# lmb-freiburg/flownet2

Hardware: AMD Instinct MI355X
Metric: image-pairs/sec FlowNetC forward at 448x320 (higher is better)
Workload: dtype f32

## Files before the change

flownet2_amd/_lib.py:

```python
from __future__ import annotations

import ctypes as C
import os
import re

_HERE = os.path.dirname(os.path.abspath(__file__))
SO_PATH = os.path.join(_HERE, "libflownet2_hip.so")
INCLUDE_DIR = os.path.join(_HERE, "..", "include")

_SCALARS = {"int": C.c_int, "float": C.c_float, "size_t": C.c_size_t, "long long": C.c_longlong, "unsigned long long": C.c_ulonglong,
            "char": C.c_char}
_POINTERS = {"float": C.c_void_p, "double": C.c_void_p, "void": C.c_void_p, "unsigned char": C.c_void_p, "char": C.c_char_p, "int": C.POINTER(C.c_int),
             "unsigned": C.POINTER(C.c_uint), "size_t": C.POINTER(C.c_size_t)}
_STRUCT_NAMES = {"fn2_l1loss_params": "L1LossParams", "fn2_l1loss_scale": "L1LossScale"}
_DECLARATOR = re.compile(r"^([\w\s*]*?)(\w+)\s*(?:\[(\d+)\])?$")
_FUNCTION = re.compile(r"^([\w\s*]+?)\b(fn2_\w+)\s*\(([^()]*)\)$")


class Fn2Error(RuntimeError):

    def __init__(self, status: int, message: str):
        super().__init__(f"[fn2 status {status}] {message}")
        self.status = status


def _ctype(spec, structs, where):
    words = [w for w in spec.replace("*", " ").split() if w != "const"]
    base, stars = " ".join(words), spec.count("*")
    if stars == 0 and base in _SCALARS:
        return _SCALARS[base]
    if stars == 1 and base in structs:
        return C.POINTER(structs[base])
    if stars == 1 and base in _POINTERS:
        return _POINTERS[base]
    if stars == 2 and base in ("float", "void"):
        return C.POINTER(C.c_void_p)
    raise ValueError(f"C header: unknown type `{spec.strip()}` in `{where}`")


def _declarator(text, structs, where):
    m = _DECLARATOR.match(text.strip())
    if not m or not m.group(1).strip():
        raise ValueError(f"C header: cannot read `{text.strip()}` in `{where}`")
    t = _ctype(m.group(1), structs, where)
    return m.group(2), (t * int(m.group(3)) if m.group(3) else t), m.group(1)


def parse_header(text, structs=None):
    structs = dict(structs or {})
    functions, constants = {}, {}
    text = re.sub(r"/\*.*?\*/", " ", text, flags=re.S)
    for name, value in re.findall(r"^[ \t]*#[ \t]*define[ \t]+(FN2_\w+)[ \t]+(-?(?:0[xX][0-9a-fA-F]+|\d+))[ \t]*$", text, flags=re.M):
        constants[name] = int(value, 0)
    text = re.sub(r"^[ \t]*#.*$", " ", text, flags=re.M)

    def enum(m):
        value = -1
        for item in filter(None, (s.strip() for s in m.group(1).split(","))):
            name, _, v = (s.strip() for s in item.partition("="))
            value = int(v, 0) if v else value + 1
            constants[name] = value
        return " "
    text = re.sub(r"(?:typedef\s+)?enum\s*\w*\s*\{([^{}]*)\}\s*\w*\s*;", enum, text)

    def struct(m):
        cname, fields = m.group(1), []
        for decl in filter(None, (s.strip() for s in m.group(2).split(";"))):
            first, *more = decl.split(",")
            name, t, spec = _declarator(first, structs, "struct " + cname)
            fields.append((name, t))
            fields += [_declarator(spec + " " + other, structs, "struct " + cname)[:2] for other in more]
        pyname = _STRUCT_NAMES.get(cname) or "".join(w.capitalize() for w in cname.split("_")[1:])
        structs[cname] = type(pyname, (C.Structure,), {"_fields_": fields, "__doc__": cname, "__module__": __name__})
        return " "
    text = re.sub(r"typedef\s+struct\s+(fn2_\w+)\s*\{([^{}]*)\}\s*\w+\s*;", struct, text)

    text = re.sub(r'extern\s*"C"\s*\{|\}', " ", text)
    for stmt in filter(None, (" ".join(s.split()) for s in text.split(";"))):
        m = _FUNCTION.match(stmt)
        if not m:
            raise ValueError(f"C header: cannot read the declaration `{stmt}`")
        params = m.group(3).strip()
        args = [] if params == "void" else [_declarator(p, structs, stmt)[1] for p in params.split(",")]
        functions[m.group(2)] = (_ctype(m.group(1), structs, stmt), args)
    return functions, structs, constants


def _parse_headers():
    per_header, structs, constants, metrics = [], {}, {}, {}
    for h in ("flownet2_hip.h", "flownet2_hip_solver.h", "flownet2_hip_corr_route.h", "flownet2_hip_conv_general.h",
              "flownet2_hip_conv_geometry.h", "flownet2_hip_conv_volume.h", "flownet2_hip_lpq_loss.h", "flownet2_hip_flow_metrics.h"):
        with open(os.path.join(INCLUDE_DIR, h)) as f:
            functions, structs, c = parse_header(f.read(), structs)
        per_header.append(functions)
        (metrics if h == "flownet2_hip_flow_metrics.h" else constants).update(c)
    return per_header, structs, constants, metrics


_PER_HEADER, _STRUCTS, CONSTANTS, FLOW_METRICS_CONSTANTS = _parse_headers()
(EXPORTS, SOLVER_EXPORTS, CORR_ROUTE_EXPORTS, CONV_GENERAL_EXPORTS, CONV_GEOMETRY_EXPORTS, CONV_VOLUME_EXPORTS, LPQ_LOSS_EXPORTS,
 FLOW_METRICS_EXPORTS) = (list(f) for f in _PER_HEADER)
PROTOTYPES = {name: proto for f in _PER_HEADER for name, proto in f.items()}
globals().update({cls.__name__: cls for cls in _STRUCTS.values()})
_HOOKS = parse_header("""
    int fn2_debug_set_correlation_impl(int impl);
    int fn2_debug_correlation_units_plan(int N, int H, int W, int policy, unsigned* out_words, int max_words);
    int fn2_debug_set_resample_generic(int on);
    int fn2_debug_set_correlation_trace(void* device_buffer);""")[0]

_lib = None


def lib():
    global _lib
    if _lib is not None:
        return _lib
    if not os.path.exists(SO_PATH):
        raise RuntimeError(
            f"{SO_PATH} not found: the HIP extension is not built. Run `python -m flownet2_amd.build` "
            "(or __graft_entry__.build()). flownet2_amd has no CPU / PyTorch fallback.")
    L = C.CDLL(SO_PATH)
    for table, required in ((PROTOTYPES, True), (_HOOKS, False)):
        for name, (restype, argtypes) in table.items():
            if not hasattr(L, name):
                if required:
                    raise RuntimeError(f"{SO_PATH} does not export {name}")
                continue
            fn = getattr(L, name)
            fn.restype, fn.argtypes = restype, argtypes
    _lib = L
    return L


def check(status: int):
    if status != 0:
        raise Fn2Error(status, lib().fn2_last_error_string().decode())


def version() -> str:
    return lib().fn2_version().decode()
```

flownet2_amd/csrc/bias_act.hip:

```cpp
#include "fn2_common.hpp"

namespace fn2 {

using f32x4 = __attribute__((ext_vector_type(4))) float;

template <bool VEC4>
__global__ void __launch_bounds__(256) bias_leaky_relu(float* __restrict__ data, const float* __restrict__ bias,
                                                       int C, unsigned hw, float slope) {
  const unsigned plane = blockIdx.y;
  const float b = bias ? bias[plane % (unsigned)C] : 0.f;
  float* p = data + (size_t)plane * hw;
  if constexpr (VEC4) {
    const unsigned n4 = hw / 4;
    for (unsigned i = blockIdx.x * blockDim.x + threadIdx.x; i < n4; i += gridDim.x * blockDim.x) {
      f32x4 v = reinterpret_cast<f32x4*>(p)[i];
#pragma unroll
      for (int j = 0; j < 4; ++j) { const float t = v[j] + b; v[j] = t > 0.f ? t : t * slope; }
      reinterpret_cast<f32x4*>(p)[i] = v;
    }
  } else {
    for (unsigned i = blockIdx.x * blockDim.x + threadIdx.x; i < hw; i += gridDim.x * blockDim.x) {
      const float t = p[i] + b;
      p[i] = t > 0.f ? t : t * slope;
    }
  }
}

constexpr int kBwdChunks = 8;

template <bool MASK, bool VEC4>
__global__ void __launch_bounds__(256) bias_leaky_relu_bwd(const float* __restrict__ top_data, const float* __restrict__ top_diff,
                                                           float* __restrict__ bottom_diff, float* __restrict__ partial,
                                                           unsigned hw, float slope, int C, int dctot, int dc0, int yctot, int yc0) {
  __shared__ float red[4];
  const unsigned plane = blockIdx.y;
  const size_t base = (size_t)plane * hw;
  const size_t dbase = ((size_t)(plane / (unsigned)C) * dctot + dc0 + plane % (unsigned)C) * hw;
  const size_t ybase = ((size_t)(plane / (unsigned)C) * yctot + yc0 + plane % (unsigned)C) * hw;
  float acc = 0.f;
  if constexpr (VEC4) {
    const unsigned n4 = hw / 4;
    for (unsigned i = blockIdx.x * 256u + threadIdx.x; i < n4; i += gridDim.x * 256u) {
      f32x4 g = reinterpret_cast<const f32x4*>(top_diff + dbase)[i];
      if constexpr (MASK) {
        const f32x4 y = reinterpret_cast<const f32x4*>(top_data + ybase)[i];
#pragma unroll
        for (int j = 0; j < 4; ++j) g[j] *= y[j] > 0.f ? 1.f : slope;
        reinterpret_cast<f32x4*>(bottom_diff + base)[i] = g;
      }
      acc += (g[0] + g[1]) + (g[2] + g[3]);
    }
  } else {
    for (unsigned i = blockIdx.x * 256u + threadIdx.x; i < hw; i += gridDim.x * 256u) {
      float g = top_diff[dbase + i];
      if constexpr (MASK) {
        g *= top_data[ybase + i] > 0.f ? 1.f : slope;
        bottom_diff[base + i] = g;
      }
      acc += g;
    }
  }
#pragma unroll
  for (int m = 32; m > 0; m >>= 1) acc += __shfl_xor(acc, m, 64);
  if ((threadIdx.x & 63) == 0) red[threadIdx.x >> 6] = acc;
  __syncthreads();
  if (threadIdx.x == 0) partial[(size_t)plane * gridDim.x + blockIdx.x] = (red[0] + red[1]) + (red[2] + red[3]);
}

template <bool MASK, bool VEC4>
__global__ void __launch_bounds__(256) bias_leaky_relu_bwd_channel(const float* __restrict__ top_data, const float* __restrict__ top_diff,
                                                                   float* __restrict__ bottom_diff, float* __restrict__ bias_diff,
                                                                   int N, unsigned hw, float slope, int C, int dctot, int dc0, int yctot, int yc0,
                                                                   int accumulate) {
  __shared__ float red[4];
  const unsigned c = blockIdx.x;
  float acc = 0.f;
  if constexpr (VEC4) {
    const unsigned q = hw / 4, total = (unsigned)N * q;
    for (unsigned e = threadIdx.x; e < total; e += 256u) {
      const unsigned n = e / q, i = e - n * q;
      f32x4 g = reinterpret_cast<const f32x4*>(top_diff + ((size_t)n * dctot + dc0 + c) * hw)[i];
      if constexpr (MASK) {
        const f32x4 y = reinterpret_cast<const f32x4*>(top_data + ((size_t)n * yctot + yc0 + c) * hw)[i];
#pragma unroll
        for (int j = 0; j < 4; ++j) g[j] *= y[j] > 0.f ? 1.f : slope;
        reinterpret_cast<f32x4*>(bottom_diff + ((size_t)n * C + c) * hw)[i] = g;
      }
      acc += (g[0] + g[1]) + (g[2] + g[3]);
    }
  } else {
    const unsigned total = (unsigned)N * hw;
    for (unsigned e = threadIdx.x; e < total; e += 256u) {
      const unsigned n = e / hw, i = e - n * hw;
      float g = top_diff[((size_t)n * dctot + dc0 + c) * hw + i];
      if constexpr (MASK) {
        g *= top_data[((size_t)n * yctot + yc0 + c) * hw + i] > 0.f ? 1.f : slope;
        bottom_diff[((size_t)n * C + c) * hw + i] = g;
      }
      acc += g;
    }
  }
#pragma unroll
  for (int m = 32; m > 0; m >>= 1) acc += __shfl_xor(acc, m, 64);
  if ((threadIdx.x & 63) == 0) red[threadIdx.x >> 6] = acc;
  __syncthreads();
  if (threadIdx.x == 0 && bias_diff) {
    const float tot = (red[0] + red[1]) + (red[2] + red[3]);
    bias_diff[c] = accumulate ? bias_diff[c] + tot : tot;
  }
}

__global__ void __launch_bounds__(256) bias_diff_finalize(const float* __restrict__ partial, float* __restrict__ bias_diff,
                                                          int N, int C, int chunks, int accumulate) {
  const int c = blockIdx.x * 4 + (threadIdx.x >> 6), lane = threadIdx.x & 63;
  if (c >= C) return;
  const int total = N * chunks;
  float acc = 0.f;
  for (int i = lane; i < total; i += 64) {
    const int n = i / chunks, k = i - n * chunks;
    acc += partial[((size_t)n * C + c) * chunks + k];
  }
#pragma unroll
  for (int m = 32; m > 0; m >>= 1) acc += __shfl_xor(acc, m, 64);
  if (lane == 0) bias_diff[c] = accumulate ? bias_diff[c] + acc : acc;
}

static inline bool small_map(int N, int C, long long hw) { return C >= 128 && (long long)N * hw <= 20000; }

}

using namespace fn2;

FN2_API size_t fn2_bias_leaky_relu_backward_workspace_bytes(int N, int C, int H, int W) {
  (void)H; (void)W;
  if (N <= 0 || C <= 0) return 0;
  return sizeof(float) * (size_t)N * C * kBwdChunks;
}

FN2_API int fn2_bias_leaky_relu_backward_slices(const float* top_data, const float* top_diff, int diff_channels, int diff_c0,
                                                float* bottom_diff, float* bias_diff, int N, int C, int H, int W, float negative_slope,
                                                void* workspace, size_t workspace_bytes, void* stream) {
  return fn2_bias_leaky_relu_backward_slices2(top_data, C, 0, top_diff, diff_channels, diff_c0, bottom_diff, bias_diff, N, C, H, W, negative_slope,
                                              workspace, workspace_bytes, stream);
}

FN2_API int fn2_bias_leaky_relu_backward_slices2(const float* top_data, int data_channels, int data_c0, const float* top_diff, int diff_channels,
                                                 int diff_c0, float* bottom_diff, float* bias_diff, int N, int C, int H, int W, float negative_slope,
                                                 void* workspace, size_t workspace_bytes, void* stream) {
  if (N < 0 || C <= 0 || H <= 0 || W <= 0) return fail(FN2_ERR_INVALID_ARG, "bias_leaky_relu_backward: bad shape [%d,%d,%d,%d]", N, C, H, W);
  if (diff_c0 < 0 || diff_c0 + C > diff_channels) return fail(FN2_ERR_INVALID_ARG, "bias_leaky_relu_backward: top_diff slice outside its blob");
  if (data_c0 < 0 || data_c0 + C > data_channels) return fail(FN2_ERR_INVALID_ARG, "bias_leaky_relu_backward: top_data slice outside its blob");
  if (N == 0) return FN2_OK;
  if (!top_data || !top_diff || !bottom_diff) return fail(FN2_ERR_INVALID_ARG, "bias_leaky_relu_backward: null blob");
  const long long planes = (long long)N * C, hw = (long long)H * W;
  if (planes > 65535 || hw >= (1ll << 32)) return fail(FN2_ERR_UNSUPPORTED, "bias_leaky_relu_backward: blob too large");
  const size_t need = fn2_bias_leaky_relu_backward_workspace_bytes(N, C, H, W);
  if (!workspace || workspace_bytes < need) return fail(FN2_ERR_WORKSPACE, "bias_leaky_relu_backward: workspace too small (%zu < %zu)", workspace_bytes, need);
  hipStream_t st = reinterpret_cast<hipStream_t>(stream);
  float* partial = reinterpret_cast<float*>(workspace);
  const bool vec = hw % 4 == 0 && ((reinterpret_cast<uintptr_t>(top_data) | reinterpret_cast<uintptr_t>(top_diff) | reinterpret_cast<uintptr_t>(bottom_diff)) & 15) == 0;
  if (small_map(N, C, hw)) {
    if (vec) hipLaunchKernelGGL((bias_leaky_relu_bwd_channel<true, true>), dim3((unsigned)C), dim3(256), 0, st, top_data, top_diff, bottom_diff, bias_diff, N,
                                (unsigned)hw, negative_slope, C, diff_channels, diff_c0, data_channels, data_c0, 0);
    else hipLaunchKernelGGL((bias_leaky_relu_bwd_channel<true, false>), dim3((unsigned)C), dim3(256), 0, st, top_data, top_diff, bottom_diff, bias_diff, N,
                            (unsigned)hw, negative_slope, C, diff_channels, diff_c0, data_channels, data_c0, 0);
    return check_launch("bias_leaky_relu_backward");
  }
  if (vec) hipLaunchKernelGGL((bias_leaky_relu_bwd<true, true>), dim3(kBwdChunks, (unsigned)planes), dim3(256), 0, st, top_data, top_diff, bottom_diff, partial,
                              (unsigned)hw, negative_slope, C, diff_channels, diff_c0, data_channels, data_c0);
  else hipLaunchKernelGGL((bias_leaky_relu_bwd<true, false>), dim3(kBwdChunks, (unsigned)planes), dim3(256), 0, st, top_data, top_diff, bottom_diff, partial,
                          (unsigned)hw, negative_slope, C, diff_channels, diff_c0, data_channels, data_c0);
  if (bias_diff) hipLaunchKernelGGL(bias_diff_finalize, dim3((C + 3) / 4), dim3(256), 0, st, partial, bias_diff, N, C, kBwdChunks, 0);
  return check_launch("bias_leaky_relu_backward");
}

FN2_API int fn2_conv_backward_bias(const float* top_diff, int diff_channels, int diff_c0, float* bias_diff, int N, int C, int H, int W,
                                   int accumulate, void* workspace, size_t workspace_bytes, void* stream) {
  if (N < 0 || C <= 0 || H <= 0 || W <= 0) return fail(FN2_ERR_INVALID_ARG, "conv_backward_bias: bad shape [%d,%d,%d,%d]", N, C, H, W);
  if (diff_c0 < 0 || diff_c0 + C > diff_channels) return fail(FN2_ERR_INVALID_ARG, "conv_backward_bias: top_diff slice outside its blob");
  if (N == 0) return FN2_OK;
  if (!top_diff || !bias_diff) return fail(FN2_ERR_INVALID_ARG, "conv_backward_bias: null blob");
  const long long planes = (long long)N * C, hw = (long long)H * W;
  if (planes > 65535 || hw >= (1ll << 32)) return fail(FN2_ERR_UNSUPPORTED, "conv_backward_bias: blob too large");
  const size_t need = fn2_bias_leaky_relu_backward_workspace_bytes(N, C, H, W);
  if (!workspace || workspace_bytes < need) return fail(FN2_ERR_WORKSPACE, "conv_backward_bias: workspace too small (%zu < %zu)", workspace_bytes, need);
  hipStream_t st = reinterpret_cast<hipStream_t>(stream);
  float* partial = reinterpret_cast<float*>(workspace);
  const bool vec = hw % 4 == 0 && (reinterpret_cast<uintptr_t>(top_diff) & 15) == 0;
  if (small_map(N, C, hw)) {
    if (vec) hipLaunchKernelGGL((bias_leaky_relu_bwd_channel<false, true>), dim3((unsigned)C), dim3(256), 0, st, nullptr, top_diff, nullptr, bias_diff, N,
                                (unsigned)hw, 1.0f, C, diff_channels, diff_c0, C, 0, accumulate);
    else hipLaunchKernelGGL((bias_leaky_relu_bwd_channel<false, false>), dim3((unsigned)C), dim3(256), 0, st, nullptr, top_diff, nullptr, bias_diff, N,
                            (unsigned)hw, 1.0f, C, diff_channels, diff_c0, C, 0, accumulate);
    return check_launch("conv_backward_bias");
  }
  if (vec) hipLaunchKernelGGL((bias_leaky_relu_bwd<false, true>), dim3(kBwdChunks, (unsigned)planes), dim3(256), 0, st, nullptr, top_diff, nullptr, partial,
                              (unsigned)hw, 1.0f, C, diff_channels, diff_c0, C, 0);
  else hipLaunchKernelGGL((bias_leaky_relu_bwd<false, false>), dim3(kBwdChunks, (unsigned)planes), dim3(256), 0, st, nullptr, top_diff, nullptr, partial,
                          (unsigned)hw, 1.0f, C, diff_channels, diff_c0, C, 0);
  hipLaunchKernelGGL(bias_diff_finalize, dim3((C + 3) / 4), dim3(256), 0, st, partial, bias_diff, N, C, kBwdChunks, accumulate);
  return check_launch("conv_backward_bias");
}

FN2_API int fn2_bias_leaky_relu_backward(const float* top_data, const float* top_diff, float* bottom_diff, float* bias_diff,
                                         int N, int C, int H, int W, float negative_slope, void* workspace, size_t workspace_bytes,
                                         void* stream) {
  return fn2_bias_leaky_relu_backward_slices(top_data, top_diff, C, 0, bottom_diff, bias_diff, N, C, H, W, negative_slope, workspace,
                                             workspace_bytes, stream);
}

FN2_API int fn2_bias_leaky_relu_forward(float* data, const float* bias, int N, int C, int H, int W, float negative_slope,
                                        void* stream) {
  if (N < 0 || C <= 0 || H <= 0 || W <= 0) return fail(FN2_ERR_INVALID_ARG, "bias_leaky_relu: bad shape [%d,%d,%d,%d]", N, C, H, W);
  if (N == 0) return FN2_OK;
  if (!data) return fail(FN2_ERR_INVALID_ARG, "bias_leaky_relu: null blob");
  const long long planes = (long long)N * C, hw = (long long)H * W;
  if (planes > 65535 * 32ll || hw >= (1ll << 32)) return fail(FN2_ERR_UNSUPPORTED, "bias_leaky_relu: blob too large");
  hipStream_t st = reinterpret_cast<hipStream_t>(stream);
  const bool vec = hw % 4 == 0 && (reinterpret_cast<uintptr_t>(data) & 15) == 0;
  const unsigned per = (unsigned)(vec ? hw / 4 : hw);
  unsigned bx = (per + 255) / 256;
  if (bx > 64) bx = 64;
  for (long long p0 = 0; p0 < planes; p0 += 65535) {
    const unsigned py = (unsigned)((planes - p0) < 65535 ? (planes - p0) : 65535);
    float* base = data + (size_t)p0 * hw;
    const float* bb = bias;
    if (p0 % C != 0) return fail(FN2_ERR_UNSUPPORTED, "bias_leaky_relu: N*C > 65535 with C not dividing 65535");
    if (vec) hipLaunchKernelGGL(bias_leaky_relu<true>, dim3(bx, py), dim3(256), 0, st, base, bb, C, (unsigned)hw, negative_slope);
    else     hipLaunchKernelGGL(bias_leaky_relu<false>, dim3(bx, py), dim3(256), 0, st, base, bb, C, (unsigned)hw, negative_slope);
  }
  return check_launch("bias_leaky_relu_forward");
}

namespace fn2 {
template <bool VEC4>
__global__ void __launch_bounds__(256) scale_shift(const float* __restrict__ in, float* __restrict__ out, const float* __restrict__ shift,
                                                   int C, unsigned hw, int out_ctot, int out_c0, float scale) {
  const unsigned plane = blockIdx.y;
  const unsigned n = plane / (unsigned)C, c = plane % (unsigned)C;
  const float sh = shift ? shift[c] : 0.f;
  const float* p = in + (size_t)plane * hw;
  float* q = out + ((size_t)n * out_ctot + out_c0 + c) * hw;
  if constexpr (VEC4) {
    const unsigned n4 = hw / 4;
    for (unsigned i = blockIdx.x * blockDim.x + threadIdx.x; i < n4; i += gridDim.x * blockDim.x) {
      f32x4 v = reinterpret_cast<const f32x4*>(p)[i];
#pragma unroll
      for (int j = 0; j < 4; ++j) {
        float prod = v[j] * scale;
        asm volatile("" : "+v"(prod));
        v[j] = prod + sh;
      }
      reinterpret_cast<f32x4*>(q)[i] = v;
    }
  } else {
    for (unsigned i = blockIdx.x * blockDim.x + threadIdx.x; i < hw; i += gridDim.x * blockDim.x) {
      float prod = p[i] * scale;
      asm volatile("" : "+v"(prod));
      q[i] = prod + sh;
    }
  }
}
}

FN2_API int fn2_scale_shift_forward(const float* bottom, float* top, const float* shift, int N, int C, int H, int W,
                                    int top_channels, int top_c0, float scale, void* stream) {
  if (N < 0 || C < 1 || H < 1 || W < 1) return fn2::fail(FN2_ERR_INVALID_ARG, "scale_shift: bad shape [%d,%d,%d,%d]", N, C, H, W);
  if (top_c0 < 0 || top_c0 + C > top_channels) return fn2::fail(FN2_ERR_INVALID_ARG, "scale_shift: channel slice outside the blob");
  if (N == 0) return FN2_OK;
  if (!bottom || !top) return fn2::fail(FN2_ERR_INVALID_ARG, "scale_shift: NULL blob pointer");
  if ((long long)N * C > 65535) return fn2::fail(FN2_ERR_UNSUPPORTED, "scale_shift: too many planes");
  const unsigned hw = (unsigned)H * (unsigned)W;
  const bool vec = hw % 4 == 0 && ((reinterpret_cast<uintptr_t>(bottom) | reinterpret_cast<uintptr_t>(top)) & 15) == 0;
  if (vec) hipLaunchKernelGGL(fn2::scale_shift<true>, dim3(fn2::blocks_for(hw / 4, 256, 256), (unsigned)(N * C)), dim3(256), 0, fn2::as_stream(stream), bottom, top,
                              shift, C, hw, top_channels, top_c0, scale);
  else hipLaunchKernelGGL(fn2::scale_shift<false>, dim3(fn2::blocks_for(hw, 256, 64), (unsigned)(N * C)), dim3(256), 0, fn2::as_stream(stream), bottom, top, shift,
                          C, hw, top_channels, top_c0, scale);
  return fn2::check_launch("scale_shift_forward");
}
```

flownet2_amd/csrc/conv_mfma.hip:

```cpp
#include "mfma_tile.hpp"

namespace fn2 {
namespace cv {

using namespace mfma;

struct Args {
  const float* in; const float* wp; const float* bias; float* out;
  int N, Cin, Hin, Win, in_ctot, in_c0;
  int Cout, Hout, Wout, out_ctot, out_c0;
  int pad;
  int nchunks;
  int ksteps;
  int tx, ty;
  int ng;
  unsigned total;
  unsigned nbig;
  float slope; int relu;
};

template <int KS_, int S_, int MW_, int NP_, int WM_, int WNX_, int WNY_, int CQ_, int P16_ = 0, int PIN_ = 0>
struct Cfg : Window<((P16_ ? 1 : 4) * WNY_ - 1) * S_ + KS_,
                    ((P16_ ? 16 : 4) * NP_ * WNX_ - 1) * S_ + KS_ + 4,
                    CQ_, WM_ * WNX_ * WNY_> {
// ... 170 lines not shown
}

template <int KS> struct PackTile {
  static constexpr int T = KS * KS;
  static constexpr int QT = KS == 1 ? 8 : KS == 3 ? 3 : KS == 4 ? 2 : 1;
  static constexpr int CIL = 4 * QT, ROW = CIL * T + 1;
  static constexpr int LDS_FLOATS = 64 * ROW;
};

template <int KS, int ORDER>
__global__ void __launch_bounds__(256) pack_weights_view(const float* __restrict__ w, float* __restrict__ wp, int ksteps, int kalloc,
                                                         int src_co, int src_ci, long long s_co, long long s_ci, int flip) {
  using P = PackTile<KS>;
  constexpr int T = P::T, QT = P::QT, CIL = P::CIL, ROW = P::ROW;
  __shared__ float tile[P::LDS_FLOATS];
  const int grp = blockIdx.x, cq0 = blockIdx.y * QT;
  const int co0 = 64 * grp, ci0 = 4 * cq0;
  const int nquads = ksteps / T;
  constexpr int TOTAL = 64 * CIL * T;
  if constexpr (ORDER == 0) {
    const float* src = w + (size_t)co0 * s_co + (size_t)ci0 * T;
#pragma unroll
    for (int i = threadIdx.x; i < TOTAL; i += 256) {
      const int col = i / (CIL * T), e = i - col * (CIL * T), c = e / T;
      tile[col * ROW + e] = (co0 + col < src_co && ci0 + c < src_ci) ? src[(size_t)col * s_co + e] : 0.f;
    }
  } else if constexpr (ORDER == 1) {
    const float* src = w + (size_t)ci0 * s_ci + (size_t)co0 * T;
#pragma unroll
    for (int i = threadIdx.x; i < TOTAL; i += 256) {
      const int c = i / (64 * T), e = i - c * (64 * T), col = e / T, t = e - col * T;
      tile[col * ROW + c * T + t] = (co0 + col < src_co && ci0 + c < src_ci) ? src[(size_t)c * s_ci + e] : 0.f;
    }
  } else {
#pragma unroll
    for (int i = threadIdx.x; i < TOTAL; i += 256) {
      const int col = i / (CIL * T), e = i - col * (CIL * T), c = e / T, t = e - c * T;
      tile[col * ROW + e] = (co0 + col < src_co && ci0 + c < src_ci) ? w[(size_t)(co0 + col) * s_co + (size_t)(ci0 + c) * s_ci + t] : 0.f;
    }
  }
  __syncthreads();
  const int nq = min(QT, nquads - cq0);
  float* dst = wp + ((size_t)grp * kalloc + (size_t)cq0 * T) * 256;
  const int j = threadIdx.x & 3, lane = threadIdx.x >> 2;
  const float* trow = tile + (16 * j + (lane & 15)) * ROW + (lane >> 4) * T;
#pragma unroll
  for (int ks = 0; ks < QT * T; ++ks) {
    const int cq = ks / T, tap = ks - cq * T;
    if (cq < nq) dst[ks * 256 + threadIdx.x] = trow[4 * cq * T + (flip ? T - 1 - tap : tap)];
  }
  if (cq0 + QT >= nquads)
    for (int i = threadIdx.x; i < (kalloc - ksteps) * 256; i += 256) wp[((size_t)grp * kalloc + ksteps) * 256 + i] = 0.f;
}

template <int KS>
static void launch_pack_view(const float* w, float* wp, int Cout, int ksteps, int kalloc, int src_co, int src_ci, long long s_co, long long s_ci, int flip,
                             hipStream_t st) {
  using P = PackTile<KS>;
  const dim3 grid((unsigned)((Cout + 63) / 64), (unsigned)cdiv(ksteps / P::T, P::QT));
  if (s_ci == (long long)P::T) hipLaunchKernelGGL((pack_weights_view<KS, 0>), grid, dim3(256), 0, st, w, wp, ksteps, kalloc, src_co, src_ci, s_co, s_ci, flip);
  else if (s_co == (long long)P::T) hipLaunchKernelGGL((pack_weights_view<KS, 1>), grid, dim3(256), 0, st, w, wp, ksteps, kalloc, src_co, src_ci, s_co, s_ci, flip);
  else hipLaunchKernelGGL((pack_weights_view<KS, 2>), grid, dim3(256), 0, st, w, wp, ksteps, kalloc, src_co, src_ci, s_co, s_ci, flip);
}

constexpr int kSpare = 8;
constexpr int kChunkQuads = 2;

inline int chunk_quads(int KS) { return KS == 1 ? 8 : kChunkQuads; }
inline int ksteps_for(int Cin, int KS) { return cdiv(cdiv(Cin, 4), chunk_quads(KS)) * chunk_quads(KS) * KS * KS; }

template <class K>
static void set_geometry(Args& a) {
  if constexpr (K::P16) {
    a.Win *= a.Hin; a.Hin = 1; a.Wout *= a.Hout; a.Hout = 1;
  }
  a.tx = cdiv(a.Wout, K::TW); a.ty = cdiv(a.Hout, K::TH);
  a.ng = a.Cout / (16 * K::MW * K::WM);
  a.nchunks = cdiv(cdiv(a.Cin, 4), K::CQ);
}

inline long long tiles_of(const Args& a) { return (long long)a.N * a.tx * a.ty * a.ng; }

template <class K>
static int launch(const Args& base, hipStream_t st) {
  Args a = base;
  set_geometry<K>(a);
  a.nbig = (unsigned)tiles_of(a);
  return launch_tiles<&conv_mfma<K>>(a, tiles_of(a), K::THREADS, (int)(sizeof(float) * 2 * K::BUF), "conv_mfma", "conv_mfma_forward", st);
}

inline unsigned whole_rounds(long long tiles) { return (unsigned)(tiles / 256 * 256); }

template <class K>
static int launch_tail(const Args& base, hipStream_t st) {
  if constexpr (K::MW < 2) {
    return fail(FN2_ERR_UNSUPPORTED, "conv_mfma: variant has no split tail");
  } else {
    Args a = base;
    set_geometry<K>(a);
    if (tiles_of(a) > 0x1fffff00ll) return fail(FN2_ERR_UNSUPPORTED, "conv_mfma: grid too large");
    a.total = (unsigned)tiles_of(a); a.nbig = whole_rounds(a.total);
    const unsigned nsm = 2 * (a.total - a.nbig);
    const unsigned grid = a.nbig + 8 * ((nsm + 7) / 8);
    constexpr size_t lds = sizeof(float) * 2 * K::BUF;
    set_dynamic_lds_once<&conv_mfma_tail<K>>((int)lds);
    hipLaunchKernelGGL((conv_mfma_tail<K>), dim3(grid), dim3(K::THREADS), lds, st, a);
    return check_launch("conv_mfma_forward");
  }
}

struct Variant {
  int ks, s, mw, np, wm, wnx, wny, p16;
  int (*fn)(const Args&, hipStream_t);
  int (*fn_tail)(const Args&, hipStream_t);
};

#define FN2_CV_LIST(X) \
   \
  X(1, 1, 2, 7, 2, 2, 1, 8, 1) X(1, 1, 2, 7, 2, 1, 2, 8, 1) X(1, 1, 4, 7, 1, 2, 2, 8, 0) X(1, 1, 4, 7, 1, 1, 4, 8, 0) X(1, 1, 2, 6, 2, 2, 1, 8, 1) \
  X(1, 1, 2, 4, 2, 2, 1, 8, 1) X(1, 1, 2, 7, 1, 2, 2, 8, 0) X(1, 1, 2, 7, 1, 4, 1, 8, 0) X(1, 1, 2, 4, 1, 2, 2, 8, 0) X(1, 1, 4, 4, 1, 2, 2, 8, 0) \
   \
  X(3, 1, 2, 7, 2, 2, 1, 2, 1) X(3, 1, 2, 7, 2, 1, 2, 2, 1) X(3, 1, 4, 7, 1, 2, 2, 2, 0) X(3, 1, 4, 7, 1, 1, 4, 2, 0) \
  X(3, 1, 2, 6, 2, 2, 1, 2, 1) X(3, 1, 4, 6, 1, 2, 2, 2, 0) X(3, 1, 4, 4, 1, 2, 2, 2, 0) X(3, 1, 2, 4, 2, 2, 1, 2, 1) \
   \
  X(3, 2, 2, 7, 2, 1, 2, 2, 1) X(3, 2, 4, 7, 1, 1, 4, 2, 0) X(3, 2, 2, 6, 2, 2, 1, 2, 1) X(3, 2, 4, 6, 1, 2, 2, 2, 0) X(3, 2, 2, 4, 2, 2, 1, 2, 1) \
   \
  X(4, 2, 2, 7, 2, 2, 1, 2, 1) X(4, 2, 2, 7, 2, 1, 2, 2, 1) X(4, 2, 4, 7, 1, 2, 2, 2, 0) X(4, 2, 2, 6, 2, 2, 1, 2, 1) X(4, 2, 4, 4, 1, 2, 2, 2, 0) X(4, 2, 2, 4, 2, 2, 1, 2, 1) \
   \
  X(5, 2, 2, 7, 2, 2, 1, 1, 1) X(5, 2, 2, 7, 2, 1, 2, 1, 1) X(5, 2, 4, 7, 1, 2, 2, 1, 0) X(5, 2, 4, 7, 1, 1, 4, 1, 0) \
  X(5, 2, 2, 6, 2, 2, 1, 1, 1) X(5, 2, 4, 6, 1, 2, 2, 1, 0) X(5, 2, 4, 4, 1, 2, 2, 1, 0) \
   \
  X(7, 2, 2, 6, 2, 2, 1, 1, 1) X(7, 2, 2, 7, 2, 2, 1, 1, 1) X(7, 2, 4, 4, 1, 2, 2, 1, 0) X(7, 2, 4, 6, 1, 2, 2, 1, 0) X(7, 2, 2, 4, 2, 2, 1, 1, 1)

template <class K, int TAIL> struct TailFn { static constexpr int (*fn)(const Args&, hipStream_t) = nullptr; };
template <class K> struct TailFn<K, 1> { static constexpr int (*fn)(const Args&, hipStream_t) = &launch_tail<K>; };

#define FN2_CV_ROW(KS, S, MW, NP, WM, WNX, WNY, CQ, TAIL) \
  {KS, S, MW, NP, WM, WNX, WNY, 0, &launch<Cfg<KS, S, MW, NP, WM, WNX, WNY, CQ>>, TailFn<Cfg<KS, S, MW, NP, WM, WNX, WNY, CQ>, TAIL>::fn},
#define FN2_CV_ROW16(MW, NP, WM, WNX, WNY, TAIL) \
  {1, 1, MW, NP, WM, WNX, WNY, 1, &launch<Cfg<1, 1, MW, NP, WM, WNX, WNY, 8, 1>>, TailFn<Cfg<1, 1, MW, NP, WM, WNX, WNY, 8, 1>, TAIL>::fn},
#define FN2_CV_PIN(KS, S, MW, NP, WM, WNX, WNY, CQ, P16, TAIL) \
  {KS, S, MW, NP, WM, WNX, WNY, P16, &launch<Cfg<KS, S, MW, NP, WM, WNX, WNY, CQ, P16, 1>>, TailFn<Cfg<KS, S, MW, NP, WM, WNX, WNY, CQ, P16, 1>, TAIL>::fn},
static const Variant kVariants[] = {FN2_CV_LIST(FN2_CV_ROW)
  FN2_CV_ROW16(2, 7, 2, 2, 1, 1) FN2_CV_ROW16(2, 7, 4, 1, 1, 1) FN2_CV_ROW16(4, 7, 1, 4, 1, 0) FN2_CV_ROW16(4, 7, 2, 2, 1, 0) FN2_CV_ROW16(2, 5, 2, 2, 1, 1)
  FN2_CV_ROW16(2, 4, 2, 2, 1, 1) FN2_CV_ROW16(2, 7, 1, 4, 1, 0) FN2_CV_ROW16(2, 5, 1, 4, 1, 0) FN2_CV_ROW16(4, 5, 1, 4, 1, 0) FN2_CV_ROW16(2, 4, 1, 4, 1, 0)
  FN2_CV_ROW16(4, 5, 2, 2, 1, 0) FN2_CV_ROW16(4, 4, 2, 2, 1, 0)
  FN2_CV_ROW16(2, 9, 4, 1, 1, 1) FN2_CV_ROW16(2, 9, 2, 2, 1, 1) FN2_CV_ROW16(2, 3, 2, 2, 1, 1) FN2_CV_ROW16(4, 3, 1, 4, 1, 0)
  FN2_CV_ROW16(4, 9, 4, 1, 1, 0) FN2_CV_ROW16(4, 9, 2, 2, 1, 0) FN2_CV_ROW16(4, 7, 4, 1, 1, 0)
  FN2_CV_PIN(5, 2, 2, 7, 2, 2, 1, 1, 0, 1) FN2_CV_PIN(5, 2, 2, 7, 2, 1, 2, 1, 0, 1)
  FN2_CV_PIN(1, 1, 4, 9, 4, 1, 1, 8, 1, 0) FN2_CV_PIN(1, 1, 2, 9, 4, 1, 1, 8, 1, 1) FN2_CV_PIN(1, 1, 2, 5, 2, 2, 1, 8, 1, 1) FN2_CV_PIN(1, 1, 4, 7, 4, 1, 1, 8, 1, 0)
  FN2_CV_PIN(1, 1, 2, 7, 2, 2, 1, 8, 1, 1) FN2_CV_PIN(1, 1, 2, 3, 2, 2, 1, 8, 1, 1)
  FN2_CV_PIN(3, 1, 2, 7, 2, 2, 1, 2, 0, 1) FN2_CV_PIN(3, 1, 2, 6, 2, 2, 1, 2, 0, 1) FN2_CV_PIN(3, 2, 2, 7, 2, 1, 2, 2, 0, 1) FN2_CV_PIN(3, 2, 2, 6, 2, 2, 1, 2, 0, 1)
  FN2_CV_PIN(4, 2, 2, 7, 2, 2, 1, 2, 0, 1) FN2_CV_PIN(4, 2, 2, 6, 2, 2, 1, 2, 0, 1) FN2_CV_PIN(5, 2, 2, 6, 2, 2, 1, 1, 0, 1)
  FN2_CV_PIN(7, 2, 2, 6, 2, 2, 1, 1, 0, 1) FN2_CV_PIN(7, 2, 4, 6, 1, 2, 2, 1, 0, 0)};
constexpr int kNumVariants = sizeof(kVariants) / sizeof(kVariants[0]);

int g_forced_variant = -1;

static double variant_cost(const Variant& v, const Args& a, bool tail) {
  const int tw = (v.p16 ? 16 : 4) * v.np * v.wnx, th = (v.p16 ? 1 : 4) * v.wny;
  const long long wgs = v.p16 ? (long long)a.N * cdiv(a.Wout * a.Hout, tw) * (a.Cout / (16 * v.mw * v.wm))
                              : (long long)a.N * cdiv(a.Wout, tw) * cdiv(a.Hout, th) * (a.Cout / (16 * v.mw * v.wm));
  double rounds = (double)((wgs + 255) / 256);
  if (tail) {
    const long long r = wgs % 256;
    if (wgs < 256 || r == 0 || r > 128) return 1e30;
    rounds = (double)(wgs / 256) + 0.5 * 1.12;
  }
  const double eff = 1.0 / (1.0 + 0.08 * (4.0 / v.mw - 1.0) + 0.02 * (7.0 / v.np - 1.0));
  return rounds * v.mw * v.np / eff;
}

static bool variant_applies(const Variant& v, const Args& a, int KS, int S) {
  if (!v.p16 && a.Win % 4 != 0) return false;
  return v.ks == KS && v.s == S && a.Cout % (16 * v.mw * v.wm) == 0;
}

}
}

using namespace fn2;

FN2_API size_t fn2_conv_mfma_packed_floats(int Cout, int Cin, int kernel) {
  if (Cout <= 0 || Cout % 32 != 0 || Cin <= 0 || kernel <= 0) return 0;
  return (size_t)((Cout + 63) / 64) * (cv::ksteps_for(Cin, kernel) + cv::kSpare) * 256;
}

FN2_API int fn2_conv_mfma_pack_weights_view(const float* weight, float* packed, int Cout, int Cin, int kernel, int src_cout, int src_cin,
                                            long long stride_cout, long long stride_cin, int flip, void* stream);

FN2_API int fn2_conv_mfma_pack_weights(const float* weight, float* packed, int Cout, int Cin, int kernel, void* stream) {
  if (!weight || !packed) return fail(FN2_ERR_INVALID_ARG, "conv_mfma_pack_weights: null blob");
  if (Cout <= 0 || Cout % 32 != 0 || Cin <= 0 || (kernel != 1 && kernel != 3 && kernel != 4 && kernel != 5 && kernel != 7))
    return fail(FN2_ERR_UNSUPPORTED, "conv_mfma_pack_weights: needs Cout %% 32 == 0 and kernel_size 1, 3, 4, 5 or 7 (got Cout %d, kernel %d)", Cout, kernel);
  return fn2_conv_mfma_pack_weights_view(weight, packed, Cout, Cin, kernel, Cout, Cin, (long long)Cin * kernel * kernel, (long long)kernel * kernel, 0, stream);
}

FN2_API int fn2_conv_mfma_pack_weights_view(const float* weight, float* packed, int Cout, int Cin, int kernel, int src_cout, int src_cin,
                                            long long stride_cout, long long stride_cin, int flip, void* stream) {
  if (!weight || !packed) return fail(FN2_ERR_INVALID_ARG, "conv_mfma_pack_weights_view: null blob");
  if (Cout <= 0 || Cout % 32 != 0 || Cin <= 0 || (kernel != 1 && kernel != 3 && kernel != 4 && kernel != 5 && kernel != 7))
    return fail(FN2_ERR_UNSUPPORTED, "conv_mfma_pack_weights_view: needs Cout %% 32 == 0 and kernel_size 1, 3, 4, 5 or 7 (got Cout %d, kernel %d)", Cout, kernel);
  if (src_cout < 1 || src_cout > Cout || src_cin < 1 || src_cin > Cin || stride_cout < 1 || stride_cin < 1)
    return fail(FN2_ERR_INVALID_ARG, "conv_mfma_pack_weights_view: bad source view (%d of %d, %d of %d channels, strides %lld / %lld)", src_cout, Cout,
                src_cin, Cin, stride_cout, stride_cin);
  const int ksteps = cv::ksteps_for(Cin, kernel), kalloc = ksteps + cv::kSpare;
  hipStream_t st = as_stream(stream);
  switch (kernel) {
    case 1: cv::launch_pack_view<1>(weight, packed, Cout, ksteps, kalloc, src_cout, src_cin, stride_cout, stride_cin, flip ? 1 : 0, st); break;
    case 3: cv::launch_pack_view<3>(weight, packed, Cout, ksteps, kalloc, src_cout, src_cin, stride_cout, stride_cin, flip ? 1 : 0, st); break;
    case 4: cv::launch_pack_view<4>(weight, packed, Cout, ksteps, kalloc, src_cout, src_cin, stride_cout, stride_cin, flip ? 1 : 0, st); break;
    case 5: cv::launch_pack_view<5>(weight, packed, Cout, ksteps, kalloc, src_cout, src_cin, stride_cout, stride_cin, flip ? 1 : 0, st); break;
    default: cv::launch_pack_view<7>(weight, packed, Cout, ksteps, kalloc, src_cout, src_cin, stride_cout, stride_cin, flip ? 1 : 0, st); break;
  }
  return check_launch("conv_mfma_pack_weights_view");
}

FN2_API int fn2_conv_mfma_supported(int Cin, int Hin, int Win, int Cout, int kernel, int stride, int pad) {
  if (Cin <= 0 || Hin <= 0 || Win <= 0 || Cout <= 0 || Cout % 32 != 0) return 0;
  if (kernel == 1 ? ((long long)Hin * Win) % 4 != 0 : Win % 4 != 0) return 0;
  if (!((kernel == 1 && stride == 1) || (kernel == 3 && (stride == 1 || stride == 2)) || (kernel == 4 && stride == 2) || (kernel == 5 && stride == 2) || (kernel == 7 && stride == 2))) return 0;
  if (pad < 0 || pad > 4 || pad > kernel - 1) return 0;
  if ((long long)Cin * Hin * Win >= (1ll << 28)) return 0;
  const int Hout = (Hin + 2 * pad - kernel) / stride + 1, Wout = (Win + 2 * pad - kernel) / stride + 1;
  if (Hout < 1 || Wout < 1) return 0;
  cv::Args a{};
  a.Win = Win; a.Cout = Cout;
  for (int i = 0; i < cv::kNumVariants; ++i)
    if (cv::variant_applies(cv::kVariants[i], a, kernel, stride)) return 1;
  return 0;
}

FN2_API int fn2_debug_set_conv_variant(int v) { cv::g_forced_variant = v; return FN2_OK; }
FN2_API int fn2_conv_mfma_num_variants(void) { return cv::kNumVariants; }

FN2_API int fn2_conv_mfma_forward(const float* bottom, const float* packed_weight, const float* bias, float* top,
                                  int N, int Cin, int Hin, int Win, int bottom_channels, int bottom_c0,
                                  int Cout, int top_channels, int top_c0, int kernel, int stride, int pad,
                                  int relu, float negative_slope, void* stream) {
  if (N < 0) return fail(FN2_ERR_INVALID_ARG, "conv_mfma: bad batch");
  if (N == 0) return FN2_OK;
  if (const int rc = mfma::check_conv_args("conv_mfma", bottom, packed_weight, top, Cin, bottom_channels, bottom_c0, Cout, top_channels, top_c0, [&] {
        return fn2_conv_mfma_supported(Cin, Hin, Win, Cout, kernel, stride, pad) ? FN2_OK
            : fail(FN2_ERR_UNSUPPORTED, "conv_mfma: unsupported geometry (Cin %d, %dx%d, Cout %d, k %d s %d p %d)", Cin, Hin, Win, Cout, kernel, stride, pad);
      }))
    return rc;
  cv::Args a{};
  a.in = bottom; a.wp = packed_weight; a.bias = bias; a.out = top;
  a.N = N; a.Cin = Cin; a.Hin = Hin; a.Win = Win; a.in_ctot = bottom_channels; a.in_c0 = bottom_c0;
  a.Cout = Cout; a.Hout = (Hin + 2 * pad - kernel) / stride + 1; a.Wout = (Win + 2 * pad - kernel) / stride + 1;
  a.out_ctot = top_channels; a.out_c0 = top_c0; a.pad = pad;
  a.ksteps = cv::ksteps_for(Cin, kernel) + cv::kSpare;
  a.slope = negative_slope; a.relu = relu;
  hipStream_t st = as_stream(stream);
  static TuneCache cache("conv_mfma", cv::kNumVariants);
  const TuneKey key{N, Cin, Hin, Win, Cout, kernel, stride, pad, bottom_channels == Cin, top_channels == Cout};
  mfma::Pick p;
  if (const int rc = mfma::pick_variant(p, "conv_mfma", cv::g_forced_variant, cv::kNumVariants, true, cache, key, st,
                                        [&](int i) { return cv::variant_applies(cv::kVariants[i], a, kernel, stride); },
                                        [&](int i, bool tail) { return cv::variant_cost(cv::kVariants[i], a, tail); },
                                        [&](int i, bool tail) { return tail ? cv::kVariants[i].fn_tail(a, st) : cv::kVariants[i].fn(a, st); },
                                        [&](int i) { return cv::kVariants[i].fn_tail != nullptr; }))
    return rc;
  return p.tail ? cv::kVariants[p.variant].fn_tail(a, st) : cv::kVariants[p.variant].fn(a, st);
}
```

flownet2_amd/csrc/flow_head.hip:

```cpp
#include "fn2_common.hpp"

namespace fn2 {

constexpr int kHeadPix = 64;

template <int G>
__global__ void __launch_bounds__(kHeadPix* G) conv3x3_c2_taps(const float* __restrict__ in, const float* __restrict__ w,
                                                                float* __restrict__ P, int N, int C, int H, int W, int nsplit) {
  __shared__ float red[G][18][kHeadPix];
  const int lane_pix = threadIdx.x % kHeadPix;
  const int grp = __builtin_amdgcn_readfirstlane(threadIdx.x / kHeadPix);
  const size_t plane = (size_t)H * W;
  const long long total = (long long)N * H * W;
  const long long p = (long long)blockIdx.x * kHeadPix + lane_pix;
  const bool live = p < total;
  const int n = live ? (int)(p / (long long)plane) : 0;
  const unsigned pix = live ? (unsigned)(p - (long long)n * plane) : 0u;
  const float* src = in + (size_t)n * C * plane + pix;
  float a[18];
#pragma unroll
  for (int k = 0; k < 18; ++k) a[k] = 0.f;
  const int ngroups = G * nsplit;
  const int c_per = (C + ngroups - 1) / ngroups;
  const int c_lo = min(C, ((int)blockIdx.y * G + grp) * c_per), c_hi = min(C, c_lo + c_per);
  for (int c = c_lo; c < c_hi; c += 8) {
    float v[8];
#pragma unroll
    for (int cc = 0; cc < 8; ++cc) v[cc] = (c + cc < c_hi) ? src[(size_t)(c + cc) * plane] : 0.f;
    __builtin_amdgcn_sched_barrier(0);
#pragma unroll
    for (int cc = 0; cc < 8; ++cc) {
      if (c + cc < c_hi) {
        const float* w0 = w + (size_t)(c + cc) * 9;
        const float* w1 = w + ((size_t)C + c + cc) * 9;
#pragma unroll
        for (int t = 0; t < 9; ++t) {
          a[t] = fmaf(w0[t], v[cc], a[t]);
          a[9 + t] = fmaf(w1[t], v[cc], a[9 + t]);
        }
      }
    }
  }
#pragma unroll
  for (int k = 0; k < 18; ++k) red[grp][k][lane_pix] = a[k];
  __syncthreads();
  if (live) {
    float* dst = P + ((size_t)blockIdx.y * N + n) * 18 * plane + pix;
    for (int k = grp; k < 18; k += G) {
      float sacc = 0.f;
#pragma unroll
      for (int g = 0; g < G; ++g) sacc += red[g][k][lane_pix];
      dst[(size_t)k * plane] = sacc;
    }
  }
}

template <int NSPLIT>
__global__ void __launch_bounds__(256) conv3x3_c2_gather(const float* __restrict__ P, const float* __restrict__ bias,
                                                          float* __restrict__ out, int N, int H, int W) {
  const unsigned plane = (unsigned)H * W;
  const unsigned pix = blockIdx.x * 256u + threadIdx.x;
  if (pix >= plane) return;
  const int y = pix / W, x = pix - y * W;
  const unsigned no = blockIdx.y;
  const unsigned n = no >> 1, o = no & 1;
  float v[NSPLIT][9];
#pragma unroll
  for (int sp = 0; sp < NSPLIT; ++sp) {
    const float* Pn = P + (((size_t)sp * N + n) * 18 + o * 9) * plane;
#pragma unroll
    for (int dy = 0; dy < 3; ++dy)
#pragma unroll
      for (int dx = 0; dx < 3; ++dx) {
        const int yy = y + dy - 1, xx = x + dx - 1;
        const bool ok = yy >= 0 && yy < H && xx >= 0 && xx < W;
        v[sp][dy * 3 + dx] = ok ? Pn[(size_t)(dy * 3 + dx) * plane + (unsigned)yy * W + xx] : 0.f;
      }
  }
  float sacc = bias ? bias[o] : 0.f;
#pragma unroll
  for (int sp = 0; sp < NSPLIT; ++sp)
#pragma unroll
    for (int t = 0; t < 9; ++t) sacc += v[sp][t];
  out[(size_t)no * plane + pix] = sacc;
}

__global__ void __launch_bounds__(256) deconv4x4s2_c2(const float* __restrict__ in, const float* __restrict__ w,
                                                       const float* __restrict__ bias, float* __restrict__ out,
                                                       int N, int H, int W, int out_ctot, int out_c0) {
  const int Ho = 2 * H, Wo = 2 * W;
  const long long total = (long long)N * Ho * Wo;
  for (long long idx = blockIdx.x * (long long)blockDim.x + threadIdx.x; idx < total; idx += (long long)gridDim.x * blockDim.x) {
    const int X = (int)(idx % Wo), Y = (int)((idx / Wo) % Ho), n = (int)(idx / ((long long)Wo * Ho));
    float a0 = bias ? bias[0] : 0.f, a1 = bias ? bias[1] : 0.f;
#pragma unroll
    for (int ty = 0; ty < 2; ++ty) {
      const int ky = ((Y + 1) & 1) + 2 * ty;
      const int iy = (Y + 1 - ky) / 2;
      if (Y + 1 - ky < 0 || iy >= H) continue;
#pragma unroll
      for (int tx = 0; tx < 2; ++tx) {
        const int kx = ((X + 1) & 1) + 2 * tx;
        const int ix = (X + 1 - kx) / 2;
        if (X + 1 - kx < 0 || ix >= W) continue;
#pragma unroll
        for (int c = 0; c < 2; ++c) {
          const float v = in[(((size_t)n * 2 + c) * H + iy) * W + ix];
          a0 = fmaf(w[((c * 2 + 0) * 4 + ky) * 4 + kx], v, a0);
          a1 = fmaf(w[((c * 2 + 1) * 4 + ky) * 4 + kx], v, a1);
        }
      }
    }
    out[(((size_t)n * out_ctot + out_c0 + 0) * Ho + Y) * Wo + X] = a0;
    out[(((size_t)n * out_ctot + out_c0 + 1) * Ho + Y) * Wo + X] = a1;
  }
}

}

using namespace fn2;

constexpr int kHeadG = 16;

static int head_splits(int N, int C, int H, int W) {
  const long long blocks = ((long long)order_batch(N) * H * W + kHeadPix - 1) / kHeadPix;
  int nsplit = 1;
  while (nsplit < 8 && blocks * kHeadG * nsplit < 4096 && C >= 8 * kHeadG * nsplit * 2) nsplit *= 2;
  return nsplit;
}

FN2_API size_t fn2_predict_flow_conv_workspace_bytes(int N, int C, int H, int W) {
  if (N < 1 || C < 1 || H < 1 || W < 1) return 0;
  return sizeof(float) * (size_t)head_splits(N, C, H, W) * N * 18 * H * W;
}

FN2_API int fn2_predict_flow_conv_forward(const float* in, const float* weight, const float* bias, float* out,
                                          int N, int C, int H, int W, void* workspace, size_t workspace_bytes, void* stream) {
  if (N < 0 || C < 1 || H < 1 || W < 1) return fail(FN2_ERR_INVALID_ARG, "predict_flow_conv: bad shape [%d,%d,%d,%d]", N, C, H, W);
  if (N == 0) return FN2_OK;
  if (!in || !weight || !out) return fail(FN2_ERR_INVALID_ARG, "predict_flow_conv: NULL blob pointer");
  if ((long long)H * W >= (1ll << 31) || 2ll * N > 65535) return fail(FN2_ERR_UNSUPPORTED, "predict_flow_conv: blob too large");
  const size_t need = fn2_predict_flow_conv_workspace_bytes(N, C, H, W);
  if (!workspace || workspace_bytes < need) return fail(FN2_ERR_WORKSPACE, "predict_flow_conv: workspace too small (%zu < %zu)", workspace_bytes, need);
  const long long total = (long long)N * H * W;
  const unsigned blocks = (unsigned)((total + kHeadPix - 1) / kHeadPix);
  const int nsplit = head_splits(N, C, H, W);
  hipStream_t st = as_stream(stream);
  float* P = reinterpret_cast<float*>(workspace);
  hipLaunchKernelGGL(conv3x3_c2_taps<kHeadG>, dim3(blocks, nsplit), dim3(kHeadPix * kHeadG), 0, st, in, weight, P, N, C, H, W, nsplit);
  const dim3 g2(((unsigned)H * W + 255) / 256, 2 * N);
  switch (nsplit) {
    case 1: hipLaunchKernelGGL(conv3x3_c2_gather<1>, g2, dim3(256), 0, st, P, bias, out, N, H, W); break;
    case 2: hipLaunchKernelGGL(conv3x3_c2_gather<2>, g2, dim3(256), 0, st, P, bias, out, N, H, W); break;
    case 4: hipLaunchKernelGGL(conv3x3_c2_gather<4>, g2, dim3(256), 0, st, P, bias, out, N, H, W); break;
    default: hipLaunchKernelGGL(conv3x3_c2_gather<8>, g2, dim3(256), 0, st, P, bias, out, N, H, W); break;
  }
  return check_launch("predict_flow_conv_forward");
}

FN2_API int fn2_upsample_flow_deconv_forward(const float* in, const float* weight, const float* bias, float* out,
                                             int N, int H, int W, void* stream) {
  if (N < 0 || H < 1 || W < 1) return fail(FN2_ERR_INVALID_ARG, "upsample_flow_deconv: bad shape");
  if (N == 0) return FN2_OK;
  if (!in || !weight || !out) return fail(FN2_ERR_INVALID_ARG, "upsample_flow_deconv: NULL blob pointer");
  const long long total = (long long)N * 4 * H * W;
  hipLaunchKernelGGL(deconv4x4s2_c2, dim3(blocks_for(total, 256, 4096)), dim3(256), 0, as_stream(stream), in, weight, bias, out, N, H, W, 2, 0);
  return check_launch("upsample_flow_deconv_forward");
}

FN2_API int fn2_upsample_flow_deconv_forward_into(const float* in, const float* weight, const float* bias, float* top,
                                                  int N, int H, int W, int top_channels, int top_c0, void* stream) {
  if (N < 0 || H < 1 || W < 1) return fail(FN2_ERR_INVALID_ARG, "upsample_flow_deconv: bad shape");
  if (top_c0 < 0 || top_c0 + 2 > top_channels) return fail(FN2_ERR_INVALID_ARG, "upsample_flow_deconv: channel slice outside the blob");
  if (N == 0) return FN2_OK;
  if (!in || !weight || !top) return fail(FN2_ERR_INVALID_ARG, "upsample_flow_deconv: NULL blob pointer");
  const long long total = (long long)N * 4 * H * W;
  hipLaunchKernelGGL(deconv4x4s2_c2, dim3(blocks_for(total, 256, 4096)), dim3(256), 0, as_stream(stream), in, weight, bias, top, N, H, W, top_channels, top_c0);
  return check_launch("upsample_flow_deconv_forward_into");
}
```

flownet2_amd/csrc/resample.hip:

```cpp
#include "fn2_common.hpp"

#include <cmath>

#pragma clang fp contract(off)

namespace fn2 {

__device__ __forceinline__ float bicubic_coeff(float x_) {
  const float x = fabsf(x_);
  if (x <= 1.0f) return x * x * (1.5f * x - 2.5f) + 1.0f;
  else if (x < 2.0f) return x * (x * (-0.5f * x + 2.5f) - 4.0f) + 2.0f;
  else return 0.0f;
}
__device__ __forceinline__ float triangle_coeff(float x) {
  if (-1 <= x && x < 0) return x + 1;
  if (0 <= x && x <= 1) return 1 - x;
  return 0;
}

struct ResampleArgs {
  int NC, Hin, Win, Hout, Wout;
  float fx, fy, ax, ay;
  int rx, ry;
  int ppt;
  int C, octot, oc0, o2ctot, o2c0;
  float in_scale, out2_scale;
};

__device__ __forceinline__ size_t top_plane(int plane, int C, int ctot, int c0) {
  const int n = plane / C;
  return (size_t)n * ctot + c0 + (plane - n * C);
}
__device__ __forceinline__ float scaled(float v, float s) { return v * s; }


template <bool EXTRA>
__global__ void __launch_bounds__(256) resample_nearest(const float* __restrict__ in, float* __restrict__ out, float* __restrict__ out2, ResampleArgs a) {
  const unsigned hw_out = (unsigned)a.Hout * a.Wout, hw_in = (unsigned)a.Hin * a.Win;
  const unsigned p = blockIdx.x * 256u + threadIdx.x;
  if (p >= hw_out) return;
  const int y_out = p / a.Wout, x_out = p - y_out * a.Wout;
  const float x_in = x_out * a.fx + a.fy / 2.0f - 0.5f;
  const float y_in = y_out * a.fy + a.fx / 2.0f - 0.5f;
  int xr = (int)roundf(x_in), yr = (int)roundf(y_in);
  xr = min(max(xr, 0), a.Win - 1);
  yr = min(max(yr, 0), a.Hin - 1);
  const unsigned src = (unsigned)yr * a.Win + xr;
  for (int c = blockIdx.y * a.ppt; c < min(a.NC, (int)(blockIdx.y + 1) * a.ppt); ++c) {
    const float raw = in[(size_t)c * hw_in + src];
    const float v = EXTRA ? scaled(raw, a.in_scale) : raw;
    out[(EXTRA ? top_plane(c, a.C, a.octot, a.oc0) : (size_t)c) * hw_out + p] = v;
    if (EXTRA && out2) out2[top_plane(c, a.C, a.o2ctot, a.o2c0) * hw_out + p] = scaled(v, a.out2_scale);
  }
}

template <bool CUBIC, bool FAST, bool EXTRA>
__global__ void __launch_bounds__(256) resample_interp(const float* __restrict__ in, float* __restrict__ out, float* __restrict__ out2, ResampleArgs a) {
  const unsigned hw_out = (unsigned)a.Hout * a.Wout, hw_in = (unsigned)a.Hin * a.Win;
  const unsigned p = blockIdx.x * 256u + threadIdx.x;
  if (p >= hw_out) return;
  const int y_out = p / a.Wout, x_out = p - y_out * a.Wout;
  const float x_in = x_out * a.fx + a.fy / 2.0f - 0.5f;
  const float y_in = y_out * a.fy + a.fx / 2.0f - 0.5f;
  const int xr = (int)roundf(x_in), yr = (int)roundf(y_in);
  const int c_lo = blockIdx.y * a.ppt, c_hi = min(a.NC, c_lo + a.ppt);
  if constexpr (FAST) {
    float px[5], ky[5];
    unsigned xo[5], yo[5], mx = 0u, my = 0u;
#pragma unroll
    for (int i = 0; i < 5; ++i) {
      const int x = xr - 2 + i, y = yr - 2 + i;
      const bool okx = x >= 0 && x < a.Win && (i >= 2 - a.rx && i <= 2 + a.rx);
      const bool oky = y >= 0 && y < a.Hin && (i >= 2 - a.ry && i <= 2 + a.ry);
      const float kx = CUBIC ? bicubic_coeff(a.ax * (x_in - x)) : triangle_coeff(a.ax * (x_in - x));
      const float kyv = CUBIC ? bicubic_coeff(a.ay * (y_in - y)) : triangle_coeff(a.ay * (y_in - y));
      px[i] = okx ? a.ax * kx * a.ay : 0.f;
      ky[i] = oky ? kyv : 0.f;
      xo[i] = okx ? (unsigned)x : 0u;
      yo[i] = oky ? (unsigned)y * a.Win : 0u;
      mx |= (okx ? 1u : 0u) << i;
      my |= (oky ? 1u : 0u) << i;
    }
    float wsum = 0.f;
#pragma unroll
    for (int j = 0; j < 5; ++j)
#pragma unroll
      for (int i = 0; i < 5; ++i) wsum += px[i] * ky[j];
    for (int c = c_lo; c < c_hi; ++c) {
      const float* src = in + (size_t)c * hw_in;
      float sum = 0.f;
#pragma unroll
      for (int j = 0; j < 5; ++j)
#pragma unroll
        for (int i = 0; i < 5; ++i) {
          const float w = px[i] * ky[j];
          const float tap = ((mx >> i) & (my >> j) & 1u) ? src[yo[j] + xo[i]] : 0.f;
          sum = fmaf(w, EXTRA ? scaled(tap, a.in_scale) : tap, sum);
        }
      const float v = (!wsum) ? 0.f : (sum / wsum);
      out[(EXTRA ? top_plane(c, a.C, a.octot, a.oc0) : (size_t)c) * hw_out + p] = v;
      if (EXTRA && out2) out2[top_plane(c, a.C, a.o2ctot, a.o2c0) * hw_out + p] = scaled(v, a.out2_scale);
    }
  } else {
    const int y0 = max(yr - a.ry, 0), y1 = min(yr + a.ry, a.Hin - 1);
    const int x0 = max(xr - a.rx, 0), x1 = min(xr + a.rx, a.Win - 1);
    for (int c = c_lo; c < c_hi; ++c) {
      const float* src = in + (size_t)c * hw_in;
      float sum = 0.f, wsum = 0.f;
      for (int y = y0; y <= y1; ++y) {
        const float kyv = CUBIC ? bicubic_coeff(a.ay * (y_in - y)) : triangle_coeff(a.ay * (y_in - y));
        for (int x = x0; x <= x1; ++x) {
          const float dx = x_in - x;
          const float w = a.ax * (CUBIC ? bicubic_coeff(a.ax * dx) : triangle_coeff(a.ax * dx)) * a.ay * kyv;
          const float tap = src[(size_t)y * a.Win + x];
          sum = fmaf(w, EXTRA ? scaled(tap, a.in_scale) : tap, sum);
          wsum += w;
        }
      }
      const float v = (!wsum) ? 0.f : (sum / wsum);
      out[(EXTRA ? top_plane(c, a.C, a.octot, a.oc0) : (size_t)c) * hw_out + p] = v;
      if (EXTRA && out2) out2[top_plane(c, a.C, a.o2ctot, a.o2c0) * hw_out + p] = scaled(v, a.out2_scale);
    }
  }
}

constexpr int kLeanTW = 64, kLeanTH = 32, kLeanRows = 8, kLeanPlanes = 2;
constexpr int kLeanFR = kLeanTH + 6, kLeanLW = 80;
constexpr int kLeanScanVec = 3, kLeanScanScalar = 11;

template <bool EXTRA>
__device__ __attribute__((noinline)) void resample_exact_rows(const float* __restrict__ src, float* __restrict__ dst, float* __restrict__ dst2,
                                                               const ResampleArgs& a, int x_out, bool live_x, int y_first, int y_last) {
  const float x_in = x_out * a.fx + a.fy / 2.0f - 0.5f;
  const int xr = (int)roundf(x_in);
  float px[5]; unsigned xo[5], mx = 0u;
#pragma unroll
  for (int i = 0; i < 5; ++i) {
    const int x = xr - 2 + i;
    const bool okx = x >= 0 && x < a.Win;
    px[i] = okx ? a.ax * triangle_coeff(a.ax * (x_in - x)) * a.ay : 0.f;
    xo[i] = okx ? (unsigned)x : 0u;
    mx |= (okx ? 1u : 0u) << i;
  }
  for (int y_out = y_first; y_out <= y_last; y_out += 4) {
    const float y_in = y_out * a.fy + a.fx / 2.0f - 0.5f;
    const int yr = (int)roundf(y_in);
    float ky[5]; unsigned yo[5], my = 0u;
#pragma unroll
    for (int j = 0; j < 5; ++j) {
      const int y = yr - 2 + j;
      const bool oky = y >= 0 && y < a.Hin;
      ky[j] = oky ? triangle_coeff(a.ay * (y_in - y)) : 0.f;
      yo[j] = oky ? (unsigned)y * a.Win : 0u;
// ... 78 lines not shown
  if (vec) {
#pragma unroll
    for (int it = 0; it < kLeanScanVec; ++it) {
      const unsigned idx = threadIdx.x + 256u * it;
      const unsigned r = ncol == 1u ? idx : __umulhi(idx, magic), q = idx - r * ncol;
#pragma unroll
      for (int pl = 0; pl < kLeanPlanes; ++pl) {
        f4 t = v[it][pl];
        if constexpr (EXTRA) t *= a.in_scale;
        poison[pl] = __builtin_elementwise_fma(f2{0.f, 0.f}, f2{t[0], t[1]}, poison[pl]);
        poison[pl] = __builtin_elementwise_fma(f2{0.f, 0.f}, f2{t[2], t[3]}, poison[pl]);
        if (idx < nitem) *reinterpret_cast<f4*>(&s_img[pl][r * kLeanLW + 4 * q]) = t;
      }
    }
  } else {
#pragma unroll 4
    for (int it = 0; it < kLeanScanScalar; ++it) {
      const unsigned idx = threadIdx.x + 256u * it;
      const unsigned r = ncol == 1u ? idx : __umulhi(idx, magic), q = idx - r * ncol;
      const size_t goff = (size_t)(fy0 + (int)r) * a.Win + fx0 + q;
#pragma unroll
      for (int pl = 0; pl < kLeanPlanes; ++pl) {
        float t = idx < nitem ? in[(size_t)min(c_lo + pl, a.NC - 1) * hw_in + goff] : 0.f;
        if constexpr (EXTRA) t = scaled(t, a.in_scale);
        poison[pl][0] = fmaf(0.f, t, poison[pl][0]);
        if (idx < nitem) s_img[pl][r * kLeanLW + q] = t;
      }
    }
  }
  unsigned badmask = 0u;
#pragma unroll
  for (int pl = 0; pl < kLeanPlanes; ++pl) {
    const float p = poison[pl][0] + poison[pl][1];
    badmask |= (p != p ? 1u : 0u) << pl;
  }
  if (badmask) atomicOr(&s_bad, badmask);
  __syncthreads();
  const unsigned verdict = s_bad;
  const int xl0 = min(max(cx, 0), a.Win - 1) - fx0, xl1 = min(max(cx + 1, 0), a.Win - 1) - fx0;
  char* dstb[kLeanPlanes]; char* dst2b[kLeanPlanes];
#pragma unroll
  for (int pl = 0; pl < kLeanPlanes; ++pl) {
    const int c = min(c_lo + pl, a.NC - 1);
    dstb[pl] = reinterpret_cast<char*>(out + (EXTRA ? top_plane(c, a.C, a.octot, a.oc0) : (size_t)c) * hw_out);
    dst2b[pl] = (EXTRA && out2) ? reinterpret_cast<char*>(out2 + top_plane(c, a.C, a.o2ctot, a.o2c0) * hw_out) : nullptr;
  }
  if (verdict) {
#pragma unroll
    for (int pl = 0; pl < kLeanPlanes; ++pl)
      if (c_lo + pl < a.NC && ((verdict >> pl) & 1u))
        resample_exact_rows<EXTRA>(in + (size_t)(c_lo + pl) * hw_in, reinterpret_cast<float*>(dstb[pl]), reinterpret_cast<float*>(dst2b[pl]), a, x_out, live_x,
                                   y0 + ty, yh_out);
  }
#pragma unroll
  for (int k = 0; k < kLeanRows; ++k) {
    const int row = kLeanTW + ty + 4 * k;
    const int y_out = y0 + ty + 4 * k;
    const int cy = s_c[row];
    const f2 kyv = *reinterpret_cast<const f2*>(&s_k[row][0]);
    const int yl0 = (min(max(cy, 0), a.Hin - 1) - fy0) * kLeanLW, yl1 = (min(max(cy + 1, 0), a.Hin - 1) - fy0) * kLeanLW;
    const float w0 = pxl[0] * kyv[0], w1 = pxl[1] * kyv[0], w2 = pxl[0] * kyv[1], w3 = pxl[1] * kyv[1];
    const float wsum = (((0.f + w0) + w1) + w2) + w3;
    const unsigned boff = 4u * ((unsigned)y_out * (unsigned)a.Wout + (unsigned)x_out);
    const bool live = live_x && y_out <= yh_out;
#pragma unroll
    for (int pl = 0; pl < kLeanPlanes; ++pl) {
      const float t0 = s_img[pl][yl0 + xl0], t1 = s_img[pl][yl0 + xl1], t2 = s_img[pl][yl1 + xl0], t3 = s_img[pl][yl1 + xl1];
      const float sum = fmaf(w3, t3, fmaf(w2, t2, fmaf(w1, t1, fmaf(w0, t0, 0.f))));
      const float v = (!wsum) ? 0.f : (sum / wsum);
      if (live && c_lo + pl < a.NC && !((verdict >> pl) & 1u)) {
        *reinterpret_cast<float*>(dstb[pl] + boff) = v;
        if (EXTRA && dst2b[pl]) *reinterpret_cast<float*>(dst2b[pl] + boff) = scaled(v, a.out2_scale);
      }
    }
  }
}

template <int F, bool EXTRA>
__global__ void __launch_bounds__(256) resample_up_linear(const float* __restrict__ in, float* __restrict__ out, float* __restrict__ out2, ResampleArgs a) {
  const unsigned hw_out = (unsigned)a.Hout * a.Wout, hw_in = (unsigned)a.Hin * a.Win;
  const unsigned p = blockIdx.x * 256u + threadIdx.x;
  if (p >= hw_in) return;
  const int i = p / a.Win, j = p - i * a.Win;
  unsigned xo[5], yo[5], mx = 0u, my = 0u;
#pragma unroll
  for (int t = 0; t < 5; ++t) {
    const int x = j - 2 + t, y = i - 2 + t;
    const bool okx = x >= 0 && x < a.Win, oky = y >= 0 && y < a.Hin;
    xo[t] = okx ? (unsigned)x : 0u;
    yo[t] = oky ? (unsigned)y * a.Win : 0u;
    mx |= (okx ? 1u : 0u) << t;
    my |= (oky ? 1u : 0u) << t;
  }
  float px[F][3], ky[F][3], wsum[F][F];
#pragma unroll
  for (int ph = 0; ph < F; ++ph) {
    const float x_in = (F * j + ph) * a.fx + a.fy / 2.0f - 0.5f;
    const float y_in = (F * i + ph) * a.fy + a.fx / 2.0f - 0.5f;
#pragma unroll
    for (int t = 0; t < 3; ++t) {
      const int x = j - 1 + t, y = i - 1 + t;
      px[ph][t] = ((mx >> (t + 1)) & 1u) ? a.ax * triangle_coeff(a.ax * (x_in - x)) * a.ay : 0.f;
      ky[ph][t] = ((my >> (t + 1)) & 1u) ? triangle_coeff(a.ay * (y_in - y)) : 0.f;
    }
  }
#pragma unroll
  for (int py = 0; py < F; ++py)
#pragma unroll
    for (int qx = 0; qx < F; ++qx) {
      float w = 0.f;
#pragma unroll
      for (int r = 0; r < 3; ++r)
#pragma unroll
        for (int t = 0; t < 3; ++t) w += px[qx][t] * ky[py][r];
      wsum[py][qx] = w;
    }
  using vec_t = __attribute__((ext_vector_type(F))) float;
  const int c_lo = blockIdx.y * a.ppt, c_hi = min(a.NC, c_lo + a.ppt);
  for (int c = c_lo; c < c_hi; ++c) {
    const float* src = in + (size_t)c * hw_in;
    float v[3][3], poison = 0.f;
#pragma unroll
    for (int r = 0; r < 5; ++r)
#pragma unroll
      for (int t = 0; t < 5; ++t) {
        float s = ((mx >> t) & (my >> r) & 1u) ? src[yo[r] + xo[t]] : 0.f;
        if constexpr (EXTRA) s = scaled(s, a.in_scale);
        if (r >= 1 && r <= 3 && t >= 1 && t <= 3) v[r - 1][t - 1] = s;
        else poison = fmaf(0.f, s, poison);
      }
    const size_t pix0 = (size_t)(F * i) * a.Wout + F * j;
    float* dst = out + (EXTRA ? top_plane(c, a.C, a.octot, a.oc0) : (size_t)c) * hw_out + pix0;
    float* dst2 = (EXTRA && out2) ? out2 + top_plane(c, a.C, a.o2ctot, a.o2c0) * hw_out + pix0 : nullptr;
#pragma unroll
    for (int py = 0; py < F; ++py) {
      vec_t o;
#pragma unroll
      for (int qx = 0; qx < F; ++qx) {
        float sum = poison;
#pragma unroll
        for (int r = 0; r < 3; ++r)
#pragma unroll
          for (int t = 0; t < 3; ++t) sum = fmaf(px[qx][t] * ky[py][r], v[r][t], sum);
        const float ws = wsum[py][qx];
        o[qx] = (!ws) ? 0.f : (ws == 1.0f ? sum : sum / ws);
      }
      *reinterpret_cast<vec_t*>(dst + (size_t)py * a.Wout) = o;
      if (EXTRA && dst2) {
        vec_t o2;
#pragma unroll
        for (int qx = 0; qx < F; ++qx) o2[qx] = scaled(o[qx], a.out2_scale);
        *reinterpret_cast<vec_t*>(dst2 + (size_t)py * a.Wout) = o2;
      }
    }
  }
}

}

using namespace fn2;

static int g_resample_generic = 0;
FN2_API int fn2_debug_set_resample_generic(int on) { g_resample_generic = on; return FN2_OK; }

FN2_API int fn2_resample_forward_slices(const float* in, float in_scale, float* out, int top_channels, int top_c0,
                                        float* out2, int top2_channels, int top2_c0, float out2_scale,
                                        int N, int C, int Hin, int Win, int Hout, int Wout, int type, int antialias_param, void* stream) {
  if (N < 0 || C < 1 || Hin < 1 || Win < 1) return fail(FN2_ERR_INVALID_ARG, "resample: bad bottom shape");
  if (Hout < 1 || Wout < 1) return fail(FN2_ERR_INVALID_ARG, "ResampleLayer must have top_height > 0 and top_width > 0");
  if (type != FN2_RESAMPLE_NEAREST && type != FN2_RESAMPLE_LINEAR && type != FN2_RESAMPLE_CUBIC)
    return fail(FN2_ERR_UNSUPPORTED, "ResampleLayer: only CUBIC, LINEAR and NEAREST interpolation is supported for now");
  if (N == 0) return FN2_OK;
  if (!in || !out) return fail(FN2_ERR_INVALID_ARG, "resample: NULL blob pointer");
  if (top_c0 < 0 || top_c0 + C > top_channels || (out2 && (top2_c0 < 0 || top2_c0 + C > top2_channels)))
    return fail(FN2_ERR_INVALID_ARG, "resample: channel slice outside its blob");
  ResampleArgs a;
  a.C = C; a.octot = top_channels; a.oc0 = top_c0; a.o2ctot = out2 ? top2_channels : C; a.o2c0 = out2 ? top2_c0 : 0;
  a.in_scale = in_scale; a.out2_scale = out2_scale;
  a.NC = N * C; a.Hin = Hin; a.Win = Win; a.Hout = Hout; a.Wout = Wout;
  a.fx = (float)Win / (float)Wout;
  a.fy = (float)Hin / (float)Hout;
  const bool is_down = (a.fx > 1) || (a.fy > 1);
  const bool antialias = is_down && antialias_param;
  const int kernel_width = (type == FN2_RESAMPLE_CUBIC) ? 4 : 2;
  a.ax = 1.0f / (antialias ? a.fx : 1.0f);
  a.ay = 1.0f / (antialias ? a.fy : 1.0f);
  a.rx = (a.fx < 1.0f) ? 2 : (int)std::ceil((float)kernel_width / a.ax);
  a.ry = (a.fy < 1.0f) ? 2 : (int)std::ceil((float)kernel_width / a.ay);
  if ((long long)Hout * Wout >= (1ll << 29) || (long long)Hin * Win >= (1ll << 29)) return fail(FN2_ERR_UNSUPPORTED, "resample: plane too large");
  const unsigned bx = (unsigned)(((long long)Hout * Wout + 255) / 256);
  a.ppt = 1;
  while (a.ppt < 8 && (long long)bx * ((a.NC + 2 * a.ppt - 1) / (2 * a.ppt)) >= 2048) a.ppt *= 2;
  const unsigned by = (unsigned)((a.NC + a.ppt - 1) / a.ppt);
  if (by > 65535u) return fail(FN2_ERR_UNSUPPORTED, "resample: too many planes");
  const dim3 grid(bx, by);
  hipStream_t st = as_stream(stream);
  const bool fast = a.rx <= 2 && a.ry <= 2;
  const int up = (Wout == 4 * Win && Hout == 4 * Hin) ? 4 : (Wout == 2 * Win && Hout == 2 * Hin) ? 2 : 0;
  if (type == FN2_RESAMPLE_LINEAR && up && ((reinterpret_cast<uintptr_t>(out) | reinterpret_cast<uintptr_t>(out2)) & 15) == 0 && !g_resample_generic) {
    const unsigned bxi = (unsigned)(((long long)Hin * Win + 255) / 256);
    a.ppt = 1;
    while (a.ppt < 4 && (long long)bxi * ((a.NC + 2 * a.ppt - 1) / (2 * a.ppt)) >= 8192) a.ppt *= 2;
    const dim3 gi(bxi, (unsigned)((a.NC + a.ppt - 1) / a.ppt));
    if (gi.y > 65535u) return fail(FN2_ERR_UNSUPPORTED, "resample: too many planes");
    const bool extra = in_scale != 1.0f || out2 || top_channels != C;
    if (up == 4 && extra) hipLaunchKernelGGL((resample_up_linear<4, true>), gi, dim3(256), 0, st, in, out, out2, a);
    else if (up == 4) hipLaunchKernelGGL((resample_up_linear<4, false>), gi, dim3(256), 0, st, in, out, out2, a);
    else if (extra) hipLaunchKernelGGL((resample_up_linear<2, true>), gi, dim3(256), 0, st, in, out, out2, a);
    else hipLaunchKernelGGL((resample_up_linear<2, false>), gi, dim3(256), 0, st, in, out, out2, a);
    return check_launch("resample_forward");
  }
  const bool ex = in_scale != 1.0f || out2 || top_channels != C;
  if (type == FN2_RESAMPLE_LINEAR && fast && a.ax == 1.0f && a.ay == 1.0f && a.rx == 2 && a.ry == 2 && a.fx <= 1.0f && a.fy <= 1.0f && !g_resample_generic) {
    const unsigned gx = (unsigned)((Wout + kLeanTW - 1) / kLeanTW), gy = (unsigned)((Hout + kLeanTH - 1) / kLeanTH);
    const unsigned gz = (unsigned)((a.NC + kLeanPlanes - 1) / kLeanPlanes);
    if (gy > 65535u || gz > 65535u) return fail(FN2_ERR_UNSUPPORTED, "resample: too many tiles / planes");
    if (ex) hipLaunchKernelGGL((resample_linear_lean<true>), dim3(gx, gy, gz), dim3(256), 0, st, in, out, out2, a);
    else hipLaunchKernelGGL((resample_linear_lean<false>), dim3(gx, gy, gz), dim3(256), 0, st, in, out, out2, a);
    return check_launch("resample_forward");
  }
#define FN2_RS(K_) do { if (ex) hipLaunchKernelGGL((K_<true>), grid, dim3(256), 0, st, in, out, out2, a); \
                        else hipLaunchKernelGGL((K_<false>), grid, dim3(256), 0, st, in, out, out2, a); } while (0)
#define FN2_RSI(C_, F_) do { if (ex) hipLaunchKernelGGL((resample_interp<C_, F_, true>), grid, dim3(256), 0, st, in, out, out2, a); \
                             else hipLaunchKernelGGL((resample_interp<C_, F_, false>), grid, dim3(256), 0, st, in, out, out2, a); } while (0)
  if (type == FN2_RESAMPLE_NEAREST) FN2_RS(resample_nearest);
  else if (type == FN2_RESAMPLE_CUBIC) { if (fast) FN2_RSI(true, true); else FN2_RSI(true, false); }
  else { if (fast) FN2_RSI(false, true); else FN2_RSI(false, false); }
#undef FN2_RS
#undef FN2_RSI
  return check_launch("resample_forward");
}

FN2_API int fn2_resample_forward(const float* in, float* out, int N, int C, int Hin, int Win, int Hout, int Wout,
                                 int type, int antialias_param, void* stream) {
  return fn2_resample_forward_slices(in, 1.0f, out, C, 0, nullptr, 0, 0, 1.0f, N, C, Hin, Win, Hout, Wout, type, antialias_param, stream);
}
```

flownet2_amd/functional.py:

```python
from __future__ import annotations

import collections
import os

import torch

from . import ops


_BATCH_INVARIANT = [False]


def set_batch_invariant(on: bool = True):
    _BATCH_INVARIANT[0] = bool(on)
    ops.set_batch_invariant(bool(on))


def batch_invariant() -> bool:
    return _BATCH_INVARIANT[0]


LIBRARY_FALLBACKS = [0]


# ... 302 lines not shown
        d0, d1 = ops.l1loss_backward_multi(ctx.params, b0, b1, ctx.weights, g.contiguous(), ctx.ws, need1=need1)
        grads = [d if ctx.needs_input_grad[3 + k] else None for k, d in enumerate(d0)]
        grads += [d if ctx.needs_input_grad[3 + n + k] else None for k, d in enumerate(d1)]
        return (None, None, None) + tuple(grads)


def l1_loss_multi(preds, targets, weights, l2_per_location=False, l2_prescale_by_channels=False, normalize_by_num_entries=False,
                  epsilon=1e-2, plateau=0.0):
    p = ops.l1_params(l2_per_location, l2_prescale_by_channels, normalize_by_num_entries, epsilon, plateau)
    blobs = [t.contiguous() for t in preds] + [t.contiguous() for t in targets]
    return _L1LossMulti.apply(p, tuple(float(w) for w in weights), len(preds), *blobs)


class _LpqLoss(torch.autograd.Function):
    @staticmethod
    def forward(ctx, b0, b1, params):
        loss, ws = ops.lpq_loss_forward(params, b0, b1)
        ctx.params, ctx.ws = params, ws
        ctx.save_for_backward(b0, b1)
        return loss

    @staticmethod
    def backward(ctx, g):
        b0, b1 = ctx.saved_tensors
        d0, d1 = ops.lpq_loss_backward(ctx.params, b0, b1, float(g), ctx.ws)
        return (d0 if ctx.needs_input_grad[0] else None), (d1 if (b1 is not None and ctx.needs_input_grad[1]) else None), None


def lpq_loss(b0, b1=None, p=1.0, q=1.0, p_epsilon=0.0, q_epsilon=1e-2, l2_prescale_by_channels=False, normalize_by_num_entries=False):
    params = ops.lpq_params(p, q, p_epsilon, q_epsilon, l2_prescale_by_channels, normalize_by_num_entries)
    return _LpqLoss.apply(b0.contiguous(), b1.contiguous() if b1 is not None else None, params)


class _LpqLossMulti(torch.autograd.Function):

    @staticmethod
    def forward(ctx, params, weights, n, *blobs):
        b0, b1 = list(blobs[:n]), list(blobs[n:])
        total, losses, ws = ops.lpq_loss_forward_multi(params, b0, b1, weights)
        ctx.params, ctx.weights, ctx.n, ctx.ws = params, weights, n, ws
        ctx.save_for_backward(*blobs)
        ctx.mark_non_differentiable(losses)
        return total, losses

    @staticmethod
    def backward(ctx, g, _g_losses):
        n = ctx.n
        blobs = ctx.saved_tensors
        b0, b1 = list(blobs[:n]), list(blobs[n:])
        need1 = any(ctx.needs_input_grad[3 + n:])
        d0, d1 = ops.lpq_loss_backward_multi(ctx.params, b0, b1, ctx.weights, g.contiguous(), ctx.ws, need1=need1)
        grads = [d if ctx.needs_input_grad[3 + k] else None for k, d in enumerate(d0)]
        grads += [d if ctx.needs_input_grad[3 + n + k] else None for k, d in enumerate(d1)]
        return (None, None, None) + tuple(grads)


def lpq_loss_multi(preds, targets, weights, p=1.0, q=1.0, p_epsilon=0.0, q_epsilon=1e-2, l2_prescale_by_channels=False,
                   normalize_by_num_entries=False):
    params = ops.lpq_params(p, q, p_epsilon, q_epsilon, l2_prescale_by_channels, normalize_by_num_entries)
    blobs = [t.contiguous() for t in preds] + [t.contiguous() for t in targets]
    return _LpqLossMulti.apply(params, tuple(float(w) for w in weights), len(preds), *blobs)


def flow_metrics(pred, gt, valid=None, occ=None, *, outlier=(3.0, 0.05), bands=(10.0, 40.0), epe_map=False):
    from .evaluate import FlowMetrics
    if torch.is_grad_enabled() and any(t is not None and t.requires_grad for t in (pred, gt, valid, occ)):
        raise RuntimeError("flow_metrics is not differentiable: detach the inputs or call it under torch.no_grad() (the training loss is "
                           "l1_loss / lpq_loss)")
    results, emap = ops.flow_metrics(pred, gt, valid, occ, outlier=outlier, bands=bands, epe_map=epe_map)
    return FlowMetrics(results[:-1].cpu().numpy(), epe_map=emap)


def add_loss_flags(ap):
    ap.add_argument("--loss", choices=("l1", "lpq"), default="l1", help="l1: L1Loss{l2_per_location} (the default); lpq: LpqLoss with --lpq-p / --lpq-q")
    ap.add_argument("--lpq-p", type=float, nargs="+", default=[2.0], metavar="P", help="p of every episode (one value: constant)")
    ap.add_argument("--lpq-q", type=float, nargs="+", default=[0.2], metavar="Q", help="q of every episode")
    ap.add_argument("--lpq-starts", type=int, nargs="+", default=[], metavar="ITER", help="iteration at which each episode starts (the first is 0)")
    ap.add_argument("--lpq-p-epsilon", type=float, default=0.0)
    ap.add_argument("--lpq-q-epsilon", type=float, default=1e-2)


def loss_schedule(args):
    from .lpq_schedule import LpqSchedule
    return LpqSchedule(args.lpq_starts, args.lpq_p, args.lpq_q) if args.loss == "lpq" else None


class _PredictFlow(torch.autograd.Function):

    @staticmethod
    def forward(ctx, x, weight, bias):
        ctx.save_for_backward(x, weight)
        ctx.has_bias = bias is not None
        return ops.predict_flow_conv_forward(x.contiguous(), weight.contiguous(), bias)

    @staticmethod
    def backward(ctx, g):
        x, w = ctx.saved_tensors
        blob, c0 = _channel_slice(x)
        g = g.contiguous()
        need_x, need_w, need_b = ctx.needs_input_grad[0], ctx.needs_input_grad[1], ctx.has_bias and ctx.needs_input_grad[2]
        side = _wgrad_side_stream(g, x, w) if (need_w or need_b) and need_x else None
        if side is None:
            return ops.predict_flow_conv_backward((blob, c0, x.shape[1]), w, g, need_x, need_w, need_b)
        dx, _, _ = ops.predict_flow_conv_backward((blob, c0, x.shape[1]), w, g, True, False, False)
        main = torch.cuda.current_stream(g.device)
        side.wait_stream(main)
        with torch.cuda.stream(side):
            _, dw, db = ops.predict_flow_conv_backward((blob, c0, x.shape[1]), w, g, False, need_w, need_b)
        for t in (g, blob):
            t.record_stream(side)
        for t in (dw, db):
            if t is not None:
                t.record_stream(main)
        if dw is not None:
            _SIDE_PENDING.append((w, dw.data_ptr()))
        return dx, dw, db


class _UpsampleFlow(torch.autograd.Function):

    @staticmethod
    def forward(ctx, x, weight, bias, into=None):
        ctx.save_for_backward(x, weight)
        ctx.has_bias = bias is not None
        if into is None:
            return ops.upsample_flow_deconv_forward(x.contiguous(), weight.contiguous(), bias)
        ops.upsample_flow_deconv_forward(x.contiguous(), weight.contiguous(), bias, out=into[0], out_c0=into[1])
        return into[0][:, into[1]:into[1] + 2]

    @staticmethod
    def backward(ctx, g):
        x, w = ctx.saved_tensors
        dx, dw, db = ops.upsample_flow_deconv_backward(x.contiguous(), w, g.contiguous(), ctx.needs_input_grad[0], ctx.needs_input_grad[1],
                                                       ctx.has_bias and ctx.needs_input_grad[2])
        return dx, dw, db, None


def predict_flow_conv(x, weight, bias=None):
    run = lambda xx, ww, bb: ops.predict_flow_conv_forward(xx.contiguous(), ww.contiguous(), bb)
    if _needs_grad(x, weight, bias):
        if ops.predict_flow_conv_backward_supported(x.shape[0], x.shape[1], x.shape[2], x.shape[3]):
            return _PredictFlow.apply(x, weight, bias)
        return _OwnForwardConv.apply(x, weight, bias, run, 1, 1, 0.0, False, False)
    return run(x, weight, bias)


def upsample_flow_deconv(x, weight, bias=None, out=None, out_c0=0):
    if out is not None and not _needs_grad(x, weight, bias):
        return ops.upsample_flow_deconv_forward(x.contiguous(), weight.contiguous(), bias, out=out, out_c0=out_c0)
    run = lambda xx, ww, bb: ops.upsample_flow_deconv_forward(xx.contiguous(), ww.contiguous(), bb)
    if _needs_grad(x, weight, bias):
        return _UpsampleFlow.apply(x, weight, bias, None if out is None else (out, out_c0))
    return run(x, weight, bias)


class _BiasLeakyReLU(torch.autograd.Function):

    @staticmethod
    def forward(ctx, y, bias, negative_slope):
        ctx.mark_dirty(y)
        ops.bias_leaky_relu_(y, bias, negative_slope)
        ctx.slope = negative_slope
        ctx.has_bias = bias is not None
        ctx.save_for_backward(y)
        return y

    @staticmethod
    def backward(ctx, g):
        (y,) = ctx.saved_tensors
        d, db = ops.bias_leaky_relu_backward(y, g.contiguous(), ctx.slope, ctx.has_bias and ctx.needs_input_grad[1])
        return d, db, None


def conv_bias_leaky_relu(y, bias, negative_slope=0.1):
    if not y.is_contiguous():
        if bias is not None:
            y = y + bias.view(1, -1, 1, 1)
        return torch.nn.functional.leaky_relu(y, negative_slope)
    if torch.is_grad_enabled() and (y.requires_grad or (bias is not None and bias.requires_grad)):
        return _BiasLeakyReLU.apply(y, bias, negative_slope)
    return ops.bias_leaky_relu_(y, bias, negative_slope)


def invalidate_weight_caches():
    _bump_weight_generation()
    _PACKED_T.clear()


_WEIGHT_GENERATION = [0]


def weight_generation() -> int:
    return _WEIGHT_GENERATION[0]


def _bump_weight_generation(*_a, **_k):
    _WEIGHT_GENERATION[0] += 1


try:
    from torch.optim.optimizer import register_optimizer_step_post_hook as _reg_step_hook
    _reg_step_hook(_bump_weight_generation)
    _HAVE_STEP_HOOK = True
except Exception:
    _HAVE_STEP_HOOK = False


def _cached(cache, key, w, make):
    import weakref
    if w.requires_grad and (not _HAVE_STEP_HOOK or (w.is_cuda and torch.cuda.is_current_stream_capturing())):
        cache.pop(key, None)
        return make()
    gen = _WEIGHT_GENERATION[0] if w.requires_grad else -1
    hit = cache.get(key)
    if hit is None or hit[0]() is not w or hit[1] != w._version or hit[3] != gen:
        hit = (weakref.ref(w, lambda _r, k=key: cache.pop(k, None)), w._version, make(), gen)
        cache[key] = hit
    return hit[2]


_ROUTE_FORCE = [False]


def set_route_force(on: bool = True):
    _ROUTE_FORCE[0] = bool(on)


ArithSwitch = collections.namedtuple("ArithSwitch", "key env setter getter what of report covers")
ARITH_SWITCHES = (
    ArithSwitch("conv", "FN2_CONV_ARITH", "set_conv_arithmetic", "conv_arithmetic", "conv", "convolution forward", "convolution forward",
                "split-bf16 on the direct 5x5 / 2 layers"),
    ArithSwitch("deconv", "FN2_DECONV_ARITH", "set_deconv_arithmetic", "deconv_arithmetic", "deconv", "deconvolution forward", "deconvolution forward",
                "split-bf16 in the GEMM of the 4x4 / 2 layers"),
    ArithSwitch("wino", "FN2_WINO_ARITH", "set_winograd_arithmetic", "winograd_arithmetic", "winograd", "Winograd 3x3 forward", "winograd forward",
                "split-bf16 on the 3x3 / 1 layers with Cout % 64 == 0"),
    ArithSwitch("corr", "FN2_CORR_ARITH", "set_correlation_arithmetic", "correlation_arithmetic", "correlation", "correlation forward", "correlation forward",
                "split-bf16 in the FlowNetC correlation (same fp64 bound as the exact kernel; measured times: profiles/corr_bf16x3_bench.md)"),
    ArithSwitch("dgrad", "FN2_DGRAD_ARITH", "set_conv_backward_arithmetic", "conv_backward_arithmetic", "conv backward", "convolution data gradient",
                "data-gradient", "split-bf16 on the 5x5 / 2 layers"),
    ArithSwitch("wgrad", "FN2_WGRAD_ARITH", "set_conv_weight_gradient_arithmetic", "conv_weight_gradient_arithmetic", "conv weight gradient",
                "convolution weight gradient", "weight-gradient", "split-bf16 on the 5x5 / 2 layers"),
)
_CONV_ARITHMETICS = ("fp32", "bf16x3")
_ARITH_SWITCH = {s.key: s for s in ARITH_SWITCHES}
_ARITH = {s.key: "fp32" for s in ARITH_SWITCHES}


def _set_arithmetic(key: str, name: str):
    if name not in _CONV_ARITHMETICS:
        raise ValueError("%s arithmetic must be one of %s, got %r" % (_ARITH_SWITCH[key].what, ", ".join(_CONV_ARITHMETICS), name))
    _ARITH[key] = name


def arithmetic(key: str) -> str:
    return _ARITH[key]


def _bf16x3(key: str) -> bool:
    return _ARITH[key] == "bf16x3"


for _s in ARITH_SWITCHES:
    if os.environ.get(_s.env):
        _set_arithmetic(_s.key, os.environ[_s.env])


def set_conv_arithmetic(name: str = "fp32"):
    _set_arithmetic("conv", name)


def conv_arithmetic() -> str:
    return arithmetic("conv")


def set_deconv_arithmetic(name: str = "fp32"):
    _set_arithmetic("deconv", name)


def deconv_arithmetic() -> str:
    return arithmetic("deconv")


def set_winograd_arithmetic(name: str = "fp32"):
    _set_arithmetic("wino", name)


def winograd_arithmetic() -> str:
    return arithmetic("wino")


get_winograd_arithmetic = winograd_arithmetic


def set_conv_backward_arithmetic(name: str):
    _set_arithmetic("dgrad", name)


def conv_backward_arithmetic() -> str:
    return arithmetic("dgrad")


def set_conv_weight_gradient_arithmetic(name: str):
    _set_arithmetic("wgrad", name)


def conv_weight_gradient_arithmetic() -> str:
# ... 367 lines not shown
```

flownet2_amd/graph_backend.py:

```python
from __future__ import annotations

import contextlib
import types

import torch.nn.functional as F

NEG_SLOPE = 0.1

_LISTENERS = []


@contextlib.contextmanager
def listening(fn):
    _LISTENERS.append(fn)
    try:
        yield fn
    finally:
        _LISTENERS.remove(fn)


def _declines(*args, **kwargs):
    return None


class GraphBackend:
    FORWARDED = ("correlation", "resample", "flow_warp", "channel_norm", "downsample", "l1_loss", "scale_shift", "resample_slices",
                 "flow_warp_slices", "channel_norm_slices", "l1_loss_multi", "downsample_ahead", "wait_ahead", "lpq_loss", "lpq_loss_multi")

    def __init__(self, obj):
        get = lambda name: getattr(obj, name, None)
        self.obj = obj
        for name in self.FORWARDED:
            if get(name) is not None:
                setattr(self, name, get(name))
        self.own_conv, self.own_deconv = get("conv_mfma_relu") or _declines, get("deconv_relu") or _declines
        self.own_correlation_relu_into = get("correlation_relu_into") or _declines
        self._predict, self._upsample = get("predict_flow_conv"), get("upsample_flow_deconv")
        self._bias_act = get("conv_bias_leaky_relu")
        self._conv2d = get("lib_conv2d") or (lambda x, w, b, s, p: F.conv2d(x, w, b, stride=s, padding=p))
        self._deconv2d = get("lib_conv_transpose2d") or (lambda x, w, b, s, p: F.conv_transpose2d(x, w, b, stride=s, padding=p))
        self._act = get("leaky_relu") or (lambda y, slope, name: F.leaky_relu(y, slope))
        self.conv_route_name, self.relu_chain_supported = get("conv_route_name"), get("relu_chain_supported")
        self.writes_slices = self.own_conv is not _declines
        self.fuses_correlation = self.own_correlation_relu_into is not _declines
        self.has_slices = get("resample_slices") is not None
        self.has_scale_shift = get("scale_shift") is not None
        self.trains_in_place = get("conv_backward") is not None
        self.has_stem_chain = self.trains_in_place and self.conv_route_name is not None and self.relu_chain_supported is not None
        self.has_multi_loss = get("l1_loss_multi") is not None
        self.has_multi_lpq_loss = get("lpq_loss_multi") is not None
        self.targets_ahead = get("downsample_ahead") is not None

    def __getattr__(self, name):
        if name in self.FORWARDED:
            return getattr(self.obj, name)
        raise AttributeError(name)

    def _ran(self, name, y, **info):
        for fn in list(_LISTENERS):
            fn(name, y, dict(info, backend=self))

    def wrote(self, kind, name, y, out, out_c0, channels, x, w=None, stride=1, pad=0):
        if _LISTENERS:
            self._ran(name, y if y.requires_grad else out[:, out_c0:out_c0 + channels], kind=kind, act=True, x=x, w=w, stride=stride, pad=pad,
                      own=True, into=True)

    def conv_wb(self, x, w, b, stride, pad, act=True, slope=NEG_SLOPE, name=None, relu_chain=None):
        y = self.own_conv(x, w, b, stride, pad, slope, act, relu_chain=relu_chain)
        own = y is not None
        if not own:
            if relu_chain is not None:
                raise RuntimeError("relu_chain: no own kernel takes this layer (its consumer was told the stem kernel would)")
            if act and self._bias_act is not None:
                y = self._bias_act(self._conv2d(x, w, None, stride, pad), b, slope)
            else:
                y = self._conv2d(x, w, b, stride, pad)
                if act:
                    y = self._act(y, slope, name)
        if _LISTENERS:
            self._ran(name, y, kind="conv", act=act, x=x, w=w, stride=stride, pad=pad, own=own, into=False)
        return y

    def conv(self, x, P, name, stride, pad, act=True, relu_chain=None):
        return self.conv_wb(x, P[name + ".w"], P[name + ".b"], stride, pad, act, NEG_SLOPE, name, relu_chain)

    def deconv_wb(self, x, w, b, act=True, slope=NEG_SLOPE, name=None):
        y = self.own_deconv(x, w, b, slope, act)
        own = y is not None
        if not own:
            if act and self._bias_act is not None:
                y = self._bias_act(self._deconv2d(x, w, None, 2, 1), b, slope)
            else:
                y = self._deconv2d(x, w, b, 2, 1)
                if act:
                    y = self._act(y, slope, name)
        if _LISTENERS:
            self._ran(name, y, kind="deconv", act=act, x=x, w=w, stride=2, pad=1, own=own, into=False)
        return y

    def deconv(self, x, P, name, act=True):
        return self.deconv_wb(x, P[name + ".w"], P[name + ".b"], act, NEG_SLOPE, name)

    def predict_flow(self, x, P, name):
        if self._predict is not None:
            return self._predict(x, P[name + ".w"], P[name + ".b"])
        return self.conv(x, P, name, 1, 1, act=False)

    def upsample_flow(self, x, P, name, out=None, out_c0=0):
        if self._upsample is None:
            return None if out is not None else self.deconv(x, P, name, act=False)
        if out is not None:
            return self._upsample(x, P[name + ".w"], P[name + ".b"], out=out, out_c0=out_c0)
        return self._upsample(x, P[name + ".w"], P[name + ".b"])

    def leaky_relu(self, x, name, slope=NEG_SLOPE):
        y = self._act(x, slope, name)
        if _LISTENERS:
            self._ran(name, y, kind="relu", act=True, x=x, own=False, into=False)
        return y


_MODULE_ADAPTERS = {}


def backend_of(obj) -> GraphBackend:
    if isinstance(obj, GraphBackend):
        return obj
    if obj is None or isinstance(obj, types.ModuleType):
        be = _MODULE_ADAPTERS.get(obj)
        if be is None:
            be = _MODULE_ADAPTERS[obj] = GraphBackend(obj)
        return be
    return GraphBackend(obj)
```

flownet2_amd/nets.py:

```python
from __future__ import annotations

import math
import os
from typing import Dict, Optional

import torch

from .graph_backend import NEG_SLOPE, GraphBackend, backend_of, listening

FLOW_SCALE = 20.0
SD_FLOW_SCALE = 0.05
LOSS_WEIGHTS = {6: 0.32, 5: 0.08, 4: 0.02, 3: 0.01, 2: 0.005}

_ENC_TAIL = [("conv4", 256, 512, 3, 2, 1), ("conv4_1", 512, 512, 3, 1, 1), ("conv5", 512, 512, 3, 2, 1),
             ("conv5_1", 512, 512, 3, 1, 1), ("conv6", 512, 1024, 3, 2, 1), ("conv6_1", 1024, 1024, 3, 1, 1)]
_DEC = [("Convolution1", "conv", 1024, 2), ("deconv5", "deconv", 1024, 512), ("upsample_flow6to5", "deconv", 2, 2),
        ("Convolution2", "conv", 1026, 2), ("deconv4", "deconv", 1026, 256), ("upsample_flow5to4", "deconv", 2, 2),
        ("Convolution3", "conv", 770, 2), ("deconv3", "deconv", 770, 128), ("upsample_flow4to3", "deconv", 2, 2),
        ("Convolution4", "conv", 386, 2), ("deconv2", "deconv", 386, 64), ("upsample_flow3to2", "deconv", 2, 2),
        ("Convolution5", "conv", 194, 2)]


def layer_table(kind: str = "C", in_channels: int = 6):
    t = []
    if kind == "C":
        t += [("conv1", "conv", 3, 64, 7, 2, 3), ("conv2", "conv", 64, 128, 5, 2, 2), ("conv3", "conv", 128, 256, 5, 2, 2),
              ("conv_redir", "conv", 256, 32, 1, 1, 0), ("conv3_1", "conv", 473, 256, 3, 1, 1)]
    else:
        t += [("conv1", "conv", in_channels, 64, 7, 2, 3), ("conv2", "conv", 64, 128, 5, 2, 2), ("conv3", "conv", 128, 256, 5, 2, 2),
              ("conv3_1", "conv", 256, 256, 3, 1, 1)]
    t += [(n, "conv", ci, co, k, s, p) for (n, ci, co, k, s, p) in _ENC_TAIL]
    for (n, k, ci, co) in _DEC:
        t.append((n, k, ci, co, 3, 1, 1) if k == "conv" else (n, k, ci, co, 4, 2, 1))
    return t


def init_params(kind: str = "C", seed: int = 0, device="cpu", in_channels: int = 6) -> Dict[str, torch.Tensor]:
    g = torch.Generator().manual_seed(seed)
    params = {}
    for (name, k, ci, co, ks, s, p) in layer_table(kind, in_channels):
        shape = (co, ci, ks, ks) if k == "conv" else (ci, co, ks, ks)
        fan_in = ci * ks * ks if k == "conv" else ci * ks * ks / (s * s)
        std = math.sqrt(2.0 / ((1 + NEG_SLOPE ** 2) * fan_in))
        if name.startswith("Convolution"):
            std *= 0.5
        if name.startswith("upsample_flow"):
            std = 0.25
        params[name + ".w"] = (torch.randn(shape, generator=g) * std).to(device)
        params[name + ".b"] = torch.zeros(co).to(device)
    return params


def num_params(params) -> int:
    return sum(int(v.numel()) for v in params.values())


def conv_forward(x, w, b, stride, pad, act, backend, slope=None, relu_chain=None):
    return backend_of(backend).conv_wb(x, w, b, stride, pad, act, NEG_SLOPE if slope is None else slope, relu_chain=relu_chain)


_LAST_ROUTE = [""]


def _note_route(name, y, info):
    if info["kind"] != "conv":
        return
    be, x, w = info["backend"], info["x"], info["w"]
    if not info["own"]:
        _LAST_ROUTE[0] = "library conv2d"
    elif be.conv_route_name is None:
        _LAST_ROUTE[0] = "own kernel"
    else:
        _LAST_ROUTE[0] = "fn2 %s" % be.conv_route_name(x.shape, w, info["stride"], info["pad"], info["act"], not info["into"])


def _trace_route(name, y, info):
    if info["kind"] == "conv":
        _note_route(name, y, info)
        print("conv route %-16s in %-22s k%d s%d act=%d -> %s%s" % (name, tuple(info["x"].shape), info["w"].shape[2], info["stride"], info["act"],
                                                                  _LAST_ROUTE[0], " (into its Concat blob)" if info["into"] else ""))


if os.environ.get("FN2_TRACE_CONV") == "1":
    listening(_trace_route).__enter__()


_CONSTS: Dict[tuple, torch.Tensor] = {}


def _const(device, values):
    key = (str(device), tuple(float(v) for v in values))
    if key not in _CONSTS:
        _CONSTS[key] = torch.tensor(key[1], device=device, dtype=torch.float32)
    return _CONSTS[key]


def deconv_forward(x, w, b, act=True, backend=None, slope=None):
    return backend_of(backend).deconv_wb(x, w, b, act, NEG_SLOPE if slope is None else slope)


def _conv_into_concat(x, P, name, stride, pad, extra_channels, be, relu_chain=None):
    w = P[name + ".w"]
    training = torch.is_grad_enabled() and (x.requires_grad or _any_requires_grad(P))
    if be.writes_slices and w.shape[2] in (3, 5) and (be.trains_in_place or not training):
        k = w.shape[2]
        ho, wo = (x.shape[2] + 2 * pad - k) // stride + 1, (x.shape[3] + 2 * pad - k) // stride + 1
        blob = torch.empty((x.shape[0], w.shape[0] + extra_channels, ho, wo), device=x.device, dtype=x.dtype)
        y = be.own_conv(x, w, P[name + ".b"], stride, pad, NEG_SLOPE, True, out=blob, out_c0=0, relu_chain=relu_chain)
        if y is not None:
            be.wrote("conv", name, y, blob, 0, w.shape[0], x, w, stride, pad)
            return blob, (y if (training and y.requires_grad) else blob[:, :w.shape[0]])
    if relu_chain is not None:
        raise RuntimeError("relu_chain: conv '%s' left the own-kernel route after its producer was told it would fold the ReLU derivative" % name)
    return None, be.conv(x, P, name, stride, pad)


def _any_requires_grad(P) -> bool:
    vals = P.P.values() if isinstance(P, _Prefixed) else P.values()
    return any(v.requires_grad for v in vals)


def _refine_stage(P, skip, x, dname, flow, uname, be):
    blob, s = skip if isinstance(skip, tuple) else (None, skip)
    if blob is None:
        return torch.cat([s, be.deconv(x, P, dname), be.upsample_flow(flow, P, uname)], 1)
    wd, bd = P[dname + ".w"], P[dname + ".b"]
    cs, cd = s.shape[1], wd.shape[1]
    assert blob.shape[1] == cs + cd + 2
    d = be.own_deconv(x, wd, bd, NEG_SLOPE, True, out=blob, out_c0=cs)
    if d is not None:
        be.wrote("deconv", dname, d, blob, cs, cd, x, wd, 2, 1)
    stage_params = [wd, bd, P[uname + ".w"], P[uname + ".b"]]
    if torch.is_grad_enabled() and (s.requires_grad or x.requires_grad or flow.requires_grad or any(p.requires_grad for p in stage_params)):
        u = be.upsample_flow(flow, P, uname, out=blob, out_c0=cs + cd) if d is not None else None
        if d is None or u is None:
            return torch.cat([s, be.deconv(x, P, dname), be.upsample_flow(flow, P, uname)], 1)
        part = lambda t, c0, c: t if t.requires_grad else blob[:, c0:c0 + c]
        return _ConcatInPlace.apply(blob, s, part(d, cs, cd), part(u, cs + cd, 2))
    if d is None:
        blob[:, cs:cs + cd].copy_(be.deconv(x, P, dname))
    if be.upsample_flow(flow, P, uname, out=blob, out_c0=cs + cd) is None:
        blob[:, cs + cd:].copy_(be.upsample_flow(flow, P, uname))
    return blob


def _decoder(P, conv6_1, conv5_1, conv4_1, conv3_1, conv2, be):
    flow6 = be.predict_flow(conv6_1, P, "Convolution1")
    c5 = _refine_stage(P, conv5_1, conv6_1, "deconv5", flow6, "upsample_flow6to5", be)
    flow5 = be.predict_flow(c5, P, "Convolution2")
    c4 = _refine_stage(P, conv4_1, c5, "deconv4", flow5, "upsample_flow5to4", be)
    flow4 = be.predict_flow(c4, P, "Convolution3")
    c3 = _refine_stage(P, conv3_1, c4, "deconv3", flow4, "upsample_flow4to3", be)
    flow3 = be.predict_flow(c3, P, "Convolution4")
    c2 = _refine_stage(P, conv2, c3, "deconv2", flow3, "upsample_flow3to2", be)
    flow2 = be.predict_flow(c2, P, "Convolution5")
    return {2: flow2, 3: flow3, 4: flow4, 5: flow5, 6: flow6}


def _skip_conv(x, P, name, stride, pad, dname, be, relu_chain=None):
    return _conv_into_concat(x, P, name, stride, pad, P[dname + ".w"].shape[1] + 2, be, relu_chain=relu_chain)


RELU_CHAIN = [True]


def _stem_chain(P, x, be):
    if not (RELU_CHAIN[0] and be.has_stem_chain and torch.is_grad_enabled() and x.is_cuda):
        return None, None
    w1, w2 = P["conv1.w"], P["conv2.w"]
    if not (w1.requires_grad and w2.requires_grad and P["conv1.b"].requires_grad) or x.requires_grad:
        return None, None
    if be.conv_route_name(x.shape, w1, 2, 3) != "stem":
        return None, None
    c1_shape = (x.shape[0], w1.shape[0], (x.shape[2] - 1) // 2 + 1, (x.shape[3] - 1) // 2 + 1)
    if not be.relu_chain_supported(c1_shape, w2, 2, 2):
        return None, None
    cell = {"masked": False, "slope": NEG_SLOPE}
    return (1, cell), (2, cell)


class _ConcatInPlace(torch.autograd.Function):

    @staticmethod
    def forward(ctx, blob, *parts):
        ctx.cuts = [p.shape[1] for p in parts]
        assert sum(ctx.cuts) == blob.shape[1] and all(p.data_ptr() >= blob.data_ptr() for p in parts)
        return blob.view_as(blob)

    @staticmethod
    def backward(ctx, g):
        out, c0 = [None], 0
        for c in ctx.cuts:
            out.append(g[:, c0:c0 + c])
            c0 += c
        return tuple(out)


class _SplitTowers(torch.autograd.Function):

    @staticmethod
    def forward(ctx, x):
        n = x.shape[0] // 2
        return x[:n], x[n:]

    @staticmethod
    def backward(ctx, ga, gb):
        return torch.cat([ga, gb], 0)


class _StackedAndFirstTower(torch.autograd.Function):

    @staticmethod
    def forward(ctx, x):
        return x.view_as(x), x[:x.shape[0] // 2]

    @staticmethod
    def backward(ctx, g_all, g_first):
        if g_all._base is not None or not g_all.is_contiguous():
            g_all = g_all.clone(memory_format=torch.contiguous_format)
        g_all[:g_first.shape[0]].add_(g_first)
        return g_all


_CORR = dict(pad=20, kernel_size=1, max_displacement=20, stride_1=1, stride_2=2)


def flownet_c_core(P, img0, img1, backend, towers=None):
    be = backend_of(backend)
    x = towers if towers is not None else torch.cat([img0, img1], 0)
    n = x.shape[0] // 2
    chain1, chain2 = _stem_chain(P, x, be)
    c1 = be.conv(x, P, "conv1", 2, 3, relu_chain=chain1)
    blob2, c2 = _skip_conv(c1, P, "conv2", 2, 2, "deconv2", be, relu_chain=chain2)
    training = torch.is_grad_enabled() and c2.requires_grad
    c2_first = None
    if training:
        c2, c2_first = _StackedAndFirstTower.apply(c2)
    c3 = be.conv(c2, P, "conv3", 2, 2)
    c3a, c3b = _SplitTowers.apply(c3) if (training and c3.requires_grad) else (c3[:n], c3[n:])
    wr, br = P["conv_redir.w"], P["conv_redir.b"]
    cr = wr.shape[0]
    cat = None
    if be.fuses_correlation:
        cat = torch.empty((n, cr + 441, c3a.shape[2], c3a.shape[3]), device=c3a.device, dtype=c3a.dtype)
        if be.trains_in_place and torch.is_grad_enabled() and (c3a.requires_grad or c3b.requires_grad):
            redir = be.own_conv(c3a, wr, br, 1, 0, NEG_SLOPE, True, out=cat, out_c0=0)
            if redir is not None:
                be.wrote("conv", "conv_redir", redir, cat, 0, cr, c3a, wr, 1, 0)
            corr = be.own_correlation_relu_into(c3a, c3b, cat, cr, NEG_SLOPE, training=True, **_CORR)
            be.wrote("relu", "relu", corr, cat, cr, 441, c3a)
            if redir is not None and redir.requires_grad:
                cat = _ConcatInPlace.apply(cat, redir, corr)
            else:
                cat = torch.cat([be.conv(c3a, P, "conv_redir", 1, 0), corr], 1)
        else:
            corr = be.own_correlation_relu_into(c3a, c3b, cat, cr, NEG_SLOPE, **_CORR)
            if corr is None:
                cat = None
            else:
                be.wrote("relu", "relu", corr, cat, cr, 441, c3a)
                redir = None
                if not (torch.is_grad_enabled() and _any_requires_grad(P)):
                    redir = be.own_conv(c3a, wr, br, 1, 0, NEG_SLOPE, True, out=cat, out_c0=0)
                if redir is None:
                    cat[:, :cr].copy_(be.conv(c3a, P, "conv_redir", 1, 0))
                else:
                    be.wrote("conv", "conv_redir", redir, cat, 0, cr, c3a, wr, 1, 0)
    if cat is None:
        redir = be.conv(c3a, P, "conv_redir", 1, 0)
        corr = be.correlation(c3a, c3b, **_CORR)
        cat = torch.cat([redir, be.leaky_relu(corr, "relu")], 1)
    blob3, c31 = _skip_conv(cat, P, "conv3_1", 1, 1, "deconv3", be)
    c4 = be.conv(c31, P, "conv4", 2, 1)
    blob4, c41 = _skip_conv(c4, P, "conv4_1", 1, 1, "deconv4", be)
    c5 = be.conv(c41, P, "conv5", 2, 1)
    blob5, c51 = _skip_conv(c5, P, "conv5_1", 1, 1, "deconv5", be)
    c6 = be.conv(c51, P, "conv6", 2, 1)
    c61 = be.conv(c6, P, "conv6_1", 1, 1)
    c2s = c2_first if c2_first is not None else c2[:n]
    skip2 = (blob2[:n], c2s) if blob2 is not None else c2s
    return _decoder(P, c61, (blob5, c51), (blob4, c41), (blob3, c31), skip2, be)


def flownet_s_core(P, x, backend=None):
    be = backend_of(backend)
    c1 = be.conv(x, P, "conv1", 2, 3)
    blob2, c2 = _skip_conv(c1, P, "conv2", 2, 2, "deconv2", be)
    c3 = be.conv(c2, P, "conv3", 2, 2)
    blob3, c31 = _skip_conv(c3, P, "conv3_1", 1, 1, "deconv3", be)
    c4 = be.conv(c31, P, "conv4", 2, 1)
    blob4, c41 = _skip_conv(c4, P, "conv4_1", 1, 1, "deconv4", be)
    c5 = be.conv(c41, P, "conv5", 2, 1)
    blob5, c51 = _skip_conv(c5, P, "conv5_1", 1, 1, "deconv5", be)
    c6 = be.conv(c51, P, "conv6", 2, 1)
    c61 = be.conv(c6, P, "conv6_1", 1, 1)
    return _decoder(P, c61, (blob5, c51), (blob4, c41), (blob3, c31), (blob2, c2), be)


def adapted_size(h: int, w: int, divisor: int = 64):
    return int(math.ceil(h / divisor) * divisor), int(math.ceil(w / divisor) * divisor)


def deploy_forward(kind: str, P, img0, img1, backend, mean: Optional[torch.Tensor] = None):
    backend = backend_of(backend)
    N, _, H, W = img0.shape
    ah, aw = adapted_size(H, W)
    neg_default = mean is None
    if mean is None:
        mean = _const(img0.device, (0.411, 0.433, 0.45))
    if (ah, aw) == (H, W) and img0.is_cuda and not torch.is_grad_enabled() and backend.has_scale_shift:
        neg_mean = _const(img0.device, (-0.411, -0.433, -0.45)) if neg_default else (-mean).contiguous()
        if kind == "C":
            x = torch.empty((2 * N, 3, H, W), device=img0.device, dtype=torch.float32)
            backend.scale_shift(img0, 1.0 / 255.0, neg_mean, out=x[:N])
            backend.scale_shift(img1, 1.0 / 255.0, neg_mean, out=x[N:])
            flows = flownet_c_core(P, None, None, backend, towers=x)
        else:
            x = torch.empty((N, 6, H, W), device=img0.device, dtype=torch.float32)
            backend.scale_shift(img0, 1.0 / 255.0, neg_mean, out=x, out_c0=0)
            backend.scale_shift(img1, 1.0 / 255.0, neg_mean, out=x, out_c0=3)
            flows = flownet_s_core(P, x, backend)
    else:
        pre = []
        for im in (img0, img1):
            x = im * (1.0 / 255.0)
            if (ah, aw) != (H, W):
                x = backend.resample(x, ah, aw)
            pre.append(x - mean.view(1, 3, 1, 1))
        if kind == "C":
            flows = flownet_c_core(P, pre[0], pre[1], backend)
        else:
            flows = flownet_s_core(P, torch.cat(pre, 1), backend)
    if img0.is_cuda and not torch.is_grad_enabled() and backend.has_slices:
        flow = backend.resample_slices(flows[2], H, W, in_scale=FLOW_SCALE)
        if (ah, aw) == (H, W):
            return flow
    else:
        flow = flows[2] * FLOW_SCALE
        flow = backend.resample(flow, H, W)
    scale = _const(flow.device, (W / float(aw), H / float(ah)))
    return flow * scale.view(1, 2, 1, 1)


def loss_targets_ahead(gt_flow, backend, divisors=None):
    backend = backend_of(backend)
    if not (backend.targets_ahead and gt_flow.is_cuda):
        return None
    H, W = gt_flow.shape[2], gt_flow.shape[3]
    divisors = divisors or {s: 2 ** s for s in LOSS_WEIGHTS}
    gt = gt_flow * (1.0 / FLOW_SCALE)
    sizes = [(H // divisors[s], W // divisors[s]) for s in LOSS_WEIGHTS]
    tgts, ev = backend.downsample_ahead(gt, sizes)
    return {"targets": dict(zip(LOSS_WEIGHTS, tgts)), "event": ev, "sizes": dict(zip(LOSS_WEIGHTS, sizes))}


FINAL_FLOW_GT_SCALE = {"SD": 1.0 / SD_FLOW_SCALE, "fusion": 1.0}


def _lpq_kwargs(loss):
    if not (isinstance(loss, (tuple, list)) and 3 <= len(loss) <= 5 and loss[0] == "lpq"):
        raise ValueError('loss: None or ("lpq", p, q[, p_epsilon[, q_epsilon]]), got %r' % (loss,))
    p_eps, q_eps = (tuple(loss[3:]) + (0.0, 1e-2)[len(loss) - 3:])
    return dict(p=float(loss[1]), q=float(loss[2]), p_epsilon=float(p_eps), q_epsilon=float(q_eps), normalize_by_num_entries=True)


def final_flow_loss(flow, gt_flow, backend, scale, loss=None):
    backend = backend_of(backend)
    tgt = backend.downsample(gt_flow * scale, flow.shape[2], flow.shape[3])
    if loss is not None:
        return backend.lpq_loss(flow, tgt, **_lpq_kwargs(loss))
    return backend.l1_loss(flow, tgt, l2_per_location=True, normalize_by_num_entries=True)


def multiscale_loss(flows, gt_flow, backend, targets=None, loss=None):
    backend = backend_of(backend)
    lpq = _lpq_kwargs(loss) if loss is not None else None
    if (backend.has_multi_loss if lpq is None else backend.has_multi_lpq_loss) and gt_flow.is_cuda:
        scales = list(LOSS_WEIGHTS.items())
        preds = [flows[s] for s, _ in scales]
        if targets is not None and all(tuple(targets["sizes"][s]) == tuple(flows[s].shape[2:]) for s, _ in scales):
            backend.wait_ahead(targets["event"])
            tgts = [targets["targets"][s] for s, _ in scales]
        else:
            gt = gt_flow * (1.0 / FLOW_SCALE)
            tgts = [backend.downsample(gt, p.shape[2], p.shape[3]) for p in preds]
        if lpq is not None:
            return backend.lpq_loss_multi(preds, tgts, [w for _, w in scales], **lpq)[0]
        return backend.l1_loss_multi(preds, tgts, [w for _, w in scales], l2_per_location=True, normalize_by_num_entries=True)[0]
    gt = gt_flow * (1.0 / FLOW_SCALE)
    total = 0.0
    for s, w in LOSS_WEIGHTS.items():
        pred = flows[s]
        tgt = backend.downsample(gt, pred.shape[2], pred.shape[3])
        if lpq is not None:
            total = total + w * backend.lpq_loss(pred, tgt, **lpq)
        else:
            total = total + w * backend.l1_loss(pred, tgt, l2_per_location=True, normalize_by_num_entries=True)
    return total


def conv_flops(kind: str, h: int, w: int, in_channels: int = 6) -> float:
    fl = 0.0
    size = {}
    hh, ww = h, w
    res = {"conv1": 2, "conv2": 4, "conv3": 8, "conv_redir": 8, "conv3_1": 8, "conv4": 16, "conv4_1": 16, "conv5": 32, "conv5_1": 32,
           "conv6": 64, "conv6_1": 64, "Convolution1": 64, "deconv5": 32, "upsample_flow6to5": 32, "Convolution2": 32,
           "deconv4": 16, "upsample_flow5to4": 16, "Convolution3": 16, "deconv3": 8, "upsample_flow4to3": 8, "Convolution4": 8,
           "deconv2": 4, "upsample_flow3to2": 4, "Convolution5": 4}
    for (name, k, ci, co, ks, s, p) in layer_table(kind, in_channels):
        oh, ow = hh // res[name], ww // res[name]
        macs = oh * ow * co * ci * ks * ks if k == "conv" else (oh // 2) * (ow // 2) * ci * co * ks * ks
        mult = 2 if (kind == "C" and name in ("conv1", "conv2", "conv3")) else 1
        fl += 2.0 * macs * mult
    return fl


_SD_TABLE = [("conv0", "conv", 6, 64, 3, 1, 1), ("conv1", "conv", 64, 64, 3, 2, 1), ("conv1_1", "conv", 64, 128, 3, 1, 1),
             ("conv2", "conv", 128, 128, 3, 2, 1), ("conv2_1", "conv", 128, 128, 3, 1, 1), ("conv3", "conv", 128, 256, 3, 2, 1),
             ("conv3_1", "conv", 256, 256, 3, 1, 1), ("conv4", "conv", 256, 512, 3, 2, 1), ("conv4_1", "conv", 512, 512, 3, 1, 1),
             ("conv5", "conv", 512, 512, 3, 2, 1), ("conv5_1", "conv", 512, 512, 3, 1, 1), ("conv6", "conv", 512, 1024, 3, 2, 1),
             ("conv6_1", "conv", 1024, 1024, 3, 1, 1),
             ("Convolution1", "conv", 1024, 2, 3, 1, 1), ("deconv5", "deconv", 1024, 512, 4, 2, 1), ("upsample_flow6to5", "deconv", 2, 2, 4, 2, 1),
             ("interconv5", "conv", 1026, 512, 3, 1, 1), ("Convolution2", "conv", 512, 2, 3, 1, 1),
             ("deconv4", "deconv", 1026, 256, 4, 2, 1), ("upsample_flow5to4", "deconv", 2, 2, 4, 2, 1),
             ("interconv4", "conv", 770, 256, 3, 1, 1), ("Convolution3", "conv", 256, 2, 3, 1, 1),
             ("deconv3", "deconv", 770, 128, 4, 2, 1), ("upsample_flow4to3", "deconv", 2, 2, 4, 2, 1),
             ("interconv3", "conv", 386, 128, 3, 1, 1), ("Convolution4", "conv", 128, 2, 3, 1, 1),
             ("deconv2", "deconv", 386, 64, 4, 2, 1), ("upsample_flow3to2", "deconv", 2, 2, 4, 2, 1),
             ("interconv2", "conv", 194, 64, 3, 1, 1), ("Convolution5", "conv", 64, 2, 3, 1, 1)]
_FUSE_TABLE = [("conv0", "conv", 11, 64, 3, 1, 1), ("conv1", "conv", 64, 64, 3, 2, 1), ("conv1_1", "conv", 64, 128, 3, 1, 1),
               ("conv2", "conv", 128, 128, 3, 2, 1), ("conv2_1", "conv", 128, 128, 3, 1, 1),
               ("Convolution5", "conv", 128, 2, 3, 1, 1), ("deconv1", "deconv", 128, 32, 4, 2, 1), ("upsample_flow2to1", "deconv", 2, 2, 4, 2, 1),
               ("interconv1", "conv", 162, 32, 3, 1, 1), ("Convolution6", "conv", 32, 2, 3, 1, 1),
               ("deconv0", "deconv", 162, 16, 4, 2, 1), ("upsample_flow1to0", "deconv", 2, 2, 4, 2, 1),
               ("interconv0", "conv", 82, 16, 3, 1, 1), ("Convolution7", "conv", 16, 2, 3, 1, 1)]


_SD_RES = {"conv0": 1, "conv1": 2, "conv1_1": 2, "conv2": 4, "conv2_1": 4, "conv3": 8, "conv3_1": 8, "conv4": 16, "conv4_1": 16, "conv5": 32,
           "conv5_1": 32, "conv6": 64, "conv6_1": 64, "Convolution1": 64, "deconv5": 32, "upsample_flow6to5": 32, "interconv5": 32,
           "Convolution2": 32, "deconv4": 16, "upsample_flow5to4": 16, "interconv4": 16, "Convolution3": 16, "deconv3": 8,
           "upsample_flow4to3": 8, "interconv3": 8, "Convolution4": 8, "deconv2": 4, "upsample_flow3to2": 4, "interconv2": 4, "Convolution5": 4}
_FUSE_RES = {"conv0": 1, "conv1": 2, "conv1_1": 2, "conv2": 4, "conv2_1": 4, "Convolution5": 4, "deconv1": 2, "upsample_flow2to1": 2,
             "interconv1": 2, "Convolution6": 2, "deconv0": 1, "upsample_flow1to0": 1, "interconv0": 1, "Convolution7": 1}


def _table_flops(table, res, h, w):
    fl = 0.0
    for (name, k, ci, co, ks, s, p) in table:
        oh, ow = h // res[name], w // res[name]
        fl += 2.0 * (oh * ow * co * ci * ks * ks if k == "conv" else (oh // 2) * (ow // 2) * ci * co * ks * ks)
    return fl


def flownet2_conv_flops(h: int, w: int) -> float:
    return conv_flops("C", h, w) + 2 * conv_flops("S", h, w, 12) + _table_flops(_SD_TABLE, _SD_RES, h, w) + _table_flops(_FUSE_TABLE, _FUSE_RES, h, w)


def _init_table(table, prefix, g, params, device):
    for (name, k, ci, co, ks, s, p) in table:
        shape = (co, ci, ks, ks) if k == "conv" else (ci, co, ks, ks)
        fan_in = ci * ks * ks if k == "conv" else ci * ks * ks / (s * s)
        std = math.sqrt(2.0 / ((1 + NEG_SLOPE ** 2) * fan_in))
        if name.startswith("Convolution"):
            std *= 0.5
        if name.startswith("upsample_flow"):
            std = 0.25
        params[prefix + name + ".w"] = (torch.randn(shape, generator=g) * std).to(device)
        params[prefix + name + ".b"] = torch.zeros(co).to(device)


def init_params_flownet2(seed: int = 0, device="cpu") -> Dict[str, torch.Tensor]:
    g = torch.Generator().manual_seed(seed)
    P: Dict[str, torch.Tensor] = {}
    _init_table(layer_table("C"), "", g, P, device)
    _init_table(layer_table("S", 12), "net2_", g, P, device)
    _init_table(layer_table("S", 12), "net3_", g, P, device)
    _init_table(_SD_TABLE, "netsd_", g, P, device)
    _init_table(_FUSE_TABLE, "fuse_", g, P, device)
    return P


class _Prefixed(dict):

    def __init__(self, P, prefix):
        super().__init__()
        self.P, self.prefix = P, prefix

    def __getitem__(self, k):
        return self.P[self.prefix + k]


def flownet_sd_core(P, x, backend):
    be = backend_of(backend)
    c0 = be.conv(x, P, "conv0", 1, 1)
    c1 = be.conv(be.conv(c0, P, "conv1", 2, 1), P, "conv1_1", 1, 1)
    blob2, c2 = _conv_into_concat(be.conv(c1, P, "conv2", 2, 1), P, "conv2_1", 1, 1, 64 + 2, be)
    blob3, c3 = _conv_into_concat(be.conv(c2, P, "conv3", 2, 1), P, "conv3_1", 1, 1, 128 + 2, be)
    blob4, c4 = _skip_conv(be.conv(c3, P, "conv4", 2, 1), P, "conv4_1", 1, 1, "deconv4", be)
    blob5, c5 = _skip_conv(be.conv(c4, P, "conv5", 2, 1), P, "conv5_1", 1, 1, "deconv5", be)
    c6 = be.conv(be.conv(c5, P, "conv6", 2, 1), P, "conv6_1", 1, 1)
    flow6 = be.predict_flow(c6, P, "Convolution1")
    cat5 = _refine_stage(P, (blob5, c5), c6, "deconv5", flow6, "upsample_flow6to5", be)
    flow5 = be.predict_flow(be.conv(cat5, P, "interconv5", 1, 1, act=False), P, "Convolution2")
    cat4 = _refine_stage(P, (blob4, c4), cat5, "deconv4", flow5, "upsample_flow5to4", be)
    flow4 = be.predict_flow(be.conv(cat4, P, "interconv4", 1, 1, act=False), P, "Convolution3")
    cat3 = _refine_stage(P, (blob3, c3), cat4, "deconv3", flow4, "upsample_flow4to3", be)
    flow3 = be.predict_flow(be.conv(cat3, P, "interconv3", 1, 1, act=False), P, "Convolution4")
    cat2 = _refine_stage(P, (blob2, c2), cat3, "deconv2", flow3, "upsample_flow3to2", be)
    return be.predict_flow(be.conv(cat2, P, "interconv2", 1, 1, act=False), P, "Convolution5")


def fusion_core(P, x, backend):
    be = backend_of(backend)
    blob0, c0 = _conv_into_concat(x, P, "conv0", 1, 1, 16 + 2, be)
    blob1, c1 = _conv_into_concat(be.conv(c0, P, "conv1", 2, 1), P, "conv1_1", 1, 1, 32 + 2, be)
    c2 = be.conv(be.conv(c1, P, "conv2", 2, 1), P, "conv2_1", 1, 1)
    flow2 = be.predict_flow(c2, P, "Convolution5")
    cat1 = _refine_stage(P, (blob1, c1), c2, "deconv1", flow2, "upsample_flow2to1", be)
    flow1 = be.predict_flow(be.conv(cat1, P, "interconv1", 1, 1, act=False), P, "Convolution6")
    cat0 = _refine_stage(P, (blob0, c0), cat1, "deconv0", flow1, "upsample_flow1to0", be)
    return be.predict_flow(be.conv(cat0, P, "interconv0", 1, 1, act=False), P, "Convolution7")


def flownet2_deploy_forward(P, img0, img1, backend, mean: Optional[torch.Tensor] = None):
    backend = backend_of(backend)
    N, _, H, W = img0.shape
    ah, aw = adapted_size(H, W)
    neg_mean = _const(img0.device, (-0.411, -0.433, -0.45)) if mean is None else (-mean).contiguous()
    if mean is None:
        mean = _const(img0.device, (0.411, 0.433, 0.45))
    if img0.is_cuda and not torch.is_grad_enabled() and backend.has_slices:
        return _flownet2_pick_streams(P, img0, img1, backend, neg_mean)
    if (ah, aw) == (H, W) and img0.is_cuda and not torch.is_grad_enabled() and backend.has_scale_shift:
        a = backend.scale_shift(img0, 1.0 / 255.0, neg_mean)
        b = backend.scale_shift(img1, 1.0 / 255.0, neg_mean)
    else:
        a = backend.resample(img0 * (1.0 / 255.0), ah, aw) - mean.view(1, 3, 1, 1)
        b = backend.resample(img1 * (1.0 / 255.0), ah, aw) - mean.view(1, 3, 1, 1)

    def refine_input(flow_q):
        flow = backend.resample(flow_q * FLOW_SCALE, ah, aw)
        warped = backend.flow_warp(b, flow)
        err = backend.channel_norm(a - warped)
        return flow, warped, err

    flow1_q = flownet_c_core(P, a, b, backend)[2]
    f1, w1, e1 = refine_input(flow1_q)
    flow2_q = flownet_s_core(_Prefixed(P, "net2_"), torch.cat([a, b, w1, f1 * (1.0 / FLOW_SCALE), e1], 1), backend)[2]
    f2, w2, e2 = refine_input(flow2_q)
    flow3_q = flownet_s_core(_Prefixed(P, "net3_"), torch.cat([a, b, w2, f2 * (1.0 / FLOW_SCALE), e2], 1), backend)[2]
    flow_css = backend.resample(flow3_q * FLOW_SCALE, ah, aw, type=1)
    flow_sd = backend.resample(flownet_sd_core(_Prefixed(P, "netsd_"), torch.cat([a, b], 1), backend) * SD_FLOW_SCALE, ah, aw, type=1)
    err_css = backend.channel_norm(a - backend.flow_warp(b, flow_css))
    err_sd = backend.channel_norm(a - backend.flow_warp(b, flow_sd))
    fuse_in = torch.cat([a, flow_sd, flow_css, backend.channel_norm(flow_sd), backend.channel_norm(flow_css), err_sd, err_css], 1)
    flow = fusion_core(_Prefixed(P, "fuse_"), fuse_in, backend)
    flow = backend.resample(flow, H, W)
    scale = _const(flow.device, (W / float(aw), H / float(ah)))
    return flow * scale.view(1, 2, 1, 1)


_SD_STREAM = {"mode": "auto", "streams": {}, "picked": {}}


def set_sd_side_stream(mode="auto"):
    _SD_STREAM["mode"] = {True: "on", False: "off"}.get(mode, mode)
    _SD_STREAM["picked"] = {}


def _flownet2_pick_streams(P, img0, img1, backend, neg_mean):
    import time
    mode = _SD_STREAM["mode"]
    run = lambda side: _flownet2_deploy_forward_slices(P, img0, img1, backend, neg_mean, side)
    if mode != "auto":
        return run(mode == "on")
    key = (img0.device, tuple(img0.shape))
    st = _SD_STREAM["picked"].get(key)
    if isinstance(st, bool):
        return run(st)
    if torch.cuda.is_current_stream_capturing():
        return run(True)
    if st is None:
        st = _SD_STREAM["picked"][key] = {"n": 0, True: [], False: []}
    n = st["n"]
    st["n"] += 1
    if n == 0:
        return run(True)
    side = n % 2 == 1
    torch.cuda.synchronize(img0.device)
    t0 = time.perf_counter()
    out = run(side)
    torch.cuda.synchronize(img0.device)
    st[side].append(time.perf_counter() - t0)
    if n >= 4:
        _SD_STREAM["picked"][key] = min(st[True]) <= 1.01 * min(st[False])
        _SD_STREAM.setdefault("timings_ms", {})[key] = {"second_stream": round(min(st[True]) * 1e3, 4), "one_stream": round(min(st[False]) * 1e3, 4)}
    return out


def sd_side_stream_timings():
    return dict(_SD_STREAM.get("timings_ms", {}))


def sd_side_stream_picks():
    return {k: v for k, v in _SD_STREAM["picked"].items() if isinstance(v, bool)}


def _sd_side_stream(dev, on):
    if not on:
        return None
    st = _SD_STREAM["streams"].get(dev)
    if st is None:
        st = _SD_STREAM["streams"][dev] = torch.cuda.Stream(device=dev)
    return st


def _flownet2_deploy_forward_slices(P, img0, img1, backend, neg_mean, sd_beside=True):
    N, _, H, W = img0.shape
    ah, aw = adapted_size(H, W)
    dev = img0.device
    new = lambda c: torch.empty((N, c, ah, aw), device=dev, dtype=torch.float32)
    towers = torch.empty((2 * N, 3, ah, aw), device=dev, dtype=torch.float32)
    blob = new(12)
    pair = new(6)
    fuse = new(11)
    for k, img in enumerate((img0, img1)):
        if (ah, aw) == (H, W):
            src, s = img, 1.0 / 255.0
        else:
            src, s = backend.resample_slices(img, ah, aw, in_scale=1.0 / 255.0), 1.0
        backend.scale_shift(src, s, neg_mean, out=towers[k * N:(k + 1) * N])
        backend.scale_shift(src, s, neg_mean, out=blob, out_c0=3 * k)
        backend.scale_shift(src, s, neg_mean, out=pair, out_c0=3 * k)
        if k == 0:
            backend.scale_shift(src, s, neg_mean, out=fuse, out_c0=0)
    A, B, WARPED = (blob, 0, 3), (blob, 3, 3), (blob, 6, 3)

    def refine_input(flow_q):
        flow = backend.resample_slices(flow_q, ah, aw, in_scale=FLOW_SCALE, out2=(blob, 9, 2), out2_scale=1.0 / FLOW_SCALE)
        backend.flow_warp_slices(B, flow, out=WARPED)
        backend.channel_norm_slices(A, minus=WARPED, out=(blob, 11, 1))

    side = _sd_side_stream(dev, sd_beside)
    sd_q = None
    if side is not None:
        main = torch.cuda.current_stream(dev)
        side.wait_stream(main)
        with torch.cuda.stream(side):
            sd_q = flownet_sd_core(_Prefixed(P, "netsd_"), pair, backend)
    flow1_q = flownet_c_core(P, None, None, backend, towers=towers)[2]
    refine_input(flow1_q)
    flow2_q = flownet_s_core(_Prefixed(P, "net2_"), blob, backend)[2]
    refine_input(flow2_q)
    flow3_q = flownet_s_core(_Prefixed(P, "net3_"), blob, backend)[2]
    if side is not None:
        main.wait_stream(side)
        sd_q.record_stream(main)
    else:
        sd_q = flownet_sd_core(_Prefixed(P, "netsd_"), pair, backend)
    backend.resample_slices(sd_q, ah, aw, type=1, in_scale=SD_FLOW_SCALE, out=(fuse, 3, 2))
    backend.resample_slices(flow3_q, ah, aw, type=1, in_scale=FLOW_SCALE, out=(fuse, 5, 2))
    backend.channel_norm_slices((fuse, 3, 2), out=(fuse, 7, 1))
    backend.channel_norm_slices((fuse, 5, 2), out=(fuse, 8, 1))
    backend.flow_warp_slices(B, (fuse, 3, 2), out=WARPED)
    backend.channel_norm_slices(A, minus=WARPED, out=(fuse, 9, 1))
    backend.flow_warp_slices(B, (fuse, 5, 2), out=WARPED)
    backend.channel_norm_slices(A, minus=WARPED, out=(fuse, 10, 1))
    flow = fusion_core(_Prefixed(P, "fuse_"), fuse, backend)
    if (ah, aw) == (H, W):
        return flow
    flow = backend.resample(flow, H, W)
    scale = _const(flow.device, (W / float(aw), H / float(ah)))
    return flow * scale.view(1, 2, 1, 1)
# ... 1 lines not shown
```

flownet2_amd/ops.py:

```python
from __future__ import annotations

import ctypes as C

import torch

from . import _lib
from ._lib import CorrParams, L1LossParams, check


def _consts(*names):
    return tuple(_lib.CONSTANTS["FN2_" + n] for n in names)


MULTIPLY, SUBTRACT = _consts("CORR_MULTIPLY", "CORR_SUBTRACT")
FILL_ZERO, FILL_NAN = _consts("FILL_ZERO", "FILL_NAN")
NEAREST, LINEAR, CUBIC, AREA = _consts("RESAMPLE_NEAREST", "RESAMPLE_LINEAR", "RESAMPLE_CUBIC", "RESAMPLE_AREA")


def _stream():
    return C.c_void_p(torch.cuda.current_stream().cuda_stream)


def _chk(t: torch.Tensor, name: str, ndim: int = 4):
    if not isinstance(t, torch.Tensor) or not t.is_cuda:
# ... 329 lines not shown
        if b1 is not None and b1.shape != b0.shape:
            raise ValueError("LpqLoss: bottom blobs must have the same shape")
    shapes = (C.c_int * (4 * n))(*[int(d) for b in b0s for d in b.shape])
    return _ptr_array(b0s), _ptr_array(b1s), shapes, (C.c_float * n)(*[float(w) for w in weights]), b0s, b1s


def _ptr_array(tensors):
    return (C.c_void_p * len(tensors))(*[t.data_ptr() if t is not None else None for t in tensors])


def lpq_loss_forward_multi(params, bottoms0, bottoms1, weights):
    n = len(bottoms0)
    dev = bottoms0[0].device
    _, ws_bytes, sync_bytes = lpq_loss_sizes(n)
    ws = torch.empty(ws_bytes, dtype=torch.uint8, device=dev)
    key = (dev.index, int(torch.cuda.current_stream().cuda_stream))
    sync = _LPQ_SYNC.get(key)
    if sync is None:
        sync = _LPQ_SYNC[key] = torch.zeros(sync_bytes, dtype=torch.uint8, device=dev)
    losses = torch.empty((n,), device=dev, dtype=torch.float32)
    total = torch.empty((), device=dev, dtype=torch.float32)
    p0, p1, shapes, lw, _b0s, _b1s = _lpq_scales(bottoms0, bottoms1, weights)
    check(_lib.lib().fn2_lpq_loss_forward_multi(n, p0, p1, shapes, lw, *params, _ptr(losses), _ptr(total), _ptr(ws), ws.numel(), _ptr(sync),
                                                _stream()))
    return total, losses, ws


def lpq_loss_backward_multi(params, bottoms0, bottoms1, weights, total_diff, workspace, need1=False):
    n = len(bottoms0)
    p0, p1, shapes, lw, b0s, b1s = _lpq_scales(bottoms0, bottoms1, weights)
    d0 = [torch.empty_like(b) for b in b0s]
    d1 = [torch.empty_like(b) if (need1 and b1s[k] is not None) else None for k, b in enumerate(b0s)]
    td = _chk(total_diff.reshape(1), "total_diff", ndim=1) if total_diff is not None else None
    check(_lib.lib().fn2_lpq_loss_backward_multi(n, p0, p1, _ptr_array(d0), _ptr_array(d1), shapes, lw, *params, _ptr(td), _ptr(workspace),
                                                 workspace.numel(), _stream()))
    return d0, d1


_FLOW_METRICS_K = _lib.FLOW_METRICS_CONSTANTS["FN2_FLOW_METRICS_K"]


def flow_metrics_sizes(N: int, H: int, W: int):
    nbytes, k = C.c_size_t(), C.c_int()
    check(_lib.lib().fn2_flow_metrics_sizes(int(N), int(H), int(W), C.byref(nbytes), C.byref(k)))
    return nbytes.value, k.value


def flow_metrics(pred, gt, valid=None, occ=None, outlier=(3.0, 0.05), bands=(10.0, 40.0), epe_map=False):
    p, g = _chk(pred, "pred"), _chk(gt, "gt")
    if p.shape != g.shape or p.shape[1] != 2:
        raise ValueError(f"flow_metrics: pred {tuple(p.shape)} and gt {tuple(g.shape)} must both be [N,2,H,W]")
    N, _, H, W = p.shape
    v, o = _chk_opt(valid, "valid"), _chk_opt(occ, "occ")
    for name, m in (("valid", v), ("occ", o)):
        if m is not None and tuple(m.shape) != (N, 1, H, W):
            raise ValueError(f"flow_metrics: {name} {tuple(m.shape)} must be [{N},1,{H},{W}]")
    ws = torch.empty(flow_metrics_sizes(N, H, W)[0], dtype=torch.uint8, device=p.device)
    results = torch.empty((N + 1, _FLOW_METRICS_K), dtype=torch.float64, device=p.device)
    emap = torch.empty((N, 1, H, W), dtype=torch.float32, device=p.device) if epe_map else None
    check(_lib.lib().fn2_flow_metrics(_ptr(p), _ptr(g), _ptr(v), _ptr(o), N, H, W, C.c_float(float(outlier[0])), C.c_float(float(outlier[1])),
                                      C.c_float(float(bands[0])), C.c_float(float(bands[1])), _ptr(results), _ptr(emap), _ptr(ws), ws.numel(),
                                      _stream()))
    return results, emap


def channel_norm_forward(x):
    x = _chk(x, "bottom[0]")
    N, Cc, H, W = x.shape
    out = torch.empty((N, 1, H, W), device=x.device, dtype=torch.float32)
    check(_lib.lib().fn2_channel_norm_forward(_ptr(x), _ptr(out), N, Cc, H, W, _stream()))
    return out


def channel_norm_forward_slices(x, minus=None, out=None):
    b, bctot, bc0, Cc = _as_slice(x, "bottom[0]")
    N, _, H, W = b.shape
    m, mctot, mc0 = None, 0, 0
    if minus is not None:
        m, mctot, mc0, Cm = _as_slice(minus, "bottom[1]")
        if Cm != Cc or tuple(m.shape[2:]) != (H, W) or m.shape[0] != N:
            raise ValueError("channel_norm: the subtrahend does not match the bottom")
    if out is None:
        out = torch.empty((N, 1, H, W), device=b.device, dtype=torch.float32)
    top, tctot, tc0, Ct = _as_slice(out, "top[0]")
    if Ct != 1 or top.shape[0] != N or tuple(top.shape[2:]) != (H, W):
        raise ValueError("channel_norm: top slice must be one channel of the bottom's size")
    check(_lib.lib().fn2_channel_norm_forward_slices(_ptr(b), bctot, bc0, _ptr(m), mctot, mc0, _ptr(top), tctot, tc0, N, Cc, H, W, _stream()))
    return top


def channel_norm_backward(x, top, top_diff):
    x, top, td = _chk(x, "bottom[0]"), _chk(top, "top"), _chk(top_diff, "top.diff")
    N, Cc, H, W = x.shape
    d = torch.empty_like(x)
    check(_lib.lib().fn2_channel_norm_backward(_ptr(x), _ptr(top), _ptr(td), _ptr(d), N, Cc, H, W, _stream()))
    return d


def downsample_forward(x, top_height, top_width):
    x = _chk(x, "bottom[0]")
    N, Cc, H, W = x.shape
    if top_height < 1 or top_width < 1:
        raise ValueError("DownsampleLayer must have top_height > 0 and top_width > 0")
    out = torch.empty((N, Cc, int(top_height), int(top_width)), device=x.device, dtype=torch.float32)
    check(_lib.lib().fn2_downsample_forward(_ptr(x), _ptr(out), N, Cc, H, W, int(top_height), int(top_width), _stream()))
    return out


def downsample_forward_multi(x, sizes):
    x = _chk(x, "bottom[0]")
    N, Cc, H, W = x.shape
    sizes = [(int(h), int(w)) for h, w in sizes]
    outs = [torch.empty((N, Cc, h, w), device=x.device, dtype=torch.float32) for h, w in sizes]
    n = len(sizes)
    ptrs = (C.c_void_p * n)(*[_ptr(o) for o in outs])
    hs, ws = (C.c_int * n)(*[h for h, _ in sizes]), (C.c_int * n)(*[w for _, w in sizes])
    check(_lib.lib().fn2_downsample_forward_multi(_ptr(x), ptrs, hs, ws, n, N, Cc, H, W, _stream()))
    return outs


def downsample_multi_supported(x_shape, sizes) -> bool:
    H, W = int(x_shape[2]), int(x_shape[3])
    return 1 <= len(sizes) <= 8 and all(int(h) >= 2 and int(w) >= 2 and (int(h), int(w)) != (H, W) for h, w in sizes)


def predict_flow_conv_forward(x, weight, bias=None):
    x, w = _chk(x, "bottom[0]"), _chk(weight, "weight")
    N, Cc, H, W = x.shape
    if tuple(w.shape) != (2, Cc, 3, 3):
        raise ValueError(f"predict_flow weight must be [2,{Cc},3,3], got {tuple(w.shape)}")
    b = _chk(bias, "bias", ndim=1) if bias is not None else None
    out = torch.empty((N, 2, H, W), device=x.device, dtype=torch.float32)
    nbytes = _lib.lib().fn2_predict_flow_conv_workspace_bytes(N, Cc, H, W)
    ws = torch.empty(nbytes, dtype=torch.uint8, device=x.device) if nbytes else None
    check(_lib.lib().fn2_predict_flow_conv_forward(_ptr(x), _ptr(w), _ptr(b), _ptr(out), N, Cc, H, W, _ptr(ws), nbytes, _stream()))
    return out


def upsample_flow_deconv_forward(x, weight, bias=None, out=None, out_c0=0):
    x, w = _chk(x, "bottom[0]"), _chk(weight, "weight")
    N, Cc, H, W = x.shape
    if Cc != 2 or tuple(w.shape) != (2, 2, 4, 4):
        raise ValueError("upsample_flow expects a 2-channel flow and a [2,2,4,4] weight")
    b = _chk(bias, "bias", ndim=1) if bias is not None else None
    if out is not None:
        _chk(out, "top[0]")
        if out.shape[0] != N or tuple(out.shape[2:]) != (2 * H, 2 * W):
            raise ValueError(f"upsample_flow: top blob {tuple(out.shape)} does not match [{N},*,{2 * H},{2 * W}]")
        check(_lib.lib().fn2_upsample_flow_deconv_forward_into(_ptr(x), _ptr(w), _ptr(b), _ptr(out), N, H, W, out.shape[1], int(out_c0), _stream()))
        return out[:, out_c0:out_c0 + 2]
    out = torch.empty((N, 2, 2 * H, 2 * W), device=x.device, dtype=torch.float32)
    check(_lib.lib().fn2_upsample_flow_deconv_forward(_ptr(x), _ptr(w), _ptr(b), _ptr(out), N, H, W, _stream()))
    return out


def bias_leaky_relu_(x, bias=None, negative_slope=0.1):
    if not (isinstance(x, torch.Tensor) and x.is_cuda and x.dtype == torch.float32 and x.dim() == 4 and x.is_contiguous()):
        raise ValueError("bias_leaky_relu_: expected a contiguous float32 CUDA (HIP) NCHW tensor")
    N, Cc, H, W = x.shape
    b = _chk_opt(bias, "bias", 1)
    if b is not None and b.numel() != Cc:
        raise ValueError(f"bias must have {Cc} entries, got {b.numel()}")
    check(_lib.lib().fn2_bias_leaky_relu_forward(_ptr(x), _ptr(b), N, Cc, H, W, C.c_float(float(negative_slope)), _stream()))
    return x


def scale_shift_forward(x, scale, shift=None, out=None, out_c0=0):
    x = _chk(x, "bottom[0]")
    N, Cc, H, W = x.shape
    if out is None:
        out = torch.empty_like(x)
    else:
        _chk(out, "top[0]")
        if out.shape[0] != N or tuple(out.shape[2:]) != (H, W):
            raise ValueError("scale_shift: top blob does not match the bottom")
    s = _chk_opt(shift, "shift", 1)
    check(_lib.lib().fn2_scale_shift_forward(_ptr(x), _ptr(out), _ptr(s), N, Cc, H, W, out.shape[1], out_c0, C.c_float(float(scale)), _stream()))
    return out


def predict_flow_conv_backward_supported(N, C, H, W) -> bool:
    return bool(_lib.lib().fn2_predict_flow_conv_backward_supported(int(N), int(C), int(H), int(W)))


def predict_flow_conv_backward(x, weight, top_diff, need_x=True, need_w=True, need_b=True):
    xb, xctot, xc0, Cc = _as_slice(x, "bottom[0]")
    w, g = _chk(weight, "weight"), _chk(top_diff, "top.diff")
    N, _, H, W = xb.shape
    if tuple(w.shape) != (2, Cc, 3, 3) or tuple(g.shape) != (N, 2, H, W):
        raise ValueError("predict_flow_conv_backward: weight must be [2,C,3,3] and top_diff [N,2,H,W]")
    dx = torch.empty((N, Cc, H, W), device=g.device, dtype=torch.float32) if need_x else None
    dw = torch.empty_like(w) if need_w else None
    db = torch.empty(2, device=g.device, dtype=torch.float32) if need_b else None
    nbytes = _lib.lib().fn2_predict_flow_conv_backward_workspace_bytes(N, Cc, H, W) if (need_w or need_b) else 0
    ws = torch.empty(max(nbytes, 4), dtype=torch.uint8, device=g.device)
    check(_lib.lib().fn2_predict_flow_conv_backward(_ptr(xb), xctot, xc0, _ptr(w), _ptr(g), _ptr(dx), _ptr(dw), _ptr(db), N, Cc, H, W, 0,
                                                    _ptr(ws), nbytes, _stream()))
    return dx, dw, db


def upsample_flow_deconv_backward(x, weight, top_diff, need_x=True, need_w=True, need_b=True):
    x, w, g = _chk(x, "bottom[0]"), _chk(weight, "weight"), _chk(top_diff, "top.diff")
    N, Cc, H, W = x.shape
    if Cc != 2 or tuple(w.shape) != (2, 2, 4, 4) or tuple(g.shape) != (N, 2, 2 * H, 2 * W):
        raise ValueError("upsample_flow_deconv_backward: bottom [N,2,H,W], weight [2,2,4,4], top_diff [N,2,2H,2W]")
    dx = torch.empty_like(x) if need_x else None
    dw = torch.empty_like(w) if need_w else None
    db = torch.empty(2, device=g.device, dtype=torch.float32) if need_b else None
    nbytes = _lib.lib().fn2_upsample_flow_deconv_backward_workspace_bytes(N, H, W) if (need_w or need_b) else 0
    ws = torch.empty(max(nbytes, 4), dtype=torch.uint8, device=g.device)
    check(_lib.lib().fn2_upsample_flow_deconv_backward(_ptr(x), _ptr(w), _ptr(g), _ptr(dx), _ptr(dw), _ptr(db), N, H, W, 0, _ptr(ws), nbytes, _stream()))
    return dx, dw, db


def conv_k7s2_relu_supported(Cin, Hin, Win, Cout) -> bool:
    return bool(_lib.lib().fn2_conv_k7s2_relu_supported(int(Cin), int(Hin), int(Win), int(Cout)))


def conv_k7s2_wgrad_supported(N, Cin, Hin, Win, Cout) -> bool:
    return bool(_lib.lib().fn2_conv_k7s2_wgrad_supported(int(N), int(Cin), int(Hin), int(Win), int(Cout)))


def conv_k7s2_wgrad_ksplit(N, Cin, Hin, Win, Cout) -> int:
    return int(_lib.lib().fn2_conv_k7s2_wgrad_ksplit(int(N), int(Cin), int(Hin), int(Win), int(Cout)))


def conv_k7s2_wgrad(top_diff, bottom):
    d, x = _chk(top_diff, "top.diff"), _chk(bottom, "bottom[0]")
    N, Cin, H, W = x.shape
    Cout = d.shape[1]
    if tuple(d.shape) != (N, Cout, (H - 1) // 2 + 1, (W - 1) // 2 + 1):
        raise ValueError(f"conv_k7s2_wgrad: top_diff {tuple(d.shape)} does not belong to a bottom of {tuple(x.shape)}")
    dw = torch.empty((Cout, Cin, 7, 7), device=x.device, dtype=torch.float32)
    ws, need = _scratch(x.device, _lib.lib().fn2_conv_k7s2_wgrad_workspace_bytes(N, Cin, H, W, Cout))
    check(_lib.lib().fn2_conv_k7s2_wgrad(_ptr(d), _ptr(x), _ptr(dw), N, Cin, H, W, Cout, 0, _ptr(ws), need, _stream()))
    return dw


def conv_k7s2_relu_forward(x, weight, bias=None, negative_slope=0.1):
    x, w = _chk(x, "bottom[0]"), _chk(weight, "weight")
    N, Cin, H, W = x.shape
    Cout = w.shape[0]
    if tuple(w.shape) != (Cout, Cin, 7, 7):
        raise ValueError(f"stem weight must be [Cout,{Cin},7,7], got {tuple(w.shape)}")
    b = _chk_opt(bias, "bias", 1)
    out = torch.empty((N, Cout, (H - 1) // 2 + 1, (W - 1) // 2 + 1), device=x.device, dtype=torch.float32)
    check(_lib.lib().fn2_conv_k7s2_relu_forward(_ptr(x), _ptr(w), _ptr(b), _ptr(out), N, Cin, H, W, Cout,
                                                C.c_float(float(negative_slope)), _stream()))
    return out


CONV_ROUTE_NONE, CONV_ROUTE_DIRECT, CONV_ROUTE_WINOGRAD, CONV_ROUTE_PLANE, CONV_ROUTE_STEM, CONV_ROUTE_HEAD = _consts(
    "CONV_ROUTE_NONE", "CONV_ROUTE_DIRECT", "CONV_ROUTE_WINOGRAD", "CONV_ROUTE_PLANE", "CONV_ROUTE_STEM", "CONV_ROUTE_HEAD")
DECONV_ROUTE_NONE, DECONV_ROUTE_GEMM, DECONV_ROUTE_PLANE, DECONV_ROUTE_HEAD = _consts("DECONV_ROUTE_NONE", "DECONV_ROUTE_GEMM", "DECONV_ROUTE_PLANE",
                                                                                      "DECONV_ROUTE_HEAD")
ROUTE_FORCE, ROUTE_BF16X3, ROUTE_WINO_BF16X3 = _consts("ROUTE_FORCE", "ROUTE_BF16X3", "ROUTE_WINO_BF16X3")
CONV_ARITH_BF16X3, = _consts("CONV_ARITH_BF16X3")
CONV_FWD_ROUTES = {0: None, 1: "direct", 2: "wino", 3: "plane", 4: "stem", 5: "head"}
DECONV_FWD_ROUTES = {0: None, 1: "gemm", 2: "plane", 3: "head"}
CONV_ROUTES = {0: None, 1: "direct", 2: "wino", 3: "plane", 4: None, 5: None}
DECONV_ROUTES = {0: None, 1: "gemm", 2: "plane", 3: None}


def conv_route(N, Cin, Hin, Win, Cout, kernel, stride, pad, force=False):
    return CONV_ROUTES[conv_forward_route(conv_desc(N, Cin, Hin, Win, Cout, kernel, stride, pad), force)]


def deconv_route(N, Cin, Hin, Win, Cout, kernel=4, stride=2, pad=1):
    return DECONV_ROUTES[deconv_forward_route(conv_desc(N, Cin, Hin, Win, Cout, kernel, stride, pad))]


BWD_ROUTES = {0: None, 1: "wino", 2: "tconv", 3: "plane", 4: "direct", 5: "deconv_plane"}


def conv_desc(N, Cin, Hin, Win, Cout, kernel, stride, pad):
    return _lib.ConvDesc(int(N), int(Cin), int(Hin), int(Win), int(Cout), int(kernel), int(stride), int(pad))


def conv_forward_route(desc, force=False, bf16x3=False, wino_bf16x3=False) -> int:
    flags = (ROUTE_FORCE if force else 0) | (ROUTE_BF16X3 if bf16x3 else 0) | (ROUTE_WINO_BF16X3 if wino_bf16x3 else 0)
    return int(_lib.lib().fn2_conv_route(C.byref(desc), flags))


def deconv_forward_route(desc, bf16x3=False) -> int:
    return int(_lib.lib().fn2_deconv_route(C.byref(desc), ROUTE_BF16X3 if bf16x3 else 0))


def conv_pack_weights(weight, desc, route, transposed=False):
    w = _chk(weight, "weight")
    L = _lib.lib()
    floats, pack = (L.fn2_deconv_packed_weight_floats, L.fn2_deconv_pack_weights) if transposed else (L.fn2_conv_packed_weight_floats, L.fn2_conv_pack_weights)
    n = int(floats(C.byref(desc), int(route)))
    k = desc.kernel
    if n == 0 or tuple(w.shape) != ((desc.Cin, desc.Cout, k, k) if transposed else (desc.Cout, desc.Cin, k, k)):
        raise ValueError("conv_pack_weights: route %d has no operand for a weight of shape %s" % (route, tuple(w.shape)))
    packed = torch.empty(n, device=w.device, dtype=torch.float32)
    check(pack(C.byref(desc), int(route), _ptr(w), _ptr(packed), _stream()))
    return packed


def conv_forward(x, packed, bias, desc, route, transposed=False, relu=True, negative_slope=0.1, out=None, out_c0=0, in_c0=0):
    x = _chk(x, "bottom[0]")
    N, Ctot, H, W = x.shape
    k, s, p = desc.kernel, desc.stride, desc.pad
    if (N, H, W) != (desc.N, desc.Hin, desc.Win) or in_c0 < 0 or in_c0 + desc.Cin > Ctot:
        raise ValueError(f"conv_forward: bottom blob {tuple(x.shape)} does not hold the layer's [{desc.N},{desc.Cin},{desc.Hin},{desc.Win}] at channel {in_c0}")
# ... 804 lines not shown
```

Before: 3586.

## Fuse flow-head tap gather with flow upsample and final resample, pair input normalization

```diff
diff --git a/flownet2_amd/_lib.py b/flownet2_amd/_lib.py
--- a/flownet2_amd/_lib.py
+++ b/flownet2_amd/_lib.py
@@ -101,6 +101,9 @@
 (EXPORTS, SOLVER_EXPORTS, CORR_ROUTE_EXPORTS, CONV_GENERAL_EXPORTS, CONV_GEOMETRY_EXPORTS, CONV_VOLUME_EXPORTS, LPQ_LOSS_EXPORTS,
  FLOW_METRICS_EXPORTS) = (list(f) for f in _PER_HEADER)
 PROTOTYPES = {name: proto for f in _PER_HEADER for name, proto in f.items()}
+with open(os.path.join(INCLUDE_DIR, "flownet2_hip_decoder_fusion.h")) as _f:
+    DECODER_FUSION_PROTOTYPES = parse_header(_f.read(), _STRUCTS)[0]
+DECODER_FUSION_EXPORTS = list(DECODER_FUSION_PROTOTYPES)
 globals().update({cls.__name__: cls for cls in _STRUCTS.values()})
 _HOOKS = parse_header("""
     int fn2_debug_set_correlation_impl(int impl);
@@ -120,7 +123,7 @@
             f"{SO_PATH} not found: the HIP extension is not built. Run `python -m flownet2_amd.build` "
             "(or __graft_entry__.build()). flownet2_amd has no CPU / PyTorch fallback.")
     L = C.CDLL(SO_PATH)
-    for table, required in ((PROTOTYPES, True), (_HOOKS, False)):
+    for table, required in ((PROTOTYPES, True), (DECODER_FUSION_PROTOTYPES, True), (_HOOKS, False)):
         for name, (restype, argtypes) in table.items():
             if not hasattr(L, name):
                 if required:
diff --git a/flownet2_amd/csrc/bias_act.hip b/flownet2_amd/csrc/bias_act.hip
--- a/flownet2_amd/csrc/bias_act.hip
+++ b/flownet2_amd/csrc/bias_act.hip
@@ -1,4 +1,5 @@
 #include "fn2_common.hpp"
+#include "../../include/flownet2_hip_decoder_fusion.h"
 
 namespace fn2 {
 
@@ -261,6 +262,58 @@
     }
   }
 }
+
+template <bool VEC4>
+__global__ void __launch_bounds__(256) scale_shift_pair(const float* __restrict__ in0, float* __restrict__ out0, int out0_c0,
+                                                        const float* __restrict__ in1, float* __restrict__ out1, int out1_c0,
+                                                        const float* __restrict__ shift, int C, unsigned hw, int out_ctot, float scale) {
+  const bool second = blockIdx.z != 0;
+  const float* in = second ? in1 : in0;
+  float* out = second ? out1 : out0;
+  const int out_c0 = second ? out1_c0 : out0_c0;
+  const unsigned plane = blockIdx.y;
+  const unsigned n = plane / (unsigned)C, c = plane % (unsigned)C;
+  const float sh = shift ? shift[c] : 0.f;
+  const float* p = in + (size_t)plane * hw;
+  float* q = out + ((size_t)n * out_ctot + out_c0 + c) * hw;
+  if constexpr (VEC4) {
+    const unsigned n4 = hw / 4;
+    for (unsigned i = blockIdx.x * blockDim.x + threadIdx.x; i < n4; i += gridDim.x * blockDim.x) {
+      f32x4 v = reinterpret_cast<const f32x4*>(p)[i];
+#pragma unroll
+      for (int j = 0; j < 4; ++j) {
+        float prod = v[j] * scale;
+        asm volatile("" : "+v"(prod));
+        v[j] = prod + sh;
+      }
+      reinterpret_cast<f32x4*>(q)[i] = v;
+    }
+  } else {
+    for (unsigned i = blockIdx.x * blockDim.x + threadIdx.x; i < hw; i += gridDim.x * blockDim.x) {
+      float prod = p[i] * scale;
+      asm volatile("" : "+v"(prod));
+      q[i] = prod + sh;
+    }
+  }
+}
+}
+
+FN2_API int fn2_scale_shift_forward_pair(const float* bottom0, float* top0, int top0_c0, const float* bottom1, float* top1, int top1_c0,
+                                         const float* shift, int N, int C, int H, int W, int top_channels, float scale, void* stream) {
+  if (N < 0 || C < 1 || H < 1 || W < 1) return fn2::fail(FN2_ERR_INVALID_ARG, "scale_shift_pair: bad shape [%d,%d,%d,%d]", N, C, H, W);
+  if (top0_c0 < 0 || top0_c0 + C > top_channels || top1_c0 < 0 || top1_c0 + C > top_channels)
+    return fn2::fail(FN2_ERR_INVALID_ARG, "scale_shift_pair: channel slice outside the blob");
+  if (N == 0) return FN2_OK;
+  if (!bottom0 || !top0 || !bottom1 || !top1) return fn2::fail(FN2_ERR_INVALID_ARG, "scale_shift_pair: NULL blob pointer");
+  if ((long long)N * C > 65535) return fn2::fail(FN2_ERR_UNSUPPORTED, "scale_shift_pair: too many planes");
+  const unsigned hw = (unsigned)H * (unsigned)W;
+  const uintptr_t all = reinterpret_cast<uintptr_t>(bottom0) | reinterpret_cast<uintptr_t>(top0) | reinterpret_cast<uintptr_t>(bottom1) | reinterpret_cast<uintptr_t>(top1);
+  const bool vec = hw % 4 == 0 && (all & 15) == 0;
+  if (vec) hipLaunchKernelGGL(fn2::scale_shift_pair<true>, dim3(fn2::blocks_for(hw / 4, 256, 256), (unsigned)(N * C), 2), dim3(256), 0, fn2::as_stream(stream),
+                              bottom0, top0, top0_c0, bottom1, top1, top1_c0, shift, C, hw, top_channels, scale);
+  else hipLaunchKernelGGL(fn2::scale_shift_pair<false>, dim3(fn2::blocks_for(hw, 256, 64), (unsigned)(N * C), 2), dim3(256), 0, fn2::as_stream(stream),
+                          bottom0, top0, top0_c0, bottom1, top1, top1_c0, shift, C, hw, top_channels, scale);
+  return fn2::check_launch("scale_shift_forward_pair");
 }
 
 FN2_API int fn2_scale_shift_forward(const float* bottom, float* top, const float* shift, int N, int C, int H, int W,
diff --git a/flownet2_amd/csrc/conv_mfma.hip b/flownet2_amd/csrc/conv_mfma.hip
--- a/flownet2_amd/csrc/conv_mfma.hip
+++ b/flownet2_amd/csrc/conv_mfma.hip
@@ -346,7 +346,8 @@
   FN2_CV_PIN(1, 1, 2, 7, 2, 2, 1, 8, 1, 1) FN2_CV_PIN(1, 1, 2, 3, 2, 2, 1, 8, 1, 1)
   FN2_CV_PIN(3, 1, 2, 7, 2, 2, 1, 2, 0, 1) FN2_CV_PIN(3, 1, 2, 6, 2, 2, 1, 2, 0, 1) FN2_CV_PIN(3, 2, 2, 7, 2, 1, 2, 2, 0, 1) FN2_CV_PIN(3, 2, 2, 6, 2, 2, 1, 2, 0, 1)
   FN2_CV_PIN(4, 2, 2, 7, 2, 2, 1, 2, 0, 1) FN2_CV_PIN(4, 2, 2, 6, 2, 2, 1, 2, 0, 1) FN2_CV_PIN(5, 2, 2, 6, 2, 2, 1, 1, 0, 1)
-  FN2_CV_PIN(7, 2, 2, 6, 2, 2, 1, 1, 0, 1) FN2_CV_PIN(7, 2, 4, 6, 1, 2, 2, 1, 0, 0)};
+  FN2_CV_PIN(7, 2, 2, 6, 2, 2, 1, 1, 0, 1) FN2_CV_PIN(7, 2, 4, 6, 1, 2, 2, 1, 0, 0)
+  FN2_CV_ROW16(2, 1, 1, 4, 1, 0)};
 constexpr int kNumVariants = sizeof(kVariants) / sizeof(kVariants[0]);
 
 int g_forced_variant = -1;
diff --git a/flownet2_amd/csrc/flow_gather.hpp b/flownet2_amd/csrc/flow_gather.hpp
--- /dev/null
+++ b/flownet2_amd/csrc/flow_gather.hpp
@@ -0,0 +1,44 @@
+#pragma once
+#include "fn2_common.hpp"
+
+namespace fn2 {
+
+template <int NSPLIT>
+__device__ __forceinline__ float gather_flow_value(const float* __restrict__ P, const float* __restrict__ bias, int N, int H, int W,
+                                                   unsigned n, unsigned o, int y, int x) {
+  const unsigned plane = (unsigned)H * W;
+  float v[NSPLIT][9];
+#pragma unroll
+  for (int sp = 0; sp < NSPLIT; ++sp) {
+    const float* Pn = P + (((size_t)sp * N + n) * 18 + o * 9) * plane;
+#pragma unroll
+    for (int dy = 0; dy < 3; ++dy)
+#pragma unroll
+      for (int dx = 0; dx < 3; ++dx) {
+        const int yy = y + dy - 1, xx = x + dx - 1;
+        const bool ok = yy >= 0 && yy < H && xx >= 0 && xx < W;
+        v[sp][dy * 3 + dx] = ok ? Pn[(size_t)(dy * 3 + dx) * plane + (unsigned)yy * W + xx] : 0.f;
+      }
+  }
+  float sacc = bias ? bias[o] : 0.f;
+#pragma unroll
+  for (int sp = 0; sp < NSPLIT; ++sp)
+#pragma unroll
+    for (int t = 0; t < 9; ++t) sacc += v[sp][t];
+  return sacc;
+}
+
+template <int NSPLIT, int TH, int TW, int R, int THREADS>
+__device__ __forceinline__ void gather_flow_tile(float* __restrict__ tile, const float* __restrict__ P, const float* __restrict__ bias,
+                                                 int N, int H, int W, unsigned n, int y0, int x0) {
+  constexpr int LH = TH + 2 * R, LW = TW + 2 * R;
+  for (int idx = threadIdx.x; idx < 2 * LH * LW; idx += THREADS) {
+    const int o = idx / (LH * LW), r = idx - o * (LH * LW);
+    const int ly = r / LW, lx = r - ly * LW;
+    const int y = y0 - R + ly, x = x0 - R + lx;
+    const bool in_image = y >= 0 && y < H && x >= 0 && x < W;
+    tile[idx] = in_image ? gather_flow_value<NSPLIT>(P, bias, N, H, W, n, (unsigned)o, y, x) : 0.f;
+  }
+}
+
+}
diff --git a/flownet2_amd/csrc/flow_head.hip b/flownet2_amd/csrc/flow_head.hip
--- a/flownet2_amd/csrc/flow_head.hip
+++ b/flownet2_amd/csrc/flow_head.hip
@@ -1,4 +1,6 @@
 #include "fn2_common.hpp"
+#include "flow_gather.hpp"
+#include "../../include/flownet2_hip_decoder_fusion.h"
 
 namespace fn2 {
 
@@ -106,6 +108,55 @@
 #pragma unroll
         for (int c = 0; c < 2; ++c) {
           const float v = in[(((size_t)n * 2 + c) * H + iy) * W + ix];
+          a0 = fmaf(w[((c * 2 + 0) * 4 + ky) * 4 + kx], v, a0);
+          a1 = fmaf(w[((c * 2 + 1) * 4 + ky) * 4 + kx], v, a1);
+        }
+      }
+    }
+    out[(((size_t)n * out_ctot + out_c0 + 0) * Ho + Y) * Wo + X] = a0;
+    out[(((size_t)n * out_ctot + out_c0 + 1) * Ho + Y) * Wo + X] = a1;
+  }
+}
+
+constexpr int kGuT = 16, kGuL = kGuT + 2;
+
+template <int NSPLIT>
+__global__ void __launch_bounds__(256) flow_gather_upsample(const float* __restrict__ P, const float* __restrict__ bias, float* __restrict__ flow,
+                                                            const float* __restrict__ w, const float* __restrict__ ubias, float* __restrict__ out,
+                                                            int N, int H, int W, int out_ctot, int out_c0) {
+  __shared__ float tile[2 * kGuL * kGuL];
+  const unsigned n = blockIdx.z;
+  const int y0 = blockIdx.y * kGuT, x0 = blockIdx.x * kGuT;
+  gather_flow_tile<NSPLIT, kGuT, kGuT, 1, 256>(tile, P, bias, N, H, W, n, y0, x0);
+  __syncthreads();
+  {
+    const int ty = threadIdx.x / kGuT, tx = threadIdx.x % kGuT;
+    const int y = y0 + ty, x = x0 + tx;
+    if (y < H && x < W) {
+#pragma unroll
+      for (int o = 0; o < 2; ++o) flow[(((size_t)n * 2 + o) * H + y) * W + x] = tile[(o * kGuL + ty + 1) * kGuL + tx + 1];
+    }
+  }
+  const int Ho = 2 * H, Wo = 2 * W;
+#pragma unroll
+  for (int k = 0; k < 4; ++k) {
+    const int lin = k * 256 + threadIdx.x;
+    const int Y = 2 * y0 + lin / (2 * kGuT), X = 2 * x0 + lin % (2 * kGuT);
+    if (Y >= Ho || X >= Wo) continue;
+    float a0 = ubias ? ubias[0] : 0.f, a1 = ubias ? ubias[1] : 0.f;
+#pragma unroll
+    for (int ty = 0; ty < 2; ++ty) {
+      const int ky = ((Y + 1) & 1) + 2 * ty;
+      const int iy = (Y + 1 - ky) / 2;
+      if (Y + 1 - ky < 0 || iy >= H) continue;
+#pragma unroll
+      for (int tx = 0; tx < 2; ++tx) {
+        const int kx = ((X + 1) & 1) + 2 * tx;
+        const int ix = (X + 1 - kx) / 2;
+        if (X + 1 - kx < 0 || ix >= W) continue;
+#pragma unroll
+        for (int c = 0; c < 2; ++c) {
+          const float v = tile[(c * kGuL + iy - y0 + 1) * kGuL + ix - x0 + 1];
           a0 = fmaf(w[((c * 2 + 0) * 4 + ky) * 4 + kx], v, a0);
           a1 = fmaf(w[((c * 2 + 1) * 4 + ky) * 4 + kx], v, a1);
         }
@@ -178,3 +229,41 @@
   hipLaunchKernelGGL(deconv4x4s2_c2, dim3(blocks_for(total, 256, 4096)), dim3(256), 0, as_stream(stream), in, weight, bias, top, N, H, W, top_channels, top_c0);
   return check_launch("upsample_flow_deconv_forward_into");
 }
+
+FN2_API int fn2_predict_flow_splits(int N, int C, int H, int W) {
+  if (N < 1 || C < 1 || H < 1 || W < 1) return 0;
+  return head_splits(N, C, H, W);
+}
+
+FN2_API int fn2_predict_flow_taps_forward(const float* in, const float* weight, float* P, size_t P_bytes, int N, int C, int H, int W, void* stream) {
+  if (N < 0 || C < 1 || H < 1 || W < 1) return fail(FN2_ERR_INVALID_ARG, "predict_flow_taps: bad shape [%d,%d,%d,%d]", N, C, H, W);
+  if (N == 0) return FN2_OK;
+  if (!in || !weight) return fail(FN2_ERR_INVALID_ARG, "predict_flow_taps: NULL blob pointer");
+  if ((long long)H * W >= (1ll << 31) || 2ll * N > 65535) return fail(FN2_ERR_UNSUPPORTED, "predict_flow_taps: blob too large");
+  const size_t need = fn2_predict_flow_conv_workspace_bytes(N, C, H, W);
+  if (!P || P_bytes < need) return fail(FN2_ERR_WORKSPACE, "predict_flow_taps: tap image too small (%zu < %zu)", P_bytes, need);
+  const long long total = (long long)N * H * W;
+  const unsigned blocks = (unsigned)((total + kHeadPix - 1) / kHeadPix);
+  const int nsplit = head_splits(N, C, H, W);
+  hipLaunchKernelGGL(conv3x3_c2_taps<kHeadG>, dim3(blocks, nsplit), dim3(kHeadPix * kHeadG), 0, as_stream(stream), in, weight, P, N, C, H, W, nsplit);
+  return check_launch("predict_flow_taps_forward");
+}
+
+FN2_API int fn2_flow_gather_upsample_forward(const float* P, int splits, const float* bias, float* flow, const float* up_weight, const float* up_bias,
+                                             float* top, int top_channels, int top_c0, int N, int H, int W, void* stream) {
+  if (N < 0 || H < 1 || W < 1) return fail(FN2_ERR_INVALID_ARG, "flow_gather_upsample: bad shape [%d,2,%d,%d]", N, H, W);
+  if (splits != 1 && splits != 2 && splits != 4 && splits != 8) return fail(FN2_ERR_INVALID_ARG, "flow_gather_upsample: %d channel splits", splits);
+  if (top_c0 < 0 || top_c0 + 2 > top_channels) return fail(FN2_ERR_INVALID_ARG, "flow_gather_upsample: channel slice outside the blob");
+  if (N == 0) return FN2_OK;
+  if (!P || !flow || !up_weight || !top) return fail(FN2_ERR_INVALID_ARG, "flow_gather_upsample: NULL blob pointer");
+  const dim3 grid((unsigned)((W + kGuT - 1) / kGuT), (unsigned)((H + kGuT - 1) / kGuT), (unsigned)N);
+  if ((long long)H * W >= (1ll << 29) || grid.y > 65535u || N > 65535) return fail(FN2_ERR_UNSUPPORTED, "flow_gather_upsample: blob too large");
+  hipStream_t st = as_stream(stream);
+  switch (splits) {
+    case 1: hipLaunchKernelGGL(flow_gather_upsample<1>, grid, dim3(256), 0, st, P, bias, flow, up_weight, up_bias, top, N, H, W, top_channels, top_c0); break;
+    case 2: hipLaunchKernelGGL(flow_gather_upsample<2>, grid, dim3(256), 0, st, P, bias, flow, up_weight, up_bias, top, N, H, W, top_channels, top_c0); break;
+    case 4: hipLaunchKernelGGL(flow_gather_upsample<4>, grid, dim3(256), 0, st, P, bias, flow, up_weight, up_bias, top, N, H, W, top_channels, top_c0); break;
+    default: hipLaunchKernelGGL(flow_gather_upsample<8>, grid, dim3(256), 0, st, P, bias, flow, up_weight, up_bias, top, N, H, W, top_channels, top_c0); break;
+  }
+  return check_launch("flow_gather_upsample_forward");
+}
diff --git a/flownet2_amd/csrc/resample.hip b/flownet2_amd/csrc/resample.hip
--- a/flownet2_amd/csrc/resample.hip
+++ b/flownet2_amd/csrc/resample.hip
@@ -1,4 +1,6 @@
 #include "fn2_common.hpp"
+#include "flow_gather.hpp"
+#include "../../include/flownet2_hip_decoder_fusion.h"
 
 #include <cmath>
 
@@ -383,6 +385,82 @@
         for (int qx = 0; qx < F; ++qx) o2[qx] = scaled(o[qx], a.out2_scale);
         *reinterpret_cast<vec_t*>(dst2 + (size_t)py * a.Wout) = o2;
       }
+    }
+  }
+}
+
+constexpr int kGrT = 16, kGrL = kGrT + 4;
+
+template <int NSPLIT>
+__global__ void __launch_bounds__(256) flow_gather_resample_up4(const float* __restrict__ P, const float* __restrict__ bias, float* __restrict__ out,
+                                                                int N, ResampleArgs a) {
+  constexpr int F = 4;
+  __shared__ float tile[2 * kGrL * kGrL];
+  const unsigned n = blockIdx.z;
+  const int y0 = blockIdx.y * kGrT, x0 = blockIdx.x * kGrT;
+  gather_flow_tile<NSPLIT, kGrT, kGrT, 2, 256>(tile, P, bias, N, a.Hin, a.Win, n, y0, x0);
+  __syncthreads();
+  const int li = threadIdx.x / kGrT, lj = threadIdx.x % kGrT;
+  const int i = y0 + li, j = x0 + lj;
+  if (i >= a.Hin || j >= a.Win) return;
+  const unsigned hw_out = (unsigned)a.Hout * a.Wout;
+  unsigned mx = 0u, my = 0u;
+#pragma unroll
+  for (int t = 0; t < 5; ++t) {
+    const int x = j - 2 + t, y = i - 2 + t;
+    mx |= ((x >= 0 && x < a.Win) ? 1u : 0u) << t;
+    my |= ((y >= 0 && y < a.Hin) ? 1u : 0u) << t;
+  }
+  float px[F][3], ky[F][3], wsum[F][F];
+#pragma unroll
+  for (int ph = 0; ph < F; ++ph) {
+    const float x_in = (F * j + ph) * a.fx + a.fy / 2.0f - 0.5f;
+    const float y_in = (F * i + ph) * a.fy + a.fx / 2.0f - 0.5f;
+#pragma unroll
+    for (int t = 0; t < 3; ++t) {
+      const int x = j - 1 + t, y = i - 1 + t;
+      px[ph][t] = ((mx >> (t + 1)) & 1u) ? a.ax * triangle_coeff(a.ax * (x_in - x)) * a.ay : 0.f;
+      ky[ph][t] = ((my >> (t + 1)) & 1u) ? triangle_coeff(a.ay * (y_in - y)) : 0.f;
+    }
+  }
+#pragma unroll
+  for (int py = 0; py < F; ++py)
+#pragma unroll
+    for (int qx = 0; qx < F; ++qx) {
+      float w = 0.f;
+#pragma unroll
+      for (int r = 0; r < 3; ++r)
+#pragma unroll
+        for (int t = 0; t < 3; ++t) w += px[qx][t] * ky[py][r];
+      wsum[py][qx] = w;
+    }
+  using vec_t = __attribute__((ext_vector_type(F))) float;
+#pragma unroll
+  for (int o = 0; o < 2; ++o) {
+    float v[3][3], poison = 0.f;
+#pragma unroll
+    for (int r = 0; r < 5; ++r)
+#pragma unroll
+      for (int t = 0; t < 5; ++t) {
+        const float s = scaled(tile[(o * kGrL + li + r) * kGrL + lj + t], a.in_scale);
+        if (r >= 1 && r <= 3 && t >= 1 && t <= 3) v[r - 1][t - 1] = s;
+        else poison = fmaf(0.f, s, poison);
+      }
+    float* dst = out + ((size_t)n * 2 + o) * hw_out + (size_t)(F * i) * a.Wout + F * j;
+#pragma unroll
+    for (int py = 0; py < F; ++py) {
+      vec_t ov;
+#pragma unroll
+      for (int qx = 0; qx < F; ++qx) {
+        float sum = poison;
+#pragma unroll
+        for (int r = 0; r < 3; ++r)
+#pragma unroll
+          for (int t = 0; t < 3; ++t) sum = fmaf(px[qx][t] * ky[py][r], v[r][t], sum);
+        const float ws = wsum[py][qx];
+        ov[qx] = (!ws) ? 0.f : (ws == 1.0f ? sum : sum / ws);
+      }
+      *reinterpret_cast<vec_t*>(dst + (size_t)py * a.Wout) = ov;
     }
   }
 }
@@ -462,6 +540,33 @@
   return check_launch("resample_forward");
 }
 
+FN2_API int fn2_flow_gather_resample_forward(const float* P, int splits, const float* bias, float in_scale, float* out, int N, int H, int W,
+                                             int Hout, int Wout, void* stream) {
+  if (N < 0 || H < 1 || W < 1) return fail(FN2_ERR_INVALID_ARG, "flow_gather_resample: bad shape [%d,2,%d,%d]", N, H, W);
+  if (splits != 1 && splits != 2 && splits != 4 && splits != 8) return fail(FN2_ERR_INVALID_ARG, "flow_gather_resample: %d channel splits", splits);
+  if (Hout != 4 * H || Wout != 4 * W) return fail(FN2_ERR_UNSUPPORTED, "flow_gather_resample: only the exact x4 up-sampling (%dx%d -> %dx%d asked)", H, W, Hout, Wout);
+  if (N == 0) return FN2_OK;
+  if (!P || !out) return fail(FN2_ERR_INVALID_ARG, "flow_gather_resample: NULL blob pointer");
+  if (reinterpret_cast<uintptr_t>(out) & 15) return fail(FN2_ERR_UNSUPPORTED, "flow_gather_resample: top blob not 16-byte aligned");
+  const dim3 grid((unsigned)((W + kGrT - 1) / kGrT), (unsigned)((H + kGrT - 1) / kGrT), (unsigned)N);
+  if ((long long)Hout * Wout >= (1ll << 29) || grid.y > 65535u || N > 65535) return fail(FN2_ERR_UNSUPPORTED, "flow_gather_resample: blob too large");
+  ResampleArgs a;
+  a.C = 2; a.octot = 2; a.oc0 = 0; a.o2ctot = 2; a.o2c0 = 0;
+  a.in_scale = in_scale; a.out2_scale = 1.0f;
+  a.NC = N * 2; a.Hin = H; a.Win = W; a.Hout = Hout; a.Wout = Wout;
+  a.fx = (float)W / (float)Wout;
+  a.fy = (float)H / (float)Hout;
+  a.ax = 1.0f; a.ay = 1.0f; a.rx = 2; a.ry = 2; a.ppt = 1;
+  hipStream_t st = as_stream(stream);
+  switch (splits) {
+    case 1: hipLaunchKernelGGL(flow_gather_resample_up4<1>, grid, dim3(256), 0, st, P, bias, out, N, a); break;
+    case 2: hipLaunchKernelGGL(flow_gather_resample_up4<2>, grid, dim3(256), 0, st, P, bias, out, N, a); break;
+    case 4: hipLaunchKernelGGL(flow_gather_resample_up4<4>, grid, dim3(256), 0, st, P, bias, out, N, a); break;
+    default: hipLaunchKernelGGL(flow_gather_resample_up4<8>, grid, dim3(256), 0, st, P, bias, out, N, a); break;
+  }
+  return check_launch("flow_gather_resample_forward");
+}
+
 FN2_API int fn2_resample_forward(const float* in, float* out, int N, int C, int Hin, int Win, int Hout, int Wout,
                                  int type, int antialias_param, void* stream) {
   return fn2_resample_forward_slices(in, 1.0f, out, C, 0, nullptr, 0, 0, 1.0f, N, C, Hin, Win, Hout, Wout, type, antialias_param, stream);
diff --git a/flownet2_amd/functional.py b/flownet2_amd/functional.py
--- a/flownet2_amd/functional.py
+++ b/flownet2_amd/functional.py
@@ -478,6 +478,38 @@
     if _needs_grad(x, weight, bias):
         return _UpsampleFlow.apply(x, weight, bias, None if out is None else (out, out_c0))
     return run(x, weight, bias)
+
+
+_DECODER_FUSION = [True]
+
+
+def set_decoder_fusion(on: bool = True):
+    _DECODER_FUSION[0] = bool(on)
+
+
+def decoder_fusion() -> bool:
+    return _DECODER_FUSION[0]
+
+
+def predict_flow_upsample(x, weight, bias, up_weight, up_bias, out, out_c0):
+    if not _DECODER_FUSION[0] or _needs_grad(x, weight, bias, up_weight, up_bias):
+        return None
+    P, _ = ops.predict_flow_taps_forward(x.contiguous(), weight.contiguous())
+    return ops.flow_gather_upsample_forward(P, bias, up_weight.contiguous(), up_bias, out, out_c0)
+
+
+def predict_flow_resample(x, weight, bias, height, width, in_scale=1.0):
+    if not _DECODER_FUSION[0] or _needs_grad(x, weight, bias) or (int(height), int(width)) != (4 * x.shape[2], 4 * x.shape[3]):
+        return None
+    P, _ = ops.predict_flow_taps_forward(x.contiguous(), weight.contiguous())
+    return ops.flow_gather_resample_forward(P, bias, height, width, in_scale)
+
+
+def scale_shift_pair(x0, x1, scale, shift, out0, out1, out0_c0=0, out1_c0=0):
+    if not _DECODER_FUSION[0]:
+        return None
+    with torch.no_grad():
+        return ops.scale_shift_forward_pair(x0.detach().contiguous(), x1.detach().contiguous(), scale, shift, out0, out1, out0_c0, out1_c0)
 
 
 class _BiasLeakyReLU(torch.autograd.Function):
diff --git a/flownet2_amd/graph_backend.py b/flownet2_amd/graph_backend.py
--- a/flownet2_amd/graph_backend.py
+++ b/flownet2_amd/graph_backend.py
@@ -36,6 +36,8 @@
         self.own_conv, self.own_deconv = get("conv_mfma_relu") or _declines, get("deconv_relu") or _declines
         self.own_correlation_relu_into = get("correlation_relu_into") or _declines
         self._predict, self._upsample = get("predict_flow_conv"), get("upsample_flow_deconv")
+        self._predict_upsample, self._predict_resample = get("predict_flow_upsample") or _declines, get("predict_flow_resample") or _declines
+        self.scale_shift_pair = get("scale_shift_pair") or _declines
         self._bias_act = get("conv_bias_leaky_relu")
         self._conv2d = get("lib_conv2d") or (lambda x, w, b, s, p: F.conv2d(x, w, b, stride=s, padding=p))
         self._deconv2d = get("lib_conv_transpose2d") or (lambda x, w, b, s, p: F.conv_transpose2d(x, w, b, stride=s, padding=p))
@@ -113,6 +115,12 @@
             return self._upsample(x, P[name + ".w"], P[name + ".b"], out=out, out_c0=out_c0)
         return self._upsample(x, P[name + ".w"], P[name + ".b"])
 
+    def predict_flow_upsample(self, x, P, name, uname, out, out_c0):
+        return self._predict_upsample(x, P[name + ".w"], P[name + ".b"], P[uname + ".w"], P[uname + ".b"], out, out_c0)
+
+    def predict_flow_resample(self, x, P, name, height, width, in_scale):
+        return self._predict_resample(x, P[name + ".w"], P[name + ".b"], height, width, in_scale)
+
     def leaky_relu(self, x, name, slope=NEG_SLOPE):
         y = self._act(x, slope, name)
         if _LISTENERS:
diff --git a/flownet2_amd/nets.py b/flownet2_amd/nets.py
--- a/flownet2_amd/nets.py
+++ b/flownet2_amd/nets.py
@@ -144,17 +144,37 @@
     return blob
 
 
-def _decoder(P, conv6_1, conv5_1, conv4_1, conv3_1, conv2, be):
-    flow6 = be.predict_flow(conv6_1, P, "Convolution1")
-    c5 = _refine_stage(P, conv5_1, conv6_1, "deconv5", flow6, "upsample_flow6to5", be)
-    flow5 = be.predict_flow(c5, P, "Convolution2")
-    c4 = _refine_stage(P, conv4_1, c5, "deconv4", flow5, "upsample_flow5to4", be)
-    flow4 = be.predict_flow(c4, P, "Convolution3")
-    c3 = _refine_stage(P, conv3_1, c4, "deconv3", flow4, "upsample_flow4to3", be)
-    flow3 = be.predict_flow(c3, P, "Convolution4")
-    c2 = _refine_stage(P, conv2, c3, "deconv2", flow3, "upsample_flow3to2", be)
-    flow2 = be.predict_flow(c2, P, "Convolution5")
-    return {2: flow2, 3: flow3, 4: flow4, 5: flow5, 6: flow6}
+def _head_and_stage(P, head_x, hname, skip, x, dname, uname, be):
+    blob, s = skip if isinstance(skip, tuple) else (None, skip)
+    if blob is not None and not torch.is_grad_enabled():
+        wd, bd = P[dname + ".w"], P[dname + ".b"]
+        cs, cd = s.shape[1], wd.shape[1]
+        assert blob.shape[1] == cs + cd + 2
+        flow = be.predict_flow_upsample(head_x, P, hname, uname, blob, cs + cd) if blob.is_contiguous() else None
+        if flow is not None:
+            d = be.own_deconv(x, wd, bd, NEG_SLOPE, True, out=blob, out_c0=cs)
+            if d is None:
+                blob[:, cs:cs + cd].copy_(be.deconv(x, P, dname))
+            else:
+                be.wrote("deconv", dname, d, blob, cs, cd, x, wd, 2, 1)
+            return flow, blob
+    flow = be.predict_flow(head_x, P, hname)
+    return flow, _refine_stage(P, skip, x, dname, flow, uname, be)
+
+
+def _decoder(P, conv6_1, conv5_1, conv4_1, conv3_1, conv2, be, final=None):
+    flow6, c5 = _head_and_stage(P, conv6_1, "Convolution1", conv5_1, conv6_1, "deconv5", "upsample_flow6to5", be)
+    flow5, c4 = _head_and_stage(P, c5, "Convolution2", conv4_1, c5, "deconv4", "upsample_flow5to4", be)
+    flow4, c3 = _head_and_stage(P, c4, "Convolution3", conv3_1, c4, "deconv3", "upsample_flow4to3", be)
+    flow3, c2 = _head_and_stage(P, c3, "Convolution4", conv2, c3, "deconv2", "upsample_flow3to2", be)
+    flows = {3: flow3, 4: flow4, 5: flow5, 6: flow6}
+    if final is not None and not torch.is_grad_enabled():
+        up = be.predict_flow_resample(c2, P, "Convolution5", final[0], final[1], final[2])
+        if up is not None:
+            flows["final"] = up
+            return flows
+    flows[2] = be.predict_flow(c2, P, "Convolution5")
+    return flows
 
 
 def _skip_conv(x, P, name, stride, pad, dname, be, relu_chain=None):
@@ -225,7 +245,7 @@
 _CORR = dict(pad=20, kernel_size=1, max_displacement=20, stride_1=1, stride_2=2)
 
 
-def flownet_c_core(P, img0, img1, backend, towers=None):
+def flownet_c_core(P, img0, img1, backend, towers=None, final=None):
     be = backend_of(backend)
     x = towers if towers is not None else torch.cat([img0, img1], 0)
     n = x.shape[0] // 2
@@ -279,10 +299,10 @@
     c61 = be.conv(c6, P, "conv6_1", 1, 1)
     c2s = c2_first if c2_first is not None else c2[:n]
     skip2 = (blob2[:n], c2s) if blob2 is not None else c2s
-    return _decoder(P, c61, (blob5, c51), (blob4, c41), (blob3, c31), skip2, be)
-
-
-def flownet_s_core(P, x, backend=None):
+    return _decoder(P, c61, (blob5, c51), (blob4, c41), (blob3, c31), skip2, be, final)
+
+
+def flownet_s_core(P, x, backend=None, final=None):
     be = backend_of(backend)
     c1 = be.conv(x, P, "conv1", 2, 3)
     blob2, c2 = _skip_conv(c1, P, "conv2", 2, 2, "deconv2", be)
@@ -294,7 +314,7 @@
     blob5, c51 = _skip_conv(c5, P, "conv5_1", 1, 1, "deconv5", be)
     c6 = be.conv(c51, P, "conv6", 2, 1)
     c61 = be.conv(c6, P, "conv6_1", 1, 1)
-    return _decoder(P, c61, (blob5, c51), (blob4, c41), (blob3, c31), (blob2, c2), be)
+    return _decoder(P, c61, (blob5, c51), (blob4, c41), (blob3, c31), (blob2, c2), be, final)
 
 
 def adapted_size(h: int, w: int, divisor: int = 64):
@@ -310,16 +330,21 @@
         mean = _const(img0.device, (0.411, 0.433, 0.45))
     if (ah, aw) == (H, W) and img0.is_cuda and not torch.is_grad_enabled() and backend.has_scale_shift:
         neg_mean = _const(img0.device, (-0.411, -0.433, -0.45)) if neg_default else (-mean).contiguous()
+        final = (H, W, FLOW_SCALE) if backend.has_slices else None
         if kind == "C":
             x = torch.empty((2 * N, 3, H, W), device=img0.device, dtype=torch.float32)
-            backend.scale_shift(img0, 1.0 / 255.0, neg_mean, out=x[:N])
-            backend.scale_shift(img1, 1.0 / 255.0, neg_mean, out=x[N:])
-            flows = flownet_c_core(P, None, None, backend, towers=x)
+            if backend.scale_shift_pair(img0, img1, 1.0 / 255.0, neg_mean, x[:N], x[N:]) is None:
+                backend.scale_shift(img0, 1.0 / 255.0, neg_mean, out=x[:N])
+                backend.scale_shift(img1, 1.0 / 255.0, neg_mean, out=x[N:])
+            flows = flownet_c_core(P, None, None, backend, towers=x, final=final)
         else:
             x = torch.empty((N, 6, H, W), device=img0.device, dtype=torch.float32)
-            backend.scale_shift(img0, 1.0 / 255.0, neg_mean, out=x, out_c0=0)
-            backend.scale_shift(img1, 1.0 / 255.0, neg_mean, out=x, out_c0=3)
-            flows = flownet_s_core(P, x, backend)
+            if backend.scale_shift_pair(img0, img1, 1.0 / 255.0, neg_mean, x, x, 0, 3) is None:
+                backend.scale_shift(img0, 1.0 / 255.0, neg_mean, out=x, out_c0=0)
+                backend.scale_shift(img1, 1.0 / 255.0, neg_mean, out=x, out_c0=3)
+            flows = flownet_s_core(P, x, backend, final=final)
+        if "final" in flows:
+            return flows["final"]
     else:
         pre = []
         for im in (img0, img1):
@@ -499,14 +524,10 @@
     blob4, c4 = _skip_conv(be.conv(c3, P, "conv4", 2, 1), P, "conv4_1", 1, 1, "deconv4", be)
     blob5, c5 = _skip_conv(be.conv(c4, P, "conv5", 2, 1), P, "conv5_1", 1, 1, "deconv5", be)
     c6 = be.conv(be.conv(c5, P, "conv6", 2, 1), P, "conv6_1", 1, 1)
-    flow6 = be.predict_flow(c6, P, "Convolution1")
-    cat5 = _refine_stage(P, (blob5, c5), c6, "deconv5", flow6, "upsample_flow6to5", be)
-    flow5 = be.predict_flow(be.conv(cat5, P, "interconv5", 1, 1, act=False), P, "Convolution2")
-    cat4 = _refine_stage(P, (blob4, c4), cat5, "deconv4", flow5, "upsample_flow5to4", be)
-    flow4 = be.predict_flow(be.conv(cat4, P, "interconv4", 1, 1, act=False), P, "Convolution3")
-    cat3 = _refine_stage(P, (blob3, c3), cat4, "deconv3", flow4, "upsample_flow4to3", be)
-    flow3 = be.predict_flow(be.conv(cat3, P, "interconv3", 1, 1, act=False), P, "Convolution4")
-    cat2 = _refine_stage(P, (blob2, c2), cat3, "deconv2", flow3, "upsample_flow3to2", be)
+    _, cat5 = _head_and_stage(P, c6, "Convolution1", (blob5, c5), c6, "deconv5", "upsample_flow6to5", be)
+    _, cat4 = _head_and_stage(P, be.conv(cat5, P, "interconv5", 1, 1, act=False), "Convolution2", (blob4, c4), cat5, "deconv4", "upsample_flow5to4", be)
+    _, cat3 = _head_and_stage(P, be.conv(cat4, P, "interconv4", 1, 1, act=False), "Convolution3", (blob3, c3), cat4, "deconv3", "upsample_flow4to3", be)
+    _, cat2 = _head_and_stage(P, be.conv(cat3, P, "interconv3", 1, 1, act=False), "Convolution4", (blob2, c2), cat3, "deconv2", "upsample_flow3to2", be)
     return be.predict_flow(be.conv(cat2, P, "interconv2", 1, 1, act=False), P, "Convolution5")
 
 
@@ -515,10 +536,8 @@
     blob0, c0 = _conv_into_concat(x, P, "conv0", 1, 1, 16 + 2, be)
     blob1, c1 = _conv_into_concat(be.conv(c0, P, "conv1", 2, 1), P, "conv1_1", 1, 1, 32 + 2, be)
     c2 = be.conv(be.conv(c1, P, "conv2", 2, 1), P, "conv2_1", 1, 1)
-    flow2 = be.predict_flow(c2, P, "Convolution5")
-    cat1 = _refine_stage(P, (blob1, c1), c2, "deconv1", flow2, "upsample_flow2to1", be)
-    flow1 = be.predict_flow(be.conv(cat1, P, "interconv1", 1, 1, act=False), P, "Convolution6")
-    cat0 = _refine_stage(P, (blob0, c0), cat1, "deconv0", flow1, "upsample_flow1to0", be)
+    _, cat1 = _head_and_stage(P, c2, "Convolution5", (blob1, c1), c2, "deconv1", "upsample_flow2to1", be)
+    _, cat0 = _head_and_stage(P, be.conv(cat1, P, "interconv1", 1, 1, act=False), "Convolution6", (blob0, c0), cat1, "deconv0", "upsample_flow1to0", be)
     return be.predict_flow(be.conv(cat0, P, "interconv0", 1, 1, act=False), P, "Convolution7")
 
 
diff --git a/flownet2_amd/ops.py b/flownet2_amd/ops.py
--- a/flownet2_amd/ops.py
+++ b/flownet2_amd/ops.py
@@ -505,6 +505,63 @@
     out = torch.empty((N, 2, 2 * H, 2 * W), device=x.device, dtype=torch.float32)
     check(_lib.lib().fn2_upsample_flow_deconv_forward(_ptr(x), _ptr(w), _ptr(b), _ptr(out), N, H, W, _stream()))
     return out
+
+
+def predict_flow_taps_forward(x, weight):
+    x, w = _chk(x, "bottom[0]"), _chk(weight, "weight")
+    N, Cc, H, W = x.shape
+    if tuple(w.shape) != (2, Cc, 3, 3):
+        raise ValueError(f"predict_flow weight must be [2,{Cc},3,3], got {tuple(w.shape)}")
+    splits = _lib.lib().fn2_predict_flow_splits(N, Cc, H, W)
+    P = torch.empty((splits, N, 18, H, W), device=x.device, dtype=torch.float32)
+    check(_lib.lib().fn2_predict_flow_taps_forward(_ptr(x), _ptr(w), _ptr(P), P.numel() * 4, N, Cc, H, W, _stream()))
+    return P, splits
+
+
+def _chk_taps(P):
+    P = _chk(P, "tap image", ndim=5)
+    if P.shape[2] != 18 or P.shape[0] not in (1, 2, 4, 8):
+        raise ValueError(f"tap image must be [splits,N,18,H,W] with 1, 2, 4 or 8 splits, got {tuple(P.shape)}")
+    return P
+
+
+def flow_gather_upsample_forward(P, bias, up_weight, up_bias, out, out_c0):
+    P, uw = _chk_taps(P), _chk(up_weight, "upsample weight")
+    splits, N, _, H, W = P.shape
+    if tuple(uw.shape) != (2, 2, 4, 4):
+        raise ValueError("upsample_flow expects a [2,2,4,4] weight")
+    b, ub = _chk_opt(bias, "bias", 1), _chk_opt(up_bias, "upsample bias", 1)
+    _chk(out, "top[0]")
+    if out.shape[0] != N or tuple(out.shape[2:]) != (2 * H, 2 * W) or not out.is_contiguous():
+        raise ValueError(f"flow_gather_upsample: top blob {tuple(out.shape)} is not a contiguous [{N},*,{2 * H},{2 * W}]")
+    flow = torch.empty((N, 2, H, W), device=P.device, dtype=torch.float32)
+    check(_lib.lib().fn2_flow_gather_upsample_forward(_ptr(P), splits, _ptr(b), _ptr(flow), _ptr(uw), _ptr(ub), _ptr(out), out.shape[1], int(out_c0),
+                                                      N, H, W, _stream()))
+    return flow
+
+
+def flow_gather_resample_forward(P, bias, height, width, in_scale=1.0):
+    P = _chk_taps(P)
+    splits, N, _, H, W = P.shape
+    b = _chk_opt(bias, "bias", 1)
+    out = torch.empty((N, 2, int(height), int(width)), device=P.device, dtype=torch.float32)
+    check(_lib.lib().fn2_flow_gather_resample_forward(_ptr(P), splits, _ptr(b), C.c_float(float(in_scale)), _ptr(out), N, H, W, int(height), int(width), _stream()))
+    return out
+
+
+def scale_shift_forward_pair(x0, x1, scale, shift, out0, out1, out0_c0=0, out1_c0=0):
+    x0, x1 = _chk(x0, "bottom[0]"), _chk(x1, "bottom[1]")
+    N, Cc, H, W = x0.shape
+    for t in (out0, out1):
+        _chk(t, "top")
+        if not t.is_contiguous() or t.shape[0] != N or tuple(t.shape[2:]) != (H, W) or t.shape[1] != out0.shape[1]:
+            raise ValueError("scale_shift_pair: a top blob does not match the bottoms")
+    if x1.shape != x0.shape:
+        raise ValueError("scale_shift_pair: the two bottoms differ in shape")
+    s = _chk_opt(shift, "shift", 1)
+    check(_lib.lib().fn2_scale_shift_forward_pair(_ptr(x0), _ptr(out0), int(out0_c0), _ptr(x1), _ptr(out1), int(out1_c0), _ptr(s), N, Cc, H, W,
+                                                  out0.shape[1], C.c_float(float(scale)), _stream()))
+    return out0, out1
 
 
 def bias_leaky_relu_(x, bias=None, negative_slope=0.1):
diff --git a/include/flownet2_hip_decoder_fusion.h b/include/flownet2_hip_decoder_fusion.h
--- /dev/null
+++ b/include/flownet2_hip_decoder_fusion.h
@@ -0,0 +1,26 @@
+#ifndef FLOWNET2_HIP_DECODER_FUSION_H_
+#define FLOWNET2_HIP_DECODER_FUSION_H_
+
+#include <stddef.h>
+
+#ifdef __cplusplus
+extern "C" {
+#endif
+
+int fn2_predict_flow_splits(int N, int C, int H, int W);
+
+int fn2_predict_flow_taps_forward(const float* in, const float* weight, float* P, size_t P_bytes, int N, int C, int H, int W, void* stream);
+
+int fn2_flow_gather_upsample_forward(const float* P, int splits, const float* bias, float* flow, const float* up_weight, const float* up_bias,
+                                     float* top, int top_channels, int top_c0, int N, int H, int W, void* stream);
+
+int fn2_flow_gather_resample_forward(const float* P, int splits, const float* bias, float in_scale, float* out, int N, int H, int W,
+                                     int Hout, int Wout, void* stream);
+
+int fn2_scale_shift_forward_pair(const float* bottom0, float* top0, int top0_c0, const float* bottom1, float* top1, int top1_c0,
+                                 const float* shift, int N, int C, int H, int W, int top_channels, float scale, void* stream);
+
+#ifdef __cplusplus
+}
+#endif
+#endif
```

Measured after the change: 3603, median of 6. Within noise of the previous version (+0.5%).
